# koide3/hdl_graph_slam

Measured on AMD Instinct MI355X. Metric: registrations/sec (64-beam ~120k-pt pair), loop-closure batch, higher is better.
Workload: dtype f64; 1 GPU; loop-closure batch: 64 candidate keyframes/GPU x HDL-64E (~118848 pts) vs 1 query keyframe, FAST_GICP + getFitnessScore, cold (index + covariances rebuilt every step); candidate set: SURVEY 8d (distinct ray-casts at poses within 20 m of the query, guess = ground truth + 0.5 m / 2 deg noise, z forced to 0); candidates_per_gpu=64, points_per_cloud=118848, method=FAST_GICP, distinct_scans=16, parallelism=single GPU

## Files before the change

hdl_graph_slam_amd/csrc/hgs_consts.h:

```cpp
#pragma once
#include <cfloat>
#include <cmath>

#include "../../include/hgs_registration.h"
#include "hgs_floor.h"
#include "hgs_gicp.h"
#include "hgs_icp.h"
#include "hgs_ndt.h"
#include "hgs_vgicp.h"

namespace hgs {

inline GicpConsts gicp_consts(const hgs_params& p) {
  GicpConsts c;
  const double thr = p.max_correspondence_distance;
  c.max_corr2 = thr * thr;
  c.search_bound2 = c.max_corr2 >= (double)FLT_MAX ? FLT_MAX : nextafterf((float)c.max_corr2, FLT_MAX);
  c.rotation_eps = p.rotation_epsilon;
  c.translation_eps = p.transformation_epsilon;
  c.lm_init_lambda_factor = p.lm_init_lambda_factor;
  c.lm_max_iterations = p.lm_max_iterations;
  c.max_iterations = p.max_iterations;
  c.k_correspondences = p.correspondence_randomness;
  return c;
}

inline VgicpConsts vgicp_consts(const hgs_params& p) {
  VgicpConsts c;
  c.resolution = p.resolution;
  c.search = p.neighbor_search == HGS_DIRECT27 ? 3 : (p.neighbor_search == HGS_DIRECT7 ? 2 : 1);
  c.pad = 0;
  return c;
}

inline IcpConsts icp_consts(const hgs_params& p) {
  IcpConsts c;
  const double thr = p.max_correspondence_distance;
  c.max_corr2 = thr * thr;
  c.search_bound2 = c.max_corr2 >= (double)FLT_MAX ? FLT_MAX : nextafterf((float)c.max_corr2, FLT_MAX);
  c.max_iterations = p.max_iterations;
  c.trans_eps = p.transformation_epsilon;
  c.rot_thr = p.rotation_epsilon > 0 ? p.rotation_epsilon : 1.0 - p.transformation_epsilon;
  c.reciprocal = p.icp_reciprocal ? 1 : 0;
  c.pad = 0;
  return c;
}

inline NdtConsts ndt_consts(const hgs_params& p) {
  NdtConsts c;
  const double c1 = 10.0 * (1 - p.ndt_outlier_ratio);
  const double c2 = p.ndt_outlier_ratio / std::pow(p.resolution, 3);
  const double d3 = -std::log(c2);
  c.gauss_d1 = -std::log(c1 + c2) - d3;
  c.gauss_d2 = -2 * std::log((-std::log(c1 * std::exp(-0.5) + c2) - d3) / c.gauss_d1);
  c.step_size = p.ndt_step_size;
  c.trans_eps = p.transformation_epsilon;
  c.max_iterations = p.max_iterations;
  c.search = p.neighbor_search == HGS_DIRECT1 ? 1 : (p.neighbor_search == HGS_KDTREE ? 0 : 2);
  c.kdtree_radius2 = (float)(p.resolution * p.resolution);
  c.line_search = p.ndt_line_search ? 1 : 0;
  c.upstream_hd1_sign = p.ndt_upstream_hd1_sign;
  c.pad = 0;
  return c;
}

inline FloorConsts floor_consts(const hgs_floor_params* p) {
  FloorConsts c{};
  const double angle = (double)(float)(p->tilt_deg * M_PI / 180.0);
  c.rx = p->tilt_deg == 0.0 ? 0.f : -(float)std::sin(angle);
  c.rz = p->tilt_deg == 0.0 ? 1.f : (float)std::cos(angle);
  c.nrx = (double)c.rx, c.nrz = (double)c.rz;
  c.clip_lo = (float)(p->sensor_height + p->height_clip_range);
  c.clip_hi = (float)(p->sensor_height - p->height_clip_range);
  c.normal_cos = std::cos(p->normal_filter_thresh * M_PI / 180.0);
  c.dist_thresh = p->ransac_distance_threshold;
  c.log_prob = std::log(1.0 - p->ransac_probability);
  c.max_iterations = p->ransac_max_iterations;
  c.seed = p->seed;
  return c;
}

}
```

hdl_graph_slam_amd/csrc/hgs_device.h:

```cpp
#pragma once
#include <hip/hip_runtime.h>
#include "hgs_gicp.h"
#include "hgs_floor.h"
#include "hgs_icp.h"
#include "hgs_ndt.h"
#include "hgs_vgicp.h"

namespace hgs {

struct CloudMeta {
  int nvalid;
  int ndt_ncells;
  unsigned bbmin[3];
  unsigned bbmax[3];
  int ndt_min_b[3], ndt_max_b[3], ndt_div_mul[3];
  int ndt_error;
  int vg_ncells;
  int vg_min_b[3], vg_max_b[3], vg_div_mul[3];
  int vg_error;
  int pad[1];
};

struct CloudDesc {
  const float4* raw;
  float4* pts;
  float4* lpts;
  float4* nodes;
  float4* cov;
  int* corr;
  CloudMeta* meta;
  int n_input;
  int P;
  int sort_off;
  int pad;
};

struct TargetView {
  const float4* nodes;
  const float4* pts;
  const float4* lpts;
  const float4* cov;
  const CloudMeta* meta;
  int P;
  int seed_bits;
  const unsigned* seed_tab;
};

struct NdtTargetView {
  const int* hash_keys;
  const int* hash_vals;
  const NdtCellRec* cells;
  const CloudMeta* meta;
  const int2* hash_kv;
  int hash_mask;
  float inv_leaf;
};

struct NdtAccum {
  unsigned long long w[kAccNdt * 4];
  unsigned tiles_done;
  unsigned overflow;
  double out[kAccNdt];
};

struct DevResult {
  float T[16];
  int converged, iterations, lm_tries, pad;
  double error;
  double fit_sum;
  unsigned fit_count;
  unsigned pad2;
};

struct Progress {
  int* dev;
  volatile int* host_done;
  volatile int* host_rounds;
  int B;
  int pad;
};

constexpr int kFusedRoundMaxProblems = 4;
constexpr int kBlock = 256;
constexpr int kKnnLaneList = 16;
constexpr int kKnnLeafLog = 128;
constexpr int kNW = 1;
constexpr int kTileNN = kBlock * kNW;

void launch_pack_aos(hipStream_t s, const float4* staged , int n, float4* raw, float* intensity , CloudMeta* meta_to_reset ,
                     const CloudDesc* desc = nullptr , CloudDesc* desc_out = nullptr);
void launch_meta_init(hipStream_t s, const CloudDesc* descs, int ncloud);
void launch_bbox_count(hipStream_t s, const CloudDesc* descs, int ncloud, int max_n);
void launch_hilbert_keys(hipStream_t s, const CloudDesc* descs, int ncloud, int max_n, unsigned long long* keys, unsigned* vals, int drop_bits);
void launch_gather_sorted(hipStream_t s, const CloudDesc* descs, int ncloud, int max_slots, const unsigned* sorted_vals);
void launch_build_tree(hipStream_t s, const CloudDesc* descs, int ncloud, int max_P);
void launch_knn_cov(hipStream_t s, const CloudDesc* descs, int ncloud, int max_n, int k, int qpw, int reg_method, int gather ,
                    double* raw_stage = nullptr );

void launch_gicp_init(hipStream_t s, GicpState* states, const float* guesses, int B, Progress prog);
struct Guess16 {
  float m[16];
};
void launch_gicp_init1(hipStream_t s, GicpState* states, const float* guess_host , Progress prog);
void launch_gicp_linearize(hipStream_t s, const CloudDesc* descs, TargetView tgt, const GicpState* states, GicpConsts c, double* partials, int max_blocks, int B,
                           int qpw);
void launch_gicp_solve(hipStream_t s, const CloudDesc* descs, GicpState* states, GicpConsts c, const double* partials, int max_blocks, int B,
                       int tile_points );
void launch_gicp_error(hipStream_t s, const CloudDesc* descs, TargetView tgt, const GicpState* states, double* partials_err, int max_blocks, int B);
void launch_gicp_linearize_round2(hipStream_t s, const CloudDesc* descs, TargetView tgt, const GicpState* states_in, GicpState* states_out, GicpConsts c, double* partials,
                                  const double* partials_err, int max_blocks , int lin_blocks , int B, int qpw, Progress prog,
                                  DevResult* results, DevResult* early_out );
void launch_gicp_error_round2(hipStream_t s, const CloudDesc* descs, TargetView tgt, const GicpState* states_in, GicpState* states_out, GicpConsts c, const double* partials,
                              double* partials_err, int max_blocks, int err_blocks , int B, int lin_tile_points);
void launch_gicp_decide(hipStream_t s, const CloudDesc* descs, GicpState* states, GicpConsts c, const double* partials_err, int max_blocks, int B, Progress prog);
void launch_gicp_results(hipStream_t s, const GicpState* states, DevResult* out, int B);

void launch_icp_init(hipStream_t s, IcpState* states, const float* guesses, int B, Progress prog);
void launch_icp_correspond(hipStream_t s, const CloudDesc* descs, TargetView tgt, const IcpState* states, IcpConsts c, double* partials, int max_blocks, int B);
void launch_icp_solve(hipStream_t s, const CloudDesc* descs, IcpState* states, IcpConsts c, const double* partials, int max_blocks, int B, Progress prog);
void launch_icp_results(hipStream_t s, const IcpState* states, DevResult* out, int B);

void launch_fitness(hipStream_t s, const CloudDesc* descs, TargetView tgt, const DevResult* poses, double max_range, double* partials, int max_blocks, int B,
                    int use_seed, int qpw);
void launch_fitness_final(hipStream_t s, const CloudDesc* descs, const double* partials, int max_blocks, DevResult* out, int B, int tile_pts);
void launch_gicp_linearize(hipStream_t s, const CloudDesc* descs, const TargetView* tviews, const GicpState* states, GicpConsts c, double* partials, int max_blocks, int B,
                           int qpw);
void launch_gicp_error(hipStream_t s, const CloudDesc* descs, const TargetView* tviews, const GicpState* states, double* partials_err, int max_blocks, int B);
void launch_gicp_linearize_round2(hipStream_t s, const CloudDesc* descs, const TargetView* tviews, const GicpState* states_in, GicpState* states_out, GicpConsts c, double* partials,
                                  const double* partials_err, int max_blocks, int lin_blocks, int B, int qpw, Progress prog, DevResult* results, DevResult* early_out);
void launch_gicp_error_round2(hipStream_t s, const CloudDesc* descs, const TargetView* tviews, const GicpState* states_in, GicpState* states_out, GicpConsts c, const double* partials,
                              double* partials_err, int max_blocks, int err_blocks, int B, int lin_tile_points);
void launch_icp_correspond(hipStream_t s, const CloudDesc* descs, const TargetView* tviews, const IcpState* states, IcpConsts c, double* partials, int max_blocks, int B);
void launch_fitness(hipStream_t s, const CloudDesc* descs, const TargetView* tviews, const DevResult* poses, double max_range, double* partials, int max_blocks, int B,
                    int use_seed, int qpw);
}
struct hgs_result;
namespace hgs {
void launch_results_to_records(hipStream_t s, const DevResult* res, const int* candidate_ids, int n, int n_slots, ::hgs_result* out);
void launch_nn_query(hipStream_t s, TargetView tgt, const float4* q, int nq, int* idx, float* d2);
void launch_seed_grid_build(hipStream_t s, const float4* pts, const CloudMeta* meta, int n_max, unsigned* tab, int bits);
inline size_t seed_grid_entries(int bits) { return ((size_t)1 << bits) + ((size_t)1 << (bits - 2)) + ((size_t)1 << (bits - 4)); }
struct SeedGridJob {
  const float4* pts;
  const CloudMeta* meta;
  unsigned* tab;
  int bits;
  int pad;
};
void launch_seed_grid_build_batch(hipStream_t s, const SeedGridJob* jobs, int njobs, size_t max_entries, int max_n);
void launch_transform(hipStream_t s, const float4* raw, int n, const float* T16_colmajor_dev, float4* out);

void launch_ndt_grid_params(hipStream_t s, CloudDesc desc, float inv_leaf);
void launch_ndt_cell_keys(hipStream_t s, CloudDesc desc, float inv_leaf, unsigned long long* keys, unsigned* vals);
void launch_ndt_build_cells(hipStream_t s, CloudDesc desc, const unsigned long long* sorted_keys, const unsigned* sorted_vals, int min_points,
                            int* hash_keys, int* hash_vals, int hash_mask, NdtCellRec* cells);
void launch_ndt_init(hipStream_t s, NdtState* states, NdtAngles* angles, const float* guesses, NdtConsts c, int B, Progress prog, NdtAccum* accum_to_zero );
void launch_ndt_pack_hash(hipStream_t s, const int* keys, const int* vals, int2* kv, int cap);
void launch_ndt_pass(hipStream_t s, const CloudDesc* descs, NdtTargetView tgt, NdtState* states, NdtAngles* angles, NdtConsts c, NdtAccum* accum, const int* tile_base,
                     unsigned long long* queues, int B, int parity, int blocks, int chunk, int sorted, int debug, Progress prog);
void launch_ndt_pass(hipStream_t s, const CloudDesc* descs, const NdtTargetView* tviews, NdtState* states, NdtAngles* angles, NdtConsts c, NdtAccum* accum, const int* tile_base,
                     unsigned long long* queues, int B, int parity, int blocks, int chunk, int sorted, int debug, Progress prog);
void launch_ndt_results(hipStream_t s, const CloudDesc* descs, const NdtState* states, DevResult* out, int B);

void launch_vgicp_grid_params(hipStream_t s, CloudDesc desc, double resolution);
void launch_vgicp_cell_keys(hipStream_t s, CloudDesc desc, double resolution, unsigned long long* keys, unsigned* vals);
void launch_vgicp_build_cells(hipStream_t s, CloudDesc desc, const unsigned long long* sorted_keys, const unsigned* sorted_vals, int* hash_keys,
                              int* hash_vals, int hash_mask, NdtCellRec* cells);
void launch_vgicp_linearize(hipStream_t s, const CloudDesc* descs, NdtTargetView tgt, const GicpState* states, VgicpConsts c, double* partials,
                            int max_blocks, int B);
void launch_vgicp_error(hipStream_t s, const CloudDesc* descs, NdtTargetView tgt, const GicpState* states, VgicpConsts c, double* partials_err,
                        int max_blocks, int B);
void launch_vgicp_linearize(hipStream_t s, const CloudDesc* descs, const NdtTargetView* tviews, const GicpState* states, VgicpConsts c, double* partials,
                            int max_blocks, int B);
void launch_vgicp_error(hipStream_t s, const CloudDesc* descs, const NdtTargetView* tviews, const GicpState* states, VgicpConsts c, double* partials_err,
                        int max_blocks, int B);

struct MapSource {
  const float4* raw;
  const float* intensity;
  int n, offset;
  float T[16];
};
void launch_map_transform(hipStream_t s, const MapSource* srcs, int nsrc, int max_n, float4* out);
constexpr int kMapMaxDepth = 21;
constexpr int kMapMaxEvents = kMapMaxDepth + 3;
struct MapOctreeEvent {
  int index, depth;
  double mn[3];
  unsigned long long gained[3];
};
struct MapOctree {
  int first;
  int next_viol;
  int n_events, overflow, done, pad;
  double mx[3];
  MapOctreeEvent events[kMapMaxEvents];
};
void launch_map_first_finite(hipStream_t s, const float4* pts, int n, MapOctree* oct);
void launch_map_octree_init(hipStream_t s, const float4* pts, int n, double res, MapOctree* oct);
void launch_map_octree_step(hipStream_t s, const float4* pts, int n, double res, MapOctree* oct);
void launch_map_keys(hipStream_t s, const float4* pts, int n, double res, const MapOctree* oct, unsigned long long* keys, unsigned* vals);
void launch_map_centers(hipStream_t s, const unsigned long long* keys, const unsigned* head, const unsigned* slot, int n, double res, const MapOctree* oct, float4* out,
                        int* count_out);

struct PfFrame {
  float rows[12];
};
void launch_pf_load(hipStream_t s, const float4* staged, int n, float4* out, const float* deskew_w , double scan_period,
                    const PfFrame* frame , int* count_out, unsigned* meta_out );
void launch_pf_distance_flags(hipStream_t s, const float4* pts, int n, int use_filter, double near_thresh, double far_thresh, unsigned* keep);
void launch_pf_compact(hipStream_t s, const float4* in, int n, const unsigned* keep, const unsigned* slot, float4* out, int* count);
void launch_pf_bbox(hipStream_t s, const float4* pts, const int* count, int cap, unsigned* meta, int dist_filter = 0, double near_thresh = 0, double far_thresh = 0);
void launch_pf_grid(hipStream_t s, unsigned* meta, float inv_leaf);
void launch_pf_voxel_keys(hipStream_t s, const float4* pts, const int* count, const unsigned* meta, float inv_leaf, int cap, unsigned long long* keys, unsigned* vals,
                          int dist_filter = 0, double near_thresh = 0, double far_thresh = 0);
void launch_pf_voxel_heads(hipStream_t s, const unsigned long long* keys, int cap, unsigned* head, unsigned long long invalid_key);
constexpr unsigned long long kVoxelInvalidKey = 0xffffffffull;
constexpr unsigned long long kMapInvalidKey = ~0ull;
void launch_pf_voxel_centroids(hipStream_t s, const float4* pts, const unsigned long long* keys, const unsigned* vals, const unsigned* head, const unsigned* slot, int cap,
                               float4* out, int* count_out, unsigned* ukeys = nullptr );
void launch_pf_grid_radius_flags(hipStream_t s, const float4* cen, const int* count, const unsigned* ukeys, const unsigned* meta, float inv_leaf, float radius, float r2,
                                 int min_neighbors, int cap, unsigned* keep);
void launch_pf_approx_keys(hipStream_t s, const float4* pts, const int* count, float inv_leaf, int cap, unsigned long long* keys, unsigned* vals);
void launch_pf_approx_heads(hipStream_t s, const float4* pts, const unsigned long long* keys, const unsigned* vals, float inv_leaf, int cap, unsigned* head, unsigned* evict,
                            unsigned* bucket_used , unsigned* bucket_rank );
void launch_pf_approx_centroids(hipStream_t s, const float4* pts, const unsigned long long* keys, const unsigned* vals, const unsigned* head, const unsigned* evict,
                                const unsigned* evict_rank, const unsigned* bucket_rank, int cap, float4* out, int* count_out);
void launch_pf_radius_flags(hipStream_t s, CloudDesc d, float r2, int min_neighbors, unsigned* keep);
void launch_pf_mean_knn_dist(hipStream_t s, CloudDesc d, int mean_k, double* dist);
void launch_pf_statistical(hipStream_t s, CloudDesc d, const double* dist, double* stats, double stddev_mul, unsigned* keep);
void launch_pf_to_cloud(hipStream_t s, const float4* in, int n, float4* raw, float* intensity, CloudMeta* meta_to_reset, const CloudDesc* desc = nullptr, CloudDesc* desc_out = nullptr);

struct PfSweep {
  int off, n;
  int count;
  int deskew, frame;
  float w[3];
  double scan_period;
  float rows[12];
  unsigned meta[16];
};
constexpr int kPfBatchOrdinalBits = 12;
void launch_pfb_load(hipStream_t s, const float4* staged, PfSweep* sweeps, int nsweeps, int max_n, float4* out);
void launch_pfb_distance_flags(hipStream_t s, const float4* pts, const PfSweep* sweeps, int nsweeps, int max_n, double near_thresh, double far_thresh, unsigned* keep);
void launch_pfb_compact(hipStream_t s, const float4* in, PfSweep* sweeps, int nsweeps, int max_n, const unsigned* keep, const unsigned* slot, float4* out);
void launch_pfb_bbox(hipStream_t s, const float4* pts, PfSweep* sweeps, int nsweeps, int max_n, int dist_filter, double near_thresh, double far_thresh);
void launch_pfb_grid(hipStream_t s, PfSweep* sweeps, int nsweeps, float inv_leaf);
void launch_pfb_voxel_keys(hipStream_t s, const float4* pts, const PfSweep* sweeps, int nsweeps, int max_n, float inv_leaf, unsigned long long* keys, unsigned* vals,
                           int dist_filter, double near_thresh, double far_thresh);
void launch_pfb_voxel_heads(hipStream_t s, const unsigned long long* keys, const PfSweep* sweeps, int nsweeps, int max_n, unsigned* head);
void launch_pfb_voxel_centroids(hipStream_t s, const float4* pts, const unsigned long long* keys, const unsigned* vals, const unsigned* head, const unsigned* slot,
                                PfSweep* sweeps, int nsweeps, int max_n, float4* out, unsigned* ukeys );
void launch_pfb_grid_radius_flags(hipStream_t s, const float4* cen, const unsigned* ukeys, const PfSweep* sweeps, int nsweeps, int max_n, float inv_leaf, float radius,
                                  float r2, int min_neighbors, unsigned* keep);
void launch_pfb_to_cloud(hipStream_t s, const float4* in, const PfSweep* sweeps, const CloudDesc* descs, CloudDesc* const* desc_outs, float* const* intensities, int nsweeps,
                         int max_m);

void launch_floor_clip_flags(hipStream_t s, const float4* raw, const float* intensity, int n, FloorConsts c, float4* out , unsigned* keep);
void launch_knn_cov_raw(hipStream_t s, const CloudDesc* descs , int max_n, int k, int qpw, int gather, double* raw_stage );
void launch_floor_normal_flags(hipStream_t s, CloudDesc d, const double* raw_cov, FloorConsts c, unsigned* keep , double* normals );
void launch_floor_ransac_init(hipStream_t s, FloorRansacState* st, int max_iterations, Progress prog);
void launch_floor_ransac_planes(hipStream_t s, const float4* pts, int n, unsigned seed, int i0, int nh, const FloorRansacState* st , double* planes ,
                                int* counts );
void launch_floor_ransac_count(hipStream_t s, const float4* pts, int n, double thresh, const double* planes, int nh, const FloorRansacState* st , int* counts);
void launch_floor_ransac_decide(hipStream_t s, const int* counts, const double* planes, int i0, int nh, int n, int max_iterations, double log_prob, FloorRansacState* st,
                                Progress prog);
void launch_floor_inlier_flags(hipStream_t s, const float4* pts, int n, const FloorRansacState* st, double thresh, unsigned* keep);

void launch_gicp_debug_state(hipStream_t s, GicpState* st, const double* T12_dev);
void launch_ndt_debug_state(hipStream_t s, NdtState* st, NdtAngles* ang, const double* p6_dev, NdtConsts c);
void launch_reduce_partials(hipStream_t s, const double* partials, int ntiles, int width , double* out);

}
```

hdl_graph_slam_amd/csrc/hgs_engine.hip:

```cpp
#include <hip/hip_runtime.h>
#include <algorithm>
#include <atomic>
#include <chrono>
#include <climits>
#include <condition_variable>
#include <cmath>
#include <cstdio>
#include <cstdlib>
#include <cstring>
#include <exception>
#include <limits>
#include <mutex>
#include <new>
#include <stdexcept>
#include <string>
#include <thread>
#include <vector>

#include "../../include/hgs_registration.h"
#include "hgs_comm.h"
#include "hgs_consts.h"
#include "hgs_device.h"
#include "hgs_resources.h"
#include "hgs_sort.h"

using namespace hgs;

namespace {

thread_local std::string g_create_error;


int next_pow2(int v) {
  int p = 1;
  while (p < v) p <<= 1;
  return p;
}
size_t align_up(size_t v, size_t a) { return (v + a - 1) / a * a; }

}

struct VoxelTable {
  DeviceBuffer block;
  int* hash_keys = nullptr;
  int* hash_vals = nullptr;
  int2* hash_kv = nullptr;
  NdtCellRec* cells = nullptr;
  int hash_cap = 0;
};

struct hgs_cloud {
  hgs_handle* owner = nullptr;
  size_t n_input = 0;
  int P = 1;
  DeviceBuffer block;
  CloudDesc desc{};
  CloudDesc* dev_desc = nullptr;
  float* intensity = nullptr;
  bool has_index = false;
  bool corr_stale = false;
  bool has_cov = false;
  int cov_k = 0;
  bool has_ndt = false;
  double ndt_resolution = 0;
  int ndt_min_points = 0;
  VoxelTable ndt;
  bool has_vg = false;
  double vg_resolution = 0;
  int vg_cov_k = 0;
  long long vg_span[3] = {0, 0, 0};
  bool vg_too_large = false;
  VoxelTable vg;
  bool has_seed = false;
  DeviceBuffer seed_block;
  int seed_bits = 0;
};

struct ProfEvent {
  int stage;
  hipEvent_t a, b;
};

struct hgs_handle {
  hgs_params prm{};
  int device = 0;
  hipStream_t stream = nullptr;
  hipStream_t lane_stream[7] = {};
  hipEvent_t lane_event[8] = {};
  int lane_start = 1;
  int nn_qpw = 0;
  int nn_qpw16_below = 96, nn_qpw32_below = 0;
  int hilbert_levels = 13;
  hipEvent_t comm_event = nullptr;
  int prefilter_fast = 1;
  int upload_trace = 0;
  int floor_chunk = 64;
  int early_run_ahead = 2;
  int early_result = 1;
  PinnedBuffer h_early;
  hipEvent_t early_event = nullptr;
  bool early_pending = false, early_valid = false;
  int fused_rounds = 1;
  int fused_rounds_below = 262144;
  int fused_rounds_max_problems = kFusedRoundMaxProblems, fused_rounds_max_blocks = 640;
  int cov_split = 1;
  int resident_descs = 1;
  int knn_qpw_tiny = -1;
  int knn_tiny_below = 32768;
  int seed_grid = 1;
  int knn_replay = -1;
  int batch_lanes = 0;
  std::string err;
  hgs_cloud* target = nullptr;
  hgs_cloud* source = nullptr;
  bool own_target = false, own_source = false;
  float final_T[16];

  DeviceBuffer staging, sort_keys[2], sort_vals[2], sort_tmp, descs, states, angles, partials, partials_err, results, guesses, done, misc;
  DeviceBuffer lane_partials[7], lane_partials_err[7];
  DeviceBuffer ndt_accum;
  DeviceBuffer group_tviews, group_corr;
  DeviceBuffer group_vviews;
  DeviceBuffer seed_jobs;
  int pair_chunk = 0;
  hgs::Comm* comm = nullptr;
  DeviceBuffer comm_send, comm_recv, comm_ids;
  DeviceBuffer pf_ukeys;
  DeviceBuffer cov_raw;
  DeviceBuffer ndt_plan;
  int ndt_resident_blocks = 0;
  int ndt_chunk = 0;
  int ndt_sort = -1;
  DeviceBuffer pf_a, pf_b, pf_keep, pf_slot, pf_small, pf_dist;
  DeviceBuffer pf_table;
  PinnedBuffer h_pf_table;
  PinnedBuffer h_results, h_small, h_flags, h_comm;
  PinnedRing up;
  PinnedRing up_points;
  PinnedBuffer up_big;
  hipEvent_t up_big_event = nullptr;
  bool up_big_pending = false;
  PackPool pack_pool;
  PinnedBuffer h_xform;

  std::vector<DeviceBuffer> block_pool;
  std::vector<hgs_cloud*> live_clouds;
  std::recursive_mutex api_mutex;

  bool profiling = false;
  std::vector<ProfEvent> prof_events;
  std::vector<ProfEvent> prof_free;
  double prof_ms[HGS_STAGE_COUNT];
  uint64_t prof_launches[HGS_STAGE_COUNT];

  hgs_handle() = default;
  hgs_handle(const hgs_handle&) = delete;
  hgs_handle& operator=(const hgs_handle&) = delete;
  void synchronize_streams() {
    if (stream) (void)hipStreamSynchronize(stream);
    for (hipStream_t ls : lane_stream)
      if (ls) (void)hipStreamSynchronize(ls);
  }
  ~hgs_handle();
};

namespace {

#define HGS_HIP(h, call)                                                                                           \
  do {                                                                                                             \
    hipError_t e__ = (call);                                                                                       \
    if (e__ != hipSuccess) {                                                                                       \
      char buf__[512];                                                                                             \
      snprintf(buf__, sizeof(buf__), "%s failed: %s (%s:%d)", #call, hipGetErrorString(e__), __FILE__, __LINE__);  \
      (h)->err = buf__;                                                                                            \
      return HGS_ERR_HIP;                                                                                          \
    }                                                                                                              \
  } while (0)

#define HGS_TRY(expr)             \
  do {                            \
    int rc__ = (expr);            \
    if (rc__ != HGS_OK) return rc__; \
  } while (0)

struct StageTimer {
  hgs_handle* h;
  ProfEvent ev{};
  bool active = false;
  StageTimer(hgs_handle* h_, int stage) : h(h_) {
    if (!h->profiling) return;
    if (!h->prof_free.empty()) {
      ev = h->prof_free.back();
      h->prof_free.pop_back();
    } else {
      if (hipEventCreate(&ev.a) != hipSuccess || hipEventCreate(&ev.b) != hipSuccess) return;
    }
    ev.stage = stage;
    active = hipEventRecord(ev.a, h->stream) == hipSuccess;
  }
  ~StageTimer() {
    if (!active) return;
    (void)hipEventRecord(ev.b, h->stream);
    h->prof_events.push_back(ev);
  }
};

struct ApiLock {
  std::unique_lock<std::recursive_mutex> lk;
  explicit ApiLock(hgs_handle* h) {
    if (h) lk = std::unique_lock<std::recursive_mutex>(h->api_mutex);
  }
  explicit ApiLock(hgs_cloud* c) : ApiLock(c ? c->owner : nullptr) {}
};

int set_device(hgs_handle* h) {
  HGS_HIP(h, hipSetDevice(h->device));
  return HGS_OK;
}

constexpr size_t kUploadChunkPoints = 16384;
#ifndef HGS_UPLOAD_PARALLEL_POINTS
#define HGS_UPLOAD_PARALLEL_POINTS 49152
#endif
constexpr size_t kUploadParallelPoints = HGS_UPLOAD_PARALLEL_POINTS;
int upload_image_open(hgs_handle* h, size_t records) {
  if (h->up_big_pending) {
    HGS_HIP(h, hipEventSynchronize(h->up_big_event));
    h->up_big_pending = false;
  }
  HGS_HIP(h, h->up_big.reserve(records * sizeof(float4)));
  return HGS_OK;
}
int upload_image_close(hgs_handle* h) {
  if (!h->up_big_event) HGS_HIP(h, hipEventCreateWithFlags(&h->up_big_event, hipEventDisableTiming));
  HGS_HIP(h, hipEventRecord(h->up_big_event, h->stream));
  h->up_big_pending = true;
  return HGS_OK;
}
int upload_points_at(hgs_handle* h, const void* pts, size_t n, size_t stride_bytes, size_t off, bool in_image) {
  const bool has_intensity = stride_bytes >= 20;
  const char* src = static_cast<const char*>(pts);
  float4* const dev = h->staging.as<float4>() + off;
  if (n >= kUploadParallelPoints) {
    if (!in_image) HGS_TRY(upload_image_open(h, n));
    float4* const image = h->up_big.as<float4>() + (in_image ? off : 0);
    const size_t nchunks = (n + kUploadChunkPoints - 1) / kUploadChunkPoints;
    std::vector<std::atomic<unsigned char>> ready(nchunks);
    for (auto& r : ready) r.store(0, std::memory_order_relaxed);
    PackPool::Job job;
    job.src = src, job.dst = reinterpret_cast<float*>(image), job.n = n, job.stride = stride_bytes, job.chunk = kUploadChunkPoints, job.nchunks = nchunks;
    job.has_intensity = has_intensity, job.ready = ready.data();
    h->pack_pool.post(&job);
    hipError_t err = hipSuccess;
    for (size_t c = 0; c < nchunks; c++) {
      while (!ready[c].load(std::memory_order_acquire))
        if (!PackPool::help(job)) std::this_thread::yield();
      const size_t i0 = c * kUploadChunkPoints, m = std::min(kUploadChunkPoints, n - i0);
      if (err == hipSuccess) err = hipMemcpyAsync(dev + i0, image + i0, m * sizeof(float4), hipMemcpyHostToDevice, h->stream);
    }
    h->pack_pool.retire();
    HGS_HIP(h, err);
    if (!in_image) HGS_TRY(upload_image_close(h));
    return HGS_OK;
// ... 250 lines not shown
}

template <typename P, typename K, typename C>
int build_voxel_table(hgs_handle* h, const hgs_cloud* c, VoxelTable& t, int cap, int max_cells, bool packed, P&& grid_params, K&& cell_keys, C&& build_cells) {
  const size_t n = c->n_input;
  if (!t.block.p || t.hash_cap != cap) {
    const size_t o_keys = 0, o_vals = align_up((size_t)cap * 4, 256), o_kv = o_vals + align_up((size_t)cap * 4, 256);
    const size_t o_cells = o_kv + (packed ? align_up((size_t)cap * 8, 256) : 0);
    HGS_HIP(h, t.block.alloc(o_cells + (size_t)max_cells * sizeof(NdtCellRec)));
    char* base = t.block.as<char>();
    t.hash_keys = (int*)(base + o_keys);
    t.hash_vals = (int*)(base + o_vals);
    t.hash_kv = packed ? (int2*)(base + o_kv) : nullptr;
    t.cells = (NdtCellRec*)(base + o_cells);
    t.hash_cap = cap;
  }
  HGS_HIP(h, hipMemsetAsync(t.hash_keys, 0xff, (size_t)cap * 4, h->stream));
  grid_params();
  if (n > 0) {
    HGS_TRY(reserve_sort_pairs(h, n));
    cell_keys(h->sort_keys[0].as<unsigned long long>(), h->sort_vals[0].as<unsigned>());
    HGS_TRY(sort_pairs(h, n, 0, 32));
    build_cells(h->sort_keys[1].as<unsigned long long>(), h->sort_vals[1].as<unsigned>());
  }
  return HGS_OK;
}

int ensure_ndt_target(hgs_handle* h, hgs_cloud* c) {
  const double res = h->prm.resolution;
  const int min_pts = h->prm.ndt_min_points_per_voxel;
  if (c->has_ndt && c->ndt_resolution == res && c->ndt_min_points == min_pts) return HGS_OK;
  StageTimer tm(h, HGS_STAGE_VOXELIZE);
  const int max_cells = (int)(c->n_input / (size_t)std::max(1, min_pts)) + 1;
  const int cap = next_pow2(std::max(64, 4 * max_cells));
  const float inv_leaf = 1.0f / (float)res;
  VoxelTable& t = c->ndt;
  HGS_TRY(build_voxel_table(
      h, c, t, cap, max_cells, true, [&] { launch_ndt_grid_params(h->stream, c->desc, inv_leaf); },
      [&](unsigned long long* keys, unsigned* vals) { launch_ndt_cell_keys(h->stream, c->desc, inv_leaf, keys, vals); },
      [&](unsigned long long* keys, unsigned* vals) { launch_ndt_build_cells(h->stream, c->desc, keys, vals, min_pts, t.hash_keys, t.hash_vals, cap - 1, t.cells); }));
  launch_ndt_pack_hash(h->stream, t.hash_keys, t.hash_vals, t.hash_kv, cap);
  HGS_HIP(h, hipGetLastError());
  c->has_ndt = true;
  c->ndt_resolution = res;
  c->ndt_min_points = min_pts;
  return HGS_OK;
}

int vgicp_grid_too_large(hgs_handle* h, const hgs_cloud* c) {
  char msg[256];
  snprintf(msg, sizeof(msg),
           "FAST_VGICP: the target's voxel grid spans %lld x %lld x %lld cells at resolution %g, more than the 2147483647 a linear voxel key addresses "
           "(a far stray point in the target?)",
           c->vg_span[0], c->vg_span[1], c->vg_span[2], c->vg_resolution);
  h->err = msg;
  return HGS_ERR_UNSUPPORTED;
}

int ensure_vgicp_target(hgs_handle* h, hgs_cloud* c) {
  const double res = h->prm.resolution;
  const int k = h->prm.correspondence_randomness;
  if (c->has_vg && c->vg_resolution == res && c->vg_cov_k == cov_cache_key(h, k)) return c->vg_too_large ? vgicp_grid_too_large(h, c) : HGS_OK;
  StageTimer tm(h, HGS_STAGE_VOXELIZE);
  const int max_cells = (int)c->n_input + 1;
  const int cap = next_pow2(std::max<int>(64, 2 * max_cells));
  VoxelTable& t = c->vg;
  HGS_TRY(build_voxel_table(
      h, c, t, cap, max_cells, false, [&] { launch_vgicp_grid_params(h->stream, c->desc, res); },
      [&](unsigned long long* keys, unsigned* vals) { launch_vgicp_cell_keys(h->stream, c->desc, res, keys, vals); },
      [&](unsigned long long* keys, unsigned* vals) { launch_vgicp_build_cells(h->stream, c->desc, keys, vals, t.hash_keys, t.hash_vals, cap - 1, t.cells); }));
  HGS_HIP(h, hipGetLastError());
  HGS_HIP(h, h->h_small.reserve(sizeof(CloudMeta)));
  const CloudMeta* hm = h->h_small.as<CloudMeta>();
  HGS_HIP(h, hipMemcpyAsync(h->h_small.p, c->desc.meta, sizeof(CloudMeta), hipMemcpyDeviceToHost, h->stream));
  HGS_HIP(h, hipStreamSynchronize(h->stream));
  for (int d = 0; d < 3; d++) c->vg_span[d] = (long long)hm->vg_max_b[d] - hm->vg_min_b[d] + 1;
  c->vg_too_large = hm->vg_error != 0;
  c->has_vg = true;
  c->vg_resolution = res;
  c->vg_cov_k = cov_cache_key(h, k);
  return c->vg_too_large ? vgicp_grid_too_large(h, c) : HGS_OK;
}

NdtTargetView voxel_target_view(const hgs_cloud* c, const VoxelTable& t, float inv_leaf) {
  NdtTargetView tv;
  tv.hash_keys = t.hash_keys, tv.hash_vals = t.hash_vals, tv.cells = t.cells, tv.meta = c->desc.meta, tv.hash_kv = t.hash_kv;
  tv.hash_mask = t.hash_cap - 1, tv.inv_leaf = inv_leaf;
  return tv;
}
NdtTargetView ndt_target_view(const hgs_handle* h, const hgs_cloud* t) { return voxel_target_view(t, t->ndt, 1.0f / (float)h->prm.resolution); }
NdtTargetView vgicp_target_view(const hgs_cloud* t) { return voxel_target_view(t, t->vg, 0.f); }

TargetView target_view(const hgs_cloud* c) {
  TargetView t;
  t.nodes = c->desc.nodes, t.pts = c->desc.pts, t.lpts = c->desc.lpts, t.cov = c->desc.cov, t.meta = c->desc.meta, t.P = c->P;
  t.seed_bits = c->has_seed ? c->seed_bits : 0, t.seed_tab = c->has_seed ? c->seed_block.as<const unsigned>() : nullptr;
  return t;
}

int ensure_seed_grid(hgs_handle* h, hgs_cloud* c) {
  if (!h->seed_grid || c->has_seed || !c->has_index || c->n_input == 0) return HGS_OK;
  int bits = 12;
  while (bits < 24 && ((size_t)1 << bits) < 4 * c->n_input) bits++;
  const size_t bytes = seed_grid_entries(bits) * sizeof(unsigned);
  if (!c->seed_block.p || c->seed_bits != bits) {
    HGS_HIP(h, c->seed_block.alloc(bytes));
    c->seed_bits = bits;
  }
  HGS_HIP(h, hipMemsetAsync(c->seed_block.p, 0xff, bytes, h->stream));
  launch_seed_grid_build(h->stream, c->desc.pts, c->desc.meta, (int)c->n_input, c->seed_block.as<unsigned>(), bits);
  HGS_HIP(h, hipGetLastError());
  c->has_seed = true;
  return HGS_OK;
}

int ensure_seed_grids(hgs_handle* h, const std::vector<hgs_cloud*>& all) {
  if (!h->seed_grid) return HGS_OK;
  std::vector<hgs_cloud*> todo;
  for (hgs_cloud* c : all)
    if (!c->has_seed && c->has_index && c->n_input > 0 && std::find(todo.begin(), todo.end(), c) == todo.end()) todo.push_back(c);
  constexpr size_t kMaxJobs = 65535;
  for (size_t start = 0; start < todo.size(); start += kMaxJobs) {
    const size_t nj = std::min(kMaxJobs, todo.size() - start);
    std::vector<SeedGridJob> jobs(nj);
    size_t max_entries = 0;
    int max_n = 0;
    for (size_t j = 0; j < nj; j++) {
      hgs_cloud* c = todo[start + j];
      int bits = 12;
      while (bits < 24 && ((size_t)1 << bits) < 4 * c->n_input) bits++;
      const size_t entries = seed_grid_entries(bits);
      if (!c->seed_block.p || c->seed_bits != bits) {
        HGS_HIP(h, c->seed_block.alloc(entries * sizeof(unsigned)));
        c->seed_bits = bits;
      }
      jobs[j] = SeedGridJob{c->desc.pts, c->desc.meta, c->seed_block.as<unsigned>(), bits, 0};
      max_entries = std::max(max_entries, entries), max_n = std::max(max_n, (int)c->n_input);
    }
    HGS_HIP(h, h->seed_jobs.reserve(nj * sizeof(SeedGridJob)));
    HGS_HIP(h, h->up.upload(h->seed_jobs.p, jobs.data(), nj * sizeof(SeedGridJob), h->stream));
    launch_seed_grid_build_batch(h->stream, h->seed_jobs.as<SeedGridJob>(), (int)nj, max_entries, max_n);
    HGS_HIP(h, hipGetLastError());
    for (size_t j = 0; j < nj; j++) todo[start + j]->has_seed = true;
  }
  return HGS_OK;
}

NdtConsts engine_ndt_consts(const hgs_params& p) {
  NdtConsts c = ndt_consts(p);
  c.pad = std::getenv("HGS_TRACE") ? 1 : 0;
  return c;
}

constexpr int kMaxCountedDevices = 64;
std::atomic<int> g_streams_in_use[kMaxCountedDevices] = {};
std::atomic<int>& streams_in_use(int device) { return g_streams_in_use[(unsigned)device % kMaxCountedDevices]; }
int hw_queue_budget() {
  static const int budget = [] {
    const char* e = std::getenv("GPU_MAX_HW_QUEUES");
    const int v = e ? std::atoi(e) : 0;
    return v > 0 ? v : 4;
  }();
  return budget;
}
constexpr int kFloorMaxChunk = 4096;
constexpr int kMaxLanes = 8;

int make_progress(hgs_handle* h, int lane, int B, Progress* out) {
  if (h->early_pending) {
    HGS_HIP(h, hipEventSynchronize(h->early_event));
    h->early_pending = false;
  }
  HGS_HIP(h, h->done.reserve(64));
  HGS_HIP(h, h->h_flags.reserve(64));
  volatile int* hf = h->h_flags.as<volatile int>() + 2 * lane;
  hf[0] = 0, hf[1] = 0;
  out->dev = h->done.as<int>() + 2 * lane;
  out->host_done = hf, out->host_rounds = hf + 1;
  out->B = B, out->pad = 0;
  return HGS_OK;
}

struct BatchLane {
  hipStream_t stream = nullptr;
  int b0 = 0, B = 0;
  Progress prog{};
  double* partials = nullptr;
  double* partials_err = nullptr;
  long round = 0;
  bool finished = false;
};

int open_lanes(hgs_handle* h, int B, size_t partial_bytes_per_problem, size_t partial_err_bytes_per_problem, std::vector<BatchLane>& lanes, int tiles_per_problem) {
  const bool small_problems = tiles_per_problem > 0 && tiles_per_problem <= 96;
  const int by_size = h->prm.method == HGS_NDT_OMP ? (B > 32 && !small_problems ? 3 : 4) : (small_problems && (long)B * tiles_per_problem <= 3072 ? 1 : 4);
  const int wanted = h->batch_lanes > 0 ? h->batch_lanes : by_size;
  int n = h->profiling ? 1 : std::max(1, std::min(std::min(wanted, kMaxLanes), B));
  if (h->batch_lanes <= 0) {
    int owned = 0;
    while (owned < kMaxLanes - 1 && h->lane_stream[owned]) owned++;
    const int room = std::max(0, hw_queue_budget() - streams_in_use(h->device).load(std::memory_order_relaxed));
    n = std::min(n, 1 + owned + room);
  }
  lanes.assign(n, BatchLane{});
  for (int i = 0, b0 = 0; i < n; i++) {
    BatchLane& L = lanes[i];
    L.b0 = b0, L.B = (B - b0) / (n - i);
    b0 += L.B;
    HGS_TRY(make_progress(h, i, L.B, &L.prog));
    if (i == 0) {
      L.stream = h->stream;
      L.partials = h->partials.as<double>(), L.partials_err = h->partials_err.as<double>();
      continue;
    }
    if (!h->lane_stream[i - 1]) {
      HGS_HIP(h, hipStreamCreateWithFlags(&h->lane_stream[i - 1], hipStreamNonBlocking));
      streams_in_use(h->device).fetch_add(1, std::memory_order_relaxed);
    }
    L.stream = h->lane_stream[i - 1];
    HGS_HIP(h, h->lane_partials[i - 1].reserve((size_t)L.B * partial_bytes_per_problem));
    HGS_HIP(h, h->lane_partials_err[i - 1].reserve((size_t)L.B * partial_err_bytes_per_problem));
    L.partials = h->lane_partials[i - 1].as<double>(), L.partials_err = h->lane_partials_err[i - 1].as<double>();
  }
  if (n > 1) {
    if (h->lane_start != 0) HGS_HIP(h, hipStreamSynchronize(h->stream));
    if (!h->lane_event[0]) HGS_HIP(h, hipEventCreateWithFlags(&h->lane_event[0], hipEventDisableTiming));
    HGS_HIP(h, hipEventRecord(h->lane_event[0], h->stream));
    for (int i = 1; i < n; i++) HGS_HIP(h, hipStreamWaitEvent(lanes[i].stream, h->lane_event[0], 0));
  }
  return HGS_OK;
}

int close_lanes(hgs_handle* h, std::vector<BatchLane>& lanes) {
  for (size_t i = 1; i < lanes.size(); i++) {
    if (!h->lane_event[i]) HGS_HIP(h, hipEventCreateWithFlags(&h->lane_event[i], hipEventDisableTiming));
    HGS_HIP(h, hipEventRecord(h->lane_event[i], lanes[i].stream));
    HGS_HIP(h, hipStreamWaitEvent(h->stream, h->lane_event[i], 0));
  }
  return HGS_OK;
}

constexpr long kRunAhead = 2;
template <typename F, typename G>
void drive_lanes(std::vector<BatchLane>& lanes, long max_rounds, F&& enqueue_round, G&& on_finished, long run_ahead = kRunAhead) {
  long spins = 0;
  for (;;) {
    bool all_finished = true, enqueued = false;
    for (BatchLane& L : lanes) {
      if (L.finished) continue;
      if (*L.prog.host_done || L.round >= max_rounds) {
        L.finished = true;
        on_finished(L);
        continue;
      }
      all_finished = false;
      if (L.round - (long)*L.prog.host_rounds < run_ahead) {
        enqueue_round(L);
        L.round++;
        enqueued = true;
      }
    }
    if (all_finished) return;
    if (enqueued) {
      spins = 0;
      continue;
    }
    if ((++spins & 0x3ff) == 0) {
      for (BatchLane& L : lanes)
        if (!L.finished && !*L.prog.host_done && hipStreamQuery(L.stream) == hipSuccess && !*L.prog.host_done &&
            L.round - (long)*L.prog.host_rounds >= run_ahead) {
          enqueue_round(L);
          L.round++;
        }
    }
#if defined(__x86_64__)
    __builtin_ia32_pause();
#endif
  }
}

struct BatchShape {
  int B, max_n;
  int qpw, nn_tile;
  bool gicp_round2;
  int lin_qpw, lin_tile, lin_blocks;
  int max_blocks, err_blocks;
  const CloudDesc* d_descs;
  const TargetView* d_tviews;
  const NdtTargetView* d_vviews;
};

template <typename F>
void with_lane_target(const BatchShape& s, const BatchLane& L, const TargetView& tv, F&& launch) {
  if (s.d_tviews) launch(s.d_tviews + L.b0);
  else launch(tv);
}

int batch_shape(hgs_handle* h, const std::vector<hgs_cloud*>& sources, bool lm_rounds, BatchShape* out, int* const* corr_of = nullptr) {
  BatchShape& s = *out;
  s.d_tviews = nullptr, s.d_vviews = nullptr;
  s.B = (int)sources.size();
  s.max_n = 0;
  for (hgs_cloud* c : sources) s.max_n = std::max(s.max_n, (int)c->n_input);
  const int B = s.B, max_n = s.max_n;
  s.qpw = 64;
  s.nn_tile = (kBlock / 64) * s.qpw * kNW;
  s.gicp_round2 = lm_rounds && h->prm.method == HGS_FAST_GICP && h->fused_rounds && max_n <= h->fused_rounds_below &&
                  (B <= h->fused_rounds_max_problems || (long)B * ((max_n + kBlock - 1) / kBlock) <= (long)h->fused_rounds_max_blocks);
  const long tiles64 = (long)B * ((max_n + s.nn_tile - 1) / s.nn_tile);
  s.lin_qpw = !s.gicp_round2 ? 64 : h->nn_qpw > 0 ? h->nn_qpw : tiles64 <= (long)h->nn_qpw16_below ? 16 : tiles64 <= (long)h->nn_qpw32_below ? 32 : 64;
  s.lin_tile = (kBlock / 64) * s.lin_qpw * kNW;
  s.lin_blocks = std::max(1, (max_n + s.lin_tile - 1) / s.lin_tile);
  s.max_blocks = std::max(1, s.lin_qpw < 64 ? (max_n + 63) / 64 : (max_n + s.nn_tile - 1) / s.nn_tile);
  s.err_blocks = std::max(1, (max_n + kBlock - 1) / kBlock);
  return upload_descs(h, sources, false, &s.d_descs, nullptr, corr_of);
}

bool corr_seeds_fitness(int method) { return method == HGS_FAST_GICP || method == HGS_ICP; }
void lane_fitness(hgs_handle* h, BatchLane& L, const BatchShape& s, double max_range, bool corr_seeds) {
  StageTimer tm(h, HGS_STAGE_FITNESS);
  DevResult* res = h->results.as<DevResult>() + L.b0;
  with_lane_target(s, L, s.d_tviews ? TargetView{} : target_view(h->target),
                   [&](auto tgt) { launch_fitness(L.stream, s.d_descs + L.b0, tgt, res, max_range, L.partials_err, s.max_blocks, L.B, corr_seeds ? 1 : 0, s.qpw); });
  launch_fitness_final(L.stream, s.d_descs + L.b0, L.partials_err, s.max_blocks, res, L.B, s.nn_tile);
}
void lane_fitness_tail(hgs_handle* h, BatchLane& L, const BatchShape& s, const double* fit_max_range) {
  if (fit_max_range) lane_fitness(h, L, s, *fit_max_range, corr_seeds_fitness(h->prm.method));
}

int run_gicp_rounds(hgs_handle* h, const BatchShape& s, const float* guesses_host, bool guess_in_args, const double* fit_max_range) {
  const int B = s.B, max_blocks = s.max_blocks;
  hgs_cloud* tgt = h->target;
  const bool voxel = h->prm.method == HGS_FAST_VGICP;
  const GicpConsts c = gicp_consts(h->prm);
  const VgicpConsts vc = vgicp_consts(h->prm);
  const bool round2 = s.gicp_round2;
  const bool early = round2 && B == 1 && !fit_max_range && h->early_result && !h->profiling;
  DevResult* early_out = nullptr;
  if (early) {
    HGS_HIP(h, h->h_early.reserve(sizeof(DevResult)));
    early_out = h->h_early.as<DevResult>();
  }
  HGS_HIP(h, h->states.reserve((size_t)B * sizeof(GicpState) * (round2 ? 2 : 1)));
  GicpState* st = h->states.as<GicpState>();
  GicpState* st_other = st + B;
  const TargetView tv = s.d_tviews || s.d_vviews ? TargetView{} : target_view(tgt);
  const NdtTargetView vtv = voxel && !s.d_vviews ? vgicp_target_view(tgt) : NdtTargetView{};
  const long max_rounds = (long)std::max(1, c.max_iterations) * std::max(1, c.lm_max_iterations) + 2 + (round2 ? 1 : 0);
  std::vector<BatchLane> lanes;
  HGS_TRY(open_lanes(h, B, (size_t)max_blocks * kAccNdt * sizeof(double), (size_t)max_blocks * 2 * sizeof(double), lanes, s.err_blocks));
  auto finish_lane = [&](BatchLane& L) {
    if (early && *L.prog.host_done) {
      h->early_valid = true;
      return;
    }
    launch_gicp_results(L.stream, st + L.b0, h->results.as<DevResult>() + L.b0, L.B);
    lane_fitness_tail(h, L, s, fit_max_range);
  };
  if (guess_in_args) launch_gicp_init1(lanes[0].stream, st, guesses_host, lanes[0].prog);
  else
    for (BatchLane& L : lanes) launch_gicp_init(L.stream, st + L.b0, h->guesses.as<float>() + (size_t)L.b0 * 16, L.B, L.prog);
  drive_lanes(lanes, max_rounds, [&](BatchLane& L) {
    const CloudDesc* dd = s.d_descs + L.b0;
    GicpState* ls = st + L.b0;
    if (round2) {
      {
        StageTimer tm(h, HGS_STAGE_LINEARIZE);
        with_lane_target(s, L, tv, [&](auto t) {
          launch_gicp_linearize_round2(L.stream, dd, t, ls, st_other + L.b0, c, L.partials, L.partials_err, max_blocks, s.lin_blocks, L.B, s.lin_qpw, L.prog,
                                       h->results.as<DevResult>() + L.b0, early_out);
        });
      }
      StageTimer tm(h, HGS_STAGE_ERROR);
      with_lane_target(s, L, tv, [&](auto t) {
        launch_gicp_error_round2(L.stream, dd, t, st_other + L.b0, ls, c, L.partials, L.partials_err, max_blocks, s.err_blocks, L.B, s.lin_tile);
      });
      return;
    }
    {
      StageTimer tm(h, HGS_STAGE_LINEARIZE);
      if (voxel && s.d_vviews) launch_vgicp_linearize(L.stream, dd, s.d_vviews + L.b0, ls, vc, L.partials, max_blocks, L.B);
      else if (voxel) launch_vgicp_linearize(L.stream, dd, vtv, ls, vc, L.partials, max_blocks, L.B);
      else with_lane_target(s, L, tv, [&](auto t) { launch_gicp_linearize(L.stream, dd, t, ls, c, L.partials, max_blocks, L.B, s.qpw); });
    }
    {
      StageTimer tm(h, HGS_STAGE_SOLVE);
      launch_gicp_solve(L.stream, dd, ls, c, L.partials, max_blocks, L.B, voxel ? kBlock : s.nn_tile);
    }
    {
      StageTimer tm(h, HGS_STAGE_ERROR);
      if (voxel && s.d_vviews) launch_vgicp_error(L.stream, dd, s.d_vviews + L.b0, ls, vc, L.partials_err, max_blocks, L.B);
      else if (voxel) launch_vgicp_error(L.stream, dd, vtv, ls, vc, L.partials_err, max_blocks, L.B);
      else with_lane_target(s, L, tv, [&](auto t) { launch_gicp_error(L.stream, dd, t, ls, L.partials_err, max_blocks, L.B); });
    }
    {
      StageTimer tm(h, HGS_STAGE_SOLVE);
      launch_gicp_decide(L.stream, dd, ls, c, L.partials_err, max_blocks, L.B, L.prog);
    }
  }, finish_lane, early ? (long)h->early_run_ahead : kRunAhead);
  HGS_TRY(close_lanes(h, lanes));
  if (h->early_valid) {
    if (!h->early_event) HGS_HIP(h, hipEventCreateWithFlags(&h->early_event, hipEventDisableTiming));
    HGS_HIP(h, hipEventRecord(h->early_event, h->stream));
    h->early_pending = true;
  }
  return HGS_OK;
}

int run_icp_rounds(hgs_handle* h, const BatchShape& s, const double* fit_max_range) {
  const int B = s.B, max_blocks = s.max_blocks;
  const IcpConsts c = icp_consts(h->prm);
  HGS_HIP(h, h->states.reserve((size_t)B * sizeof(IcpState)));
  IcpState* st = h->states.as<IcpState>();
  const TargetView tv = s.d_tviews ? TargetView{} : target_view(h->target);
  const long max_rounds = (long)std::max(0, c.max_iterations) + 2;
  std::vector<BatchLane> lanes;
  HGS_TRY(open_lanes(h, B, (size_t)max_blocks * kAccIcp * sizeof(double), (size_t)max_blocks * 2 * sizeof(double), lanes, s.err_blocks));
  auto finish_lane = [&](BatchLane& L) {
    launch_icp_results(L.stream, st + L.b0, h->results.as<DevResult>() + L.b0, L.B);
    lane_fitness_tail(h, L, s, fit_max_range);
  };
  for (BatchLane& L : lanes) launch_icp_init(L.stream, st + L.b0, h->guesses.as<float>() + (size_t)L.b0 * 16, L.B, L.prog);
  drive_lanes(lanes, max_rounds, [&](BatchLane& L) {
    {
      StageTimer tm(h, HGS_STAGE_LINEARIZE);
      with_lane_target(s, L, tv, [&](auto t) { launch_icp_correspond(L.stream, s.d_descs + L.b0, t, st + L.b0, c, L.partials, max_blocks, L.B); });
    }
    StageTimer tm(h, HGS_STAGE_SOLVE);
    launch_icp_solve(L.stream, s.d_descs + L.b0, st + L.b0, c, L.partials, max_blocks, L.B, L.prog);
  }, finish_lane);
  return close_lanes(h, lanes);
}

struct NdtLanePlan {
  int* tile_base;
  unsigned long long* queues;
  int blocks, chunk;
};
int ndt_lane_plans(hgs_handle* h, const std::vector<hgs_cloud*>& sources, const std::vector<BatchLane>& lanes, std::vector<NdtLanePlan>& plans) {
  plans.assign(lanes.size(), NdtLanePlan{});
  const size_t per_lane = align_up(16 + (sources.size() + 1) * sizeof(int), 256);
  bool tile_overflow = false;
  constexpr long long kMaxNdtBlocks = 1 << 16, kMaxNdtChunk = 1 << 10;
  HGS_HIP(h, h->ndt_plan.reserve(per_lane * lanes.size()));
  void* staged = nullptr;
  int plan_slot = 0;
  HGS_HIP(h, h->up.stage(per_lane * lanes.size(), &staged, &plan_slot));
  std::memset(staged, 0, per_lane * lanes.size());
  char* const host = static_cast<char*>(staged);
  for (size_t li = 0; li < lanes.size(); li++) {
    const BatchLane& L = lanes[li];
    int* tb = reinterpret_cast<int*>(host + li * per_lane + 16);
    tb[0] = 0;
    long long tiles64 = 0;
    for (int k = 0; k < L.B; k++) {
      tiles64 += std::max<long long>(1, ((long long)sources[L.b0 + k]->n_input + kBlock - 1) / kBlock);
      tile_overflow = tile_overflow || tiles64 > (long long)INT_MAX - (long long)kMaxNdtBlocks * kMaxNdtChunk;
      tb[k + 1] = tile_overflow ? 0 : (int)tiles64;
    }
    NdtLanePlan& P = plans[li];
    const int total = tb[L.B];
    if (tile_overflow) continue;
    P.blocks = std::max(1, std::min(total, h->ndt_resident_blocks > 0 ? std::min(h->ndt_resident_blocks, (int)kMaxNdtBlocks) : (lanes.size() > 1 ? 512 : 768)));
    P.chunk = h->ndt_chunk > 0 ? std::min(h->ndt_chunk, (int)kMaxNdtChunk) : 8;
    P.queues = reinterpret_cast<unsigned long long*>((char*)h->ndt_plan.p + li * per_lane);
    P.tile_base = reinterpret_cast<int*>((char*)h->ndt_plan.p + li * per_lane + 16);
  }
  if (tile_overflow) {
    h->err = "NDT batch too large: the tiles of one lane do not fit 32-bit item arithmetic (more than ~5e11 source points in one call)";
    return HGS_ERR_INVALID_ARGUMENT;
  }
  HGS_HIP(h, hipMemcpyAsync(h->ndt_plan.p, host, per_lane * lanes.size(), hipMemcpyHostToDevice, h->stream));
  HGS_HIP(h, h->up.commit(plan_slot, h->stream));
  if (lanes.size() > 1) {
    HGS_HIP(h, hipEventRecord(h->lane_event[0], h->stream));
    for (size_t i = 1; i < lanes.size(); i++) HGS_HIP(h, hipStreamWaitEvent(lanes[i].stream, h->lane_event[0], 0));
  }
  return HGS_OK;
}

int run_ndt_rounds(hgs_handle* h, const std::vector<hgs_cloud*>& sources, const BatchShape& s, const double* fit_max_range) {
  const int B = s.B, max_blocks = s.max_blocks;
  const NdtConsts c = engine_ndt_consts(h->prm);
  HGS_HIP(h, h->states.reserve((size_t)B * sizeof(NdtState)));
  HGS_HIP(h, h->angles.reserve((size_t)B * sizeof(NdtAngles)));
  NdtState* st = h->states.as<NdtState>();
  NdtAngles* ang = h->angles.as<NdtAngles>();
  const NdtTargetView tv = s.d_vviews ? NdtTargetView{} : ndt_target_view(h, h->target);
  if (h->ndt_sort == 1) HGS_TRY(ensure_index(h, sources));
  bool sorted = h->ndt_sort != 0;
  for (hgs_cloud* sc : sources) sorted = sorted && sc->has_index;
  HGS_HIP(h, h->ndt_accum.reserve((size_t)B * sizeof(NdtAccum)));
  NdtAccum* accum = h->ndt_accum.as<NdtAccum>();
  const long max_rounds = ((long)c.max_iterations + 4) * (c.line_search ? 11 : 1);
  std::vector<BatchLane> lanes;
  HGS_TRY(open_lanes(h, B, (size_t)max_blocks * 2 * sizeof(double), (size_t)max_blocks * 2 * sizeof(double), lanes, s.err_blocks));
  auto finish_lane = [&](BatchLane& L) {
    launch_ndt_results(L.stream, s.d_descs + L.b0, st + L.b0, h->results.as<DevResult>() + L.b0, L.B);
    lane_fitness_tail(h, L, s, fit_max_range);
  };
  std::vector<NdtLanePlan> plans;
  HGS_TRY(ndt_lane_plans(h, sources, lanes, plans));
  for (BatchLane& L : lanes) launch_ndt_init(L.stream, st + L.b0, ang + L.b0, h->guesses.as<float>() + (size_t)L.b0 * 16, c, L.B, L.prog, accum + L.b0);
  drive_lanes(lanes, max_rounds, [&](BatchLane& L) {
    StageTimer tm(h, HGS_STAGE_LINEARIZE);
    const NdtLanePlan& P = plans[&L - lanes.data()];
    if (s.d_vviews)
      launch_ndt_pass(L.stream, s.d_descs + L.b0, s.d_vviews + L.b0, st + L.b0, ang + L.b0, c, accum + L.b0, P.tile_base, P.queues, L.B, (int)(L.round & 1), P.blocks,
                      P.chunk, sorted ? 1 : 0, 0, L.prog);
    else
      launch_ndt_pass(L.stream, s.d_descs + L.b0, tv, st + L.b0, ang + L.b0, c, accum + L.b0, P.tile_base, P.queues, L.B, (int)(L.round & 1), P.blocks, P.chunk,
                      sorted ? 1 : 0, 0, L.prog);
  }, finish_lane);
  return close_lanes(h, lanes);
}

int run_batch(hgs_handle* h, const std::vector<hgs_cloud*>& sources, const float* guesses_host, const double* fit_max_range = nullptr) {
  const int B = (int)sources.size();
  h->early_valid = false;
  hgs_cloud* tgt = h->target;
  const int method = h->prm.method;
  const bool gicp = method == HGS_FAST_GICP || method == HGS_FAST_VGICP;
  std::vector<hgs_cloud*> all(sources);
  if (fit_max_range) {
    std::vector<hgs_cloud*> searched(sources);
    searched.push_back(tgt);
    HGS_TRY(ensure_index(h, searched));
  }
  if (gicp) {
    all.push_back(tgt);
    HGS_TRY(ensure_cov(h, all, h->prm.correspondence_randomness));
    if (method == HGS_FAST_VGICP) HGS_TRY(ensure_vgicp_target(h, tgt));
  } else if (method == HGS_ICP) {
    all.push_back(tgt);
    HGS_TRY(ensure_index(h, all));
  } else {
    HGS_TRY(ensure_ndt_target(h, tgt));
  }
  if (fit_max_range && method != HGS_FAST_GICP) HGS_TRY(ensure_seed_grid(h, tgt));
  BatchShape s;
  HGS_TRY(batch_shape(h, sources, true, &s));
  const bool guess_in_args = B == 1 && method == HGS_FAST_GICP;
  HGS_HIP(h, h->guesses.reserve((size_t)B * 16 * sizeof(float)));
  if (!guess_in_args) HGS_HIP(h, h->up.upload(h->guesses.p, guesses_host, (size_t)B * 16 * sizeof(float), h->stream));
  HGS_HIP(h, h->results.reserve((size_t)B * sizeof(DevResult)));
  HGS_HIP(h, h->partials.reserve((size_t)B * s.max_blocks * kAccNdt * sizeof(double)));
  HGS_HIP(h, h->partials_err.reserve((size_t)B * s.max_blocks * 2 * sizeof(double)));
  if (gicp) HGS_TRY(run_gicp_rounds(h, s, guesses_host, guess_in_args, fit_max_range));
  else if (method == HGS_ICP) HGS_TRY(run_icp_rounds(h, s, fit_max_range));
  else HGS_TRY(run_ndt_rounds(h, sources, s, fit_max_range));
  HGS_HIP(h, hipGetLastError());
  return HGS_OK;
}

int run_group_batch(hgs_handle* h, const std::vector<hgs_cloud*>& targets, const std::vector<hgs_cloud*>& sources, const float* guesses_host, const double* fit_max_range) {
  const int B = (int)sources.size();
  const int method = h->prm.method;
  h->early_valid = false;
  std::vector<hgs_cloud*> all(sources);
  all.insert(all.end(), targets.begin(), targets.end());
  if (method == HGS_FAST_GICP) HGS_TRY(ensure_cov(h, all, h->prm.correspondence_randomness));
  else HGS_TRY(ensure_index(h, all));
  if (fit_max_range && method != HGS_FAST_GICP)
    for (hgs_cloud* t : targets) HGS_TRY(ensure_seed_grid(h, t));
// ... 66 lines not shown
    HGS_HIP(h, h->group_tviews.reserve((size_t)B * sizeof(TargetView)));
    HGS_HIP(h, h->up.upload(h->group_tviews.p, views.data(), (size_t)B * sizeof(TargetView), h->stream));
  }
  BatchShape s;
  HGS_TRY(batch_shape(h, sources, true, &s, voxel ? corr_of.data() : nullptr));
  s.d_vviews = h->group_vviews.as<NdtTargetView>();
  s.d_tviews = fit_max_range ? h->group_tviews.as<TargetView>() : nullptr;
  HGS_HIP(h, h->guesses.reserve((size_t)B * 16 * sizeof(float)));
  HGS_HIP(h, h->up.upload(h->guesses.p, guesses_host, (size_t)B * 16 * sizeof(float), h->stream));
  HGS_HIP(h, h->results.reserve((size_t)B * sizeof(DevResult)));
  HGS_HIP(h, h->partials.reserve((size_t)B * s.max_blocks * kAccNdt * sizeof(double)));
  HGS_HIP(h, h->partials_err.reserve((size_t)B * s.max_blocks * 2 * sizeof(double)));
  if (voxel) HGS_TRY(run_gicp_rounds(h, s, guesses_host, false, fit_max_range));
  else HGS_TRY(run_ndt_rounds(h, sources, s, fit_max_range));
  HGS_HIP(h, hipGetLastError());
  return HGS_OK;
}

int run_fitness(hgs_handle* h, const std::vector<hgs_cloud*>& sources, double max_range, bool use_corr_seeds) {
  std::vector<hgs_cloud*> all(sources);
  all.push_back(h->target);
  HGS_TRY(ensure_index(h, all));
  if (!use_corr_seeds) HGS_TRY(ensure_seed_grid(h, h->target));
  BatchShape s;
  HGS_TRY(batch_shape(h, sources, false, &s));
  HGS_HIP(h, h->partials_err.reserve((size_t)s.B * s.max_blocks * 2 * sizeof(double)));
  BatchLane whole;
  whole.stream = h->stream, whole.B = s.B, whole.partials_err = h->partials_err.as<double>();
  lane_fitness(h, whole, s, max_range, use_corr_seeds);
  HGS_HIP(h, hipGetLastError());
  return HGS_OK;
}

int fetch_results(hgs_handle* h, int B, std::vector<DevResult>& out) {
  HGS_HIP(h, h->h_results.reserve((size_t)B * sizeof(DevResult)));
  HGS_HIP(h, hipMemcpyAsync(h->h_results.p, h->results.p, (size_t)B * sizeof(DevResult), hipMemcpyDeviceToHost, h->stream));
  HGS_HIP(h, hipStreamSynchronize(h->stream));
  out.assign(h->h_results.as<DevResult>(), h->h_results.as<DevResult>() + B);
  return HGS_OK;
}

double fitness_score(const DevResult& d) { return d.fit_count > 0 ? d.fit_sum / (double)d.fit_count : std::numeric_limits<double>::max(); }

int run_pair_fitness(hgs_handle* h, hgs_cloud* const* cloud1, hgs_cloud* const* cloud2, const float* relposes, size_t n_pairs, double max_range,
                     std::vector<DevResult>& out) {
  std::vector<hgs_cloud*> all(cloud2, cloud2 + n_pairs);
  all.insert(all.end(), cloud1, cloud1 + n_pairs);
  HGS_TRY(ensure_index(h, all));
  HGS_TRY(ensure_seed_grids(h, std::vector<hgs_cloud*>(cloud1, cloud1 + n_pairs)));
  const size_t chunk = h->pair_chunk > 0 ? (size_t)h->pair_chunk : 65535;
  out.clear();
  out.reserve(n_pairs);
  for (size_t p0 = 0; p0 < n_pairs; p0 += chunk) {
    const size_t B = std::min(chunk, n_pairs - p0);
    std::vector<TargetView> views(B);
    for (size_t b = 0; b < B; b++) views[b] = target_view(cloud1[p0 + b]);
    HGS_HIP(h, h->group_tviews.reserve(B * sizeof(TargetView)));
    HGS_HIP(h, h->up.upload(h->group_tviews.p, views.data(), B * sizeof(TargetView), h->stream));
    BatchShape s;
    HGS_TRY(batch_shape(h, std::vector<hgs_cloud*>(cloud2 + p0, cloud2 + p0 + B), false, &s));
    s.d_tviews = h->group_tviews.as<TargetView>();
    std::vector<DevResult> poses(B);
    std::memset(poses.data(), 0, B * sizeof(DevResult));
    for (size_t b = 0; b < B; b++) std::memcpy(poses[b].T, relposes + 16 * (p0 + b), sizeof(float) * 16);
    HGS_HIP(h, h->results.reserve(B * sizeof(DevResult)));
    HGS_HIP(h, h->up.upload(h->results.p, poses.data(), B * sizeof(DevResult), h->stream));
    HGS_HIP(h, h->partials_err.reserve(B * s.max_blocks * 2 * sizeof(double)));
    BatchLane whole;
    whole.stream = h->stream, whole.B = (int)B, whole.partials_err = h->partials_err.as<double>();
    lane_fitness(h, whole, s, max_range, false);
    HGS_HIP(h, hipGetLastError());
    std::vector<DevResult> r;
    HGS_TRY(fetch_results(h, (int)B, r));
    out.insert(out.end(), r.begin(), r.end());
  }
  return HGS_OK;
}

void to_public(const DevResult& d, int candidate, bool with_fitness, hgs_result* r) {
  std::memcpy(r->final_transformation, d.T, sizeof(float) * 16);
  r->converged = d.converged;
  r->iterations = d.iterations;
  r->error = d.error;
  r->lm_tries = d.lm_tries;
  r->candidate_id = candidate;
  r->reserved = 0;
  if (with_fitness) {
    r->num_inliers = d.fit_count;
    r->fitness_score = fitness_score(d);
  } else {
    r->num_inliers = 0;
    r->fitness_score = std::numeric_limits<double>::quiet_NaN();
  }
}

int upload_pose_as_result(hgs_handle* h, const float T[16]) {
  HGS_HIP(h, h->results.reserve(sizeof(DevResult)));
  HGS_HIP(h, h->h_results.reserve(sizeof(DevResult)));
  DevResult* r = h->h_results.as<DevResult>();
  std::memset(r, 0, sizeof(DevResult));
  std::memcpy(r->T, T, sizeof(float) * 16);
  HGS_HIP(h, hipMemcpyAsync(h->results.p, r, sizeof(DevResult), hipMemcpyHostToDevice, h->stream));
  return HGS_OK;
}

int status_of_current_exception(hgs_handle* h) noexcept {
  int rc = HGS_ERR_INTERNAL;
  char what[256] = "unknown C++ exception inside the backend";
  try {
    throw;
  } catch (const std::bad_alloc&) {
    rc = HGS_ERR_OUT_OF_MEMORY;
    snprintf(what, sizeof(what), "out of host memory");
  } catch (const std::exception& e) {
    snprintf(what, sizeof(what), "C++ exception inside the backend: %s", e.what());
  } catch (...) {
  }
  try {
    if (h) h->err = what;
    else g_create_error = what;
  } catch (...) {
  }
  return rc;
}

int set_role_cloud(hgs_handle* h, hgs_cloud* c, hgs_cloud* hgs_handle::*role, bool hgs_handle::*own) {
  ApiLock lock(h);
  if (!h || !c || c->owner != h) return HGS_ERR_INVALID_ARGUMENT;
  if (h->*own && h->*role != c) cloud_free(h->*role);
  h->*role = c;
  h->*own = false;
  return HGS_OK;
}
int set_role_points(hgs_handle* h, const void* pts, size_t n, size_t stride_bytes, hgs_cloud* hgs_handle::*role, bool hgs_handle::*own) {
  ApiLock lock(h);
  if (!h) return HGS_ERR_INVALID_ARGUMENT;
  hgs_cloud* c = nullptr;
  HGS_TRY(hgs_cloud_create(h, pts, n, stride_bytes, &c));
  if (h->*own) cloud_free(h->*role);
  h->*role = c;
  h->*own = true;
  return HGS_OK;
}

}

hgs_handle::~hgs_handle() {
  (void)hipSetDevice(device);
  synchronize_streams();
  pack_pool.shutdown();
  if (comm) hgs::comm_destroy(comm);
  for (hipEvent_t ev : lane_event)
    if (ev) (void)hipEventDestroy(ev);
  for (hipEvent_t ev : {comm_event, early_event, up_big_event})
    if (ev) (void)hipEventDestroy(ev);
  for (const std::vector<ProfEvent>* list : {&prof_events, &prof_free})
    for (const ProfEvent& ev : *list) (void)hipEventDestroy(ev.a), (void)hipEventDestroy(ev.b);
  for (hipStream_t ls : lane_stream)
    if (ls) (void)hipStreamDestroy(ls), streams_in_use(device).fetch_sub(1, std::memory_order_relaxed);
  if (stream) (void)hipStreamDestroy(stream), streams_in_use(device).fetch_sub(1, std::memory_order_relaxed);
}

extern "C" {

int hgs_abi_version(void) { return HGS_ABI_VERSION; }

int hgs_debug_set_option(hgs_handle* h, const char* key, int value) try {
  ApiLock lock(h);
  if (!h || !key) return HGS_ERR_INVALID_ARGUMENT;
  const std::string k(key);
  if (k == "batch_lanes") h->batch_lanes = value <= 0 ? 0 : std::min(kMaxLanes, value);
  else if (k == "lane_start") h->lane_start = value != 0 ? 1 : 0;
  else if (k == "ndt_sort") h->ndt_sort = std::max(-1, std::min(1, value));
  else if (k == "cov_split") h->cov_split = value != 0 ? 1 : 0;
  else if (k == "fused_rounds") h->fused_rounds = value != 0 ? 1 : 0;
  else if (k == "early_result") h->early_result = value != 0 ? 1 : 0;
  else if (k == "early_run_ahead") h->early_run_ahead = std::max(1, std::min(8, value));
  else if (k == "fused_rounds_max_problems") h->fused_rounds_max_problems = std::max(0, value);
  else if (k == "fused_rounds_max_blocks") h->fused_rounds_max_blocks = std::max(0, value);
  else if (k == "fused_rounds_below") h->fused_rounds_below = std::max(0, value);
  else if (k == "resident_descs") h->resident_descs = value != 0 ? 1 : 0;
  else if (k == "knn_qpw_tiny") h->knn_qpw_tiny = value < 0 ? -1 : std::max(0, std::min(32, value & ~7));
  else if (k == "knn_tiny_below") h->knn_tiny_below = std::max(0, value);
  else if (k == "seed_grid") h->seed_grid = value != 0 ? 1 : 0;
  else if (k == "knn_replay") h->knn_replay = std::max(-1, std::min(2, value));
  else if (k == "ndt_resident") h->ndt_resident_blocks = std::max(0, value);
  else if (k == "ndt_chunk") h->ndt_chunk = std::max(0, value);
  else if (k == "hilbert_levels") h->hilbert_levels = std::max(4, std::min(16, value));
  else if (k == "nn_qpw") h->nn_qpw = value == 16 ? 16 : (value == 32 ? 32 : (value == 64 ? 64 : 0));
  else if (k == "nn_qpw16_below") h->nn_qpw16_below = std::max(0, value);
  else if (k == "nn_qpw32_below") h->nn_qpw32_below = std::max(0, value);
  else if (k == "upload_trace") h->upload_trace = value != 0 ? 1 : 0;
  else if (k == "prefilter_fast") h->prefilter_fast = value != 0 ? 1 : 0;
  else if (k == "floor_chunk") h->floor_chunk = std::max(1, std::min(kFloorMaxChunk, value));
  else if (k == "pair_chunk") h->pair_chunk = std::max(0, std::min(65535, value));
  else {
    h->err = "hgs_debug_set_option: unknown option '" + k + "'";
    return HGS_ERR_INVALID_ARGUMENT;
  }
  return HGS_OK;
} catch (...) {
  return status_of_current_exception(h);
}

int hgs_params_default(int32_t method, hgs_params* p) try {
  if (!p || method < HGS_FAST_GICP || method > HGS_ICP) return HGS_ERR_INVALID_ARGUMENT;
  std::memset(p, 0, sizeof(*p));
  p->method = method;
  p->max_iterations = 64;
  p->transformation_epsilon = 0.01;
  p->rotation_epsilon = method == HGS_ICP ? 0.0 : 2e-3;
  p->max_correspondence_distance = method == HGS_FAST_GICP || method == HGS_ICP ? 2.5 : (double)FLT_MAX;
  p->correspondence_randomness = 20;
  p->neighbor_search = method == HGS_NDT_OMP ? HGS_DIRECT7 : HGS_DIRECT1;
  p->resolution = method == HGS_NDT_OMP ? 0.5 : 1.0;
  p->ndt_step_size = 0.1;
  p->ndt_outlier_ratio = 0.55;
  p->ndt_min_points_per_voxel = 6;
  p->ndt_upstream_hd1_sign = 1;
  p->lm_max_iterations = 10;
  p->lm_init_lambda_factor = 1e-9;
  p->device_id = 0;
  p->regularization_method = HGS_REG_FROBENIUS;
  p->ndt_line_search = 0;
  p->icp_reciprocal = 0;
  return HGS_OK;
} catch (...) {
  return status_of_current_exception(nullptr);
}

int hgs_create(const hgs_params* p, hgs_handle** out) try {
  if (!p || !out) return HGS_ERR_INVALID_ARGUMENT;
  *out = nullptr;
  if (p->method < HGS_FAST_GICP || p->method > HGS_ICP || p->max_iterations < 0 || p->correspondence_randomness < 1 || p->correspondence_randomness > 64  || !(p->resolution > 0) ||
      p->regularization_method < HGS_REG_FROBENIUS || p->regularization_method > HGS_REG_NONE) {
    g_create_error = "invalid hgs_params";
    return HGS_ERR_INVALID_ARGUMENT;
  }
  int ndev = 0;
  hipError_t e = hipGetDeviceCount(&ndev);
  if (e != hipSuccess || ndev <= 0 || p->device_id < 0 || p->device_id >= ndev) {
    g_create_error = std::string("no usable HIP device: ") + (e != hipSuccess ? hipGetErrorString(e) : "device ordinal out of range");
    return HGS_ERR_NO_DEVICE;
  }
  hgs_handle* h = new hgs_handle();
  h->prm = *p;
  h->device = p->device_id;
  for (int i = 0; i < 16; i++) h->final_T[i] = (i % 5 == 0) ? 1.f : 0.f;
  for (int i = 0; i < HGS_STAGE_COUNT; i++) h->prof_ms[i] = 0, h->prof_launches[i] = 0;
  if (hipSetDevice(h->device) != hipSuccess || hipStreamCreateWithFlags(&h->stream, hipStreamNonBlocking) != hipSuccess) {
    g_create_error = "hipSetDevice / hipStreamCreate failed";
    delete h;
    return HGS_ERR_HIP;
  }
  streams_in_use(h->device).fetch_add(1, std::memory_order_relaxed);
  *out = h;
  return HGS_OK;
} catch (...) {
  return status_of_current_exception(nullptr);
}

int hgs_destroy(hgs_handle* h) try {
  if (!h) return HGS_OK;
  { std::lock_guard<std::recursive_mutex> wait_for_running_call(h->api_mutex); }
  (void)hipSetDevice(h->device);
  h->synchronize_streams();
  if (h->own_target) cloud_free(h->target);
  if (h->own_source) cloud_free(h->source);
  for (hgs_cloud* c : h->live_clouds) {
    cloud_release_device(c, false);
    c->owner = nullptr;
    c->n_input = 0;
  }
  delete h;
  return HGS_OK;
} catch (...) {
  return status_of_current_exception(nullptr);
}

const char* hgs_last_error(const hgs_handle* h) { return h ? h->err.c_str() : g_create_error.c_str(); }

int hgs_cloud_create(hgs_handle* h, const void* pts, size_t n, size_t stride_bytes, hgs_cloud** out) try {
  ApiLock lock(h);
  if (!h || !out || (n > 0 && !pts) || stride_bytes < 12 || (stride_bytes % 4) != 0 || n > (size_t)1 << 30) return HGS_ERR_INVALID_ARGUMENT;
  HGS_TRY(set_device(h));
  const bool trace = h->upload_trace != 0;
  const auto t0 = std::chrono::steady_clock::now();
  hgs_cloud* c = nullptr;
  HGS_TRY(cloud_alloc(h, n, &c));
  const auto t1 = std::chrono::steady_clock::now();
  auto t2 = t1;
  {
    StageTimer tm(h, HGS_STAGE_UPLOAD);
    const float4* staged = nullptr;
    {
      const int rc = upload_points_packed(h, pts, n, stride_bytes, &staged);
      t2 = std::chrono::steady_clock::now();
      if (rc != HGS_OK) {
        cloud_free(c);
        return rc;
      }
    }
    const CloudDesc resident = resident_desc(c);
    launch_pack_aos(h->stream, staged, (int)n, const_cast<float4*>(c->desc.raw), c->intensity, c->desc.meta, &resident, c->dev_desc);
    launch_bbox_count(h->stream, c->dev_desc, 1, (int)n);
    hipError_t e = hipGetLastError();
    if (e != hipSuccess) {
      h->err = std::string("cloud upload failed: ") + hipGetErrorString(e);
      cloud_free(c);
      return HGS_ERR_HIP;
    }
  }
  if (trace) {
    const auto t3 = std::chrono::steady_clock::now();
    auto us = [](auto a, auto b) { return std::chrono::duration<double, std::micro>(b - a).count(); };
    std::fprintf(stderr, "[hgs upload] n %zu: alloc %.1f us, pack + DMA enqueue %.1f us, launches %.1f us\n", n, us(t0, t1), us(t1, t2), us(t2, t3));
  }
  *out = c;
  return HGS_OK;
} catch (...) {
  return status_of_current_exception(h);
}

int hgs_cloud_destroy(hgs_cloud* c) try {
  ApiLock lock(c);
  if (!c) return HGS_OK;
  hgs_handle* h = c->owner;
  if (h) {
    (void)hipSetDevice(h->device);
    (void)hipStreamSynchronize(h->stream);
    if (h->target == c) h->target = nullptr, h->own_target = false;
    if (h->source == c) h->source = nullptr, h->own_source = false;
  }
  cloud_free(c);
  c = nullptr;
  return HGS_OK;
} catch (...) {
// ... 1266 lines not shown
  return HGS_OK;
}

}

extern "C" int hgs_detect_floor(hgs_handle* h, hgs_cloud* cloud, const hgs_floor_params* p, hgs_floor_result* out, hgs_cloud** filtered_out, hgs_cloud** inliers_out) try {
  ApiLock lock(h);
  if (filtered_out) *filtered_out = nullptr;
  if (inliers_out) *inliers_out = nullptr;
  if (!h || !cloud || !p || !out || cloud->owner != h || !floor_params_valid(p)) return HGS_ERR_INVALID_ARGUMENT;
  HGS_TRY(set_device(h));
  std::memset(out, 0, sizeof(*out));
  FloorWork w;
  const int rc = detect_floor_locked(h, cloud, p, out, filtered_out, inliers_out, w);
  cloud_free(w.clipped);
  if (rc != HGS_OK) {
    if (filtered_out && *filtered_out) cloud_free(*filtered_out), *filtered_out = nullptr;
    if (inliers_out && *inliers_out) cloud_free(*inliers_out), *inliers_out = nullptr;
  }
  return rc;
} catch (...) {
  return status_of_current_exception(h);
}

extern "C" int hgs_debug_floor_filter(hgs_handle* h, hgs_cloud* cloud, const hgs_floor_params* p, uint8_t* keep_clip, uint8_t* keep_normal, double* normals3) try {
  ApiLock lock(h);
  if (!h || !cloud || !p || cloud->owner != h || !floor_params_valid(p)) return HGS_ERR_INVALID_ARGUMENT;
  HGS_TRY(set_device(h));
  FloorWork w;
  const int rc = floor_filter(h, cloud, p, floor_consts(p), &w, keep_clip, keep_normal, normals3);
  cloud_free(w.clipped);
  return rc;
} catch (...) {
  return status_of_current_exception(h);
}

extern "C" int hgs_debug_floor_ransac_counts(hgs_handle* h, hgs_cloud* cloud, const hgs_floor_params* p, uint32_t i0, uint32_t n, int32_t* counts, double* coeffs4) try {
  ApiLock lock(h);
  if (!h || !cloud || !p || cloud->owner != h || !floor_params_valid(p) || (n > 0 && !counts) || (uint64_t)i0 + n > 0x7fffffffull) return HGS_ERR_INVALID_ARGUMENT;
  HGS_TRY(set_device(h));
  const int chunk = std::max(1, std::min(kFloorMaxChunk, h->floor_chunk));
  FloorRansacBufs b;
  HGS_TRY(floor_ransac_bufs(h, chunk, &b));
  const FloorConsts c = floor_consts(p);
  const int np = (int)cloud->n_input;
  for (uint32_t done = 0; done < n; done += (uint32_t)chunk) {
    const int nh = (int)std::min<uint32_t>((uint32_t)chunk, n - done);
    launch_floor_ransac_planes(h->stream, cloud->desc.raw, np, c.seed, (int)(i0 + done), nh, nullptr, b.planes, b.counts);
    launch_floor_ransac_count(h->stream, cloud->desc.raw, np, c.dist_thresh, b.planes, nh, nullptr, b.counts);
    HGS_HIP(h, hipGetLastError());
    HGS_HIP(h, hipMemcpyAsync(counts + done, b.counts, (size_t)nh * sizeof(int), hipMemcpyDeviceToHost, h->stream));
    if (coeffs4) HGS_HIP(h, hipMemcpyAsync(coeffs4 + 4 * (size_t)done, b.planes, (size_t)nh * 4 * sizeof(double), hipMemcpyDeviceToHost, h->stream));
    HGS_HIP(h, hipStreamSynchronize(h->stream));
  }
  return HGS_OK;
} catch (...) {
  return status_of_current_exception(h);
}

int hgs_profile_enable(hgs_handle* h, int enabled) try {
  ApiLock lock(h);
  if (!h) return HGS_ERR_INVALID_ARGUMENT;
  h->profiling = enabled != 0;
  return HGS_OK;
} catch (...) {
  return status_of_current_exception(h);
}

int hgs_profile_read(hgs_handle* h, double* ms, uint64_t* launches, int reset) try {
  ApiLock lock(h);
  if (!h) return HGS_ERR_INVALID_ARGUMENT;
  HGS_TRY(set_device(h));
  HGS_HIP(h, hipStreamSynchronize(h->stream));
  for (auto& ev : h->prof_events) {
    float t = 0.f;
    if (hipEventElapsedTime(&t, ev.a, ev.b) == hipSuccess) {
      h->prof_ms[ev.stage] += (double)t;
      h->prof_launches[ev.stage]++;
    }
    h->prof_free.push_back(ev);
  }
  h->prof_events.clear();
  for (int i = 0; i < HGS_STAGE_COUNT; i++) {
    if (ms) ms[i] = h->prof_ms[i];
    if (launches) launches[i] = h->prof_launches[i];
    if (reset) h->prof_ms[i] = 0, h->prof_launches[i] = 0;
  }
  return HGS_OK;
} catch (...) {
  return status_of_current_exception(h);
}

int hgs_synchronize(hgs_handle* h) try {
  ApiLock lock(h);
  if (!h) return HGS_ERR_INVALID_ARGUMENT;
  HGS_TRY(set_device(h));
  HGS_HIP(h, hipStreamSynchronize(h->stream));
  return HGS_OK;
} catch (...) {
  return status_of_current_exception(h);
}

int hgs_debug_target_covariances(hgs_handle* h, float* out6) try {
  ApiLock lock(h);
  if (!h || !out6) return HGS_ERR_INVALID_ARGUMENT;
  if (!h->target) return HGS_ERR_NO_TARGET;
  HGS_TRY(set_device(h));
  hgs_cloud* t = h->target;
  std::vector<hgs_cloud*> all{t};
  HGS_TRY(ensure_cov(h, all, h->prm.correspondence_randomness));
  const size_t slots = (size_t)t->P * kLeaf;
  std::vector<float4> pts(slots), cov(2 * slots);
  int nvalid = 0;
  HGS_HIP(h, hipMemcpyAsync(pts.data(), t->desc.pts, slots * sizeof(float4), hipMemcpyDeviceToHost, h->stream));
  HGS_HIP(h, hipMemcpyAsync(cov.data(), t->desc.cov, 2 * slots * sizeof(float4), hipMemcpyDeviceToHost, h->stream));
  HGS_HIP(h, hipMemcpyAsync(&nvalid, &t->desc.meta->nvalid, sizeof(int), hipMemcpyDeviceToHost, h->stream));
  HGS_HIP(h, hipStreamSynchronize(h->stream));
  std::memset(out6, 0, t->n_input * 6 * sizeof(float));
  for (int i = 0; i < nvalid; i++) {
    int o;
    std::memcpy(&o, &pts[i].w, 4);
    if (o < 0 || (size_t)o >= t->n_input) continue;
    float* p = out6 + (size_t)o * 6;
    p[0] = cov[2 * i].x, p[1] = cov[2 * i].y, p[2] = cov[2 * i].z, p[3] = cov[2 * i].w, p[4] = cov[2 * i + 1].x, p[5] = cov[2 * i + 1].y;
  }
  return HGS_OK;
} catch (...) {
  return status_of_current_exception(h);
}

int hgs_debug_gicp_linearize(hgs_handle* h, const double T12[12], double* H36, double* b6, double* err, int32_t* corr) try {
  ApiLock lock(h);
  if (!h || !T12 || !H36 || !b6 || !err) return HGS_ERR_INVALID_ARGUMENT;
  if (h->prm.method != HGS_FAST_GICP && h->prm.method != HGS_FAST_VGICP) return HGS_ERR_UNSUPPORTED;
  if (!h->target) return HGS_ERR_NO_TARGET;
  if (!h->source) return HGS_ERR_NO_SOURCE;
  HGS_TRY(set_device(h));
  hgs_cloud *s = h->source, *t = h->target;
  const bool voxel = h->prm.method == HGS_FAST_VGICP;
  std::vector<hgs_cloud*> all{s, t};
  HGS_TRY(ensure_cov(h, all, h->prm.correspondence_randomness));
  if (voxel) HGS_TRY(ensure_vgicp_target(h, t));
  const int max_blocks = std::max(1, ((int)s->n_input + kBlock - 1) / kBlock);
  std::vector<hgs_cloud*> src{s};
  const CloudDesc* d_descs = nullptr;
  HGS_TRY(upload_descs(h, src, false, &d_descs, nullptr));
  HGS_HIP(h, h->states.reserve(sizeof(GicpState)));
  HGS_HIP(h, h->partials.reserve((size_t)max_blocks * kAcc * sizeof(double)));
  HGS_HIP(h, h->misc.reserve(64 * sizeof(double)));
  HGS_HIP(h, hipMemsetAsync(h->partials.p, 0, (size_t)max_blocks * kAcc * sizeof(double), h->stream));
  HGS_HIP(h, hipMemcpyAsync(h->misc.p, T12, 12 * sizeof(double), hipMemcpyHostToDevice, h->stream));
  launch_gicp_debug_state(h->stream, h->states.as<GicpState>(), h->misc.as<double>());
  if (voxel) launch_vgicp_linearize(h->stream, d_descs, vgicp_target_view(t), h->states.as<GicpState>(), vgicp_consts(h->prm), h->partials.as<double>(), max_blocks, 1);
  else launch_gicp_linearize(h->stream, d_descs, target_view(t), h->states.as<GicpState>(), gicp_consts(h->prm), h->partials.as<double>(), max_blocks, 1, 64);
  double* d_out = h->misc.as<double>() + 16;
  launch_reduce_partials(h->stream, h->partials.as<double>(), max_blocks, kAcc, d_out);
  double acc[kAcc];
  HGS_HIP(h, hipMemcpyAsync(acc, d_out, sizeof(acc), hipMemcpyDeviceToHost, h->stream));
  const size_t s_slots = (size_t)s->P * kLeaf, t_slots = (size_t)t->P * kLeaf;
  std::vector<float4> spts, tpts;
  std::vector<int> dcorr;
  int s_nvalid = 0;
  if (corr) {
    spts.resize(s_slots), tpts.resize(t_slots), dcorr.resize(s_slots);
    HGS_HIP(h, hipMemcpyAsync(spts.data(), s->desc.pts, s_slots * sizeof(float4), hipMemcpyDeviceToHost, h->stream));
    HGS_HIP(h, hipMemcpyAsync(tpts.data(), t->desc.pts, t_slots * sizeof(float4), hipMemcpyDeviceToHost, h->stream));
    HGS_HIP(h, hipMemcpyAsync(dcorr.data(), s->desc.corr, s_slots * sizeof(int), hipMemcpyDeviceToHost, h->stream));
    HGS_HIP(h, hipMemcpyAsync(&s_nvalid, &s->desc.meta->nvalid, sizeof(int), hipMemcpyDeviceToHost, h->stream));
  }
  HGS_HIP(h, hipStreamSynchronize(h->stream));
  int k = 0;
  for (int r = 0; r < 6; r++)
    for (int c = r; c < 6; c++) H36[r * 6 + c] = H36[c * 6 + r] = acc[k++];
  for (int i = 0; i < 6; i++) b6[i] = acc[21 + i];
  *err = acc[27];
  if (corr) {
    for (size_t i = 0; i < s->n_input; i++) corr[i] = voxel ? 0 : -1;
    for (int i = 0; i < s_nvalid; i++) {
      int so, to = -1;
      std::memcpy(&so, &spts[i].w, 4);
      const int j = dcorr[i];
      if (voxel) to = j;
      else if (j >= 0 && (size_t)j < t_slots) std::memcpy(&to, &tpts[j].w, 4);
      if (so >= 0 && (size_t)so < s->n_input) corr[so] = to;
    }
  }
  return HGS_OK;
} catch (...) {
  return status_of_current_exception(h);
}

int hgs_debug_icp_correspond(hgs_handle* h, const double T12[12], double* sums17, int32_t* corr) try {
  ApiLock lock(h);
  if (!h || !T12 || !sums17) return HGS_ERR_INVALID_ARGUMENT;
  if (h->prm.method != HGS_ICP) return HGS_ERR_UNSUPPORTED;
  if (!h->target) return HGS_ERR_NO_TARGET;
  if (!h->source) return HGS_ERR_NO_SOURCE;
  HGS_TRY(set_device(h));
  hgs_cloud *s = h->source, *t = h->target;
  std::vector<hgs_cloud*> all{s, t};
  HGS_TRY(ensure_index(h, all));
  const int max_blocks = std::max(1, ((int)s->n_input + kTileNN - 1) / kTileNN);
  std::vector<hgs_cloud*> src{s};
  const CloudDesc* d_descs = nullptr;
  HGS_TRY(upload_descs(h, src, false, &d_descs, nullptr));
  IcpState st;
  for (int i = 0; i < 12; i++) st.x.m[i] = T12[i];
  st.mse = st.mse_prev = DBL_MAX, st.phase = ICP_RUN, st.iterations = st.passes = st.converged = 0;
  HGS_HIP(h, h->states.reserve(sizeof(IcpState)));
  HGS_HIP(h, h->partials.reserve((size_t)max_blocks * kAccIcp * sizeof(double)));
  HGS_HIP(h, hipMemcpyAsync(h->states.p, &st, sizeof(st), hipMemcpyHostToDevice, h->stream));
  launch_icp_correspond(h->stream, d_descs, target_view(t), h->states.as<IcpState>(), icp_consts(h->prm), h->partials.as<double>(), max_blocks, 1);
  HGS_HIP(h, hipGetLastError());
  std::vector<double> part((size_t)max_blocks * kAccIcp);
  int s_nvalid = 0;
  HGS_HIP(h, hipMemcpyAsync(&s_nvalid, &s->desc.meta->nvalid, sizeof(int), hipMemcpyDeviceToHost, h->stream));
  HGS_HIP(h, hipMemcpyAsync(part.data(), h->partials.p, part.size() * sizeof(double), hipMemcpyDeviceToHost, h->stream));
  const size_t s_slots = (size_t)s->P * kLeaf, t_slots = (size_t)t->P * kLeaf;
  std::vector<float4> spts, tpts;
  std::vector<int> dcorr;
  if (corr) {
    spts.resize(s_slots), tpts.resize(t_slots), dcorr.resize(s_slots);
    HGS_HIP(h, hipMemcpyAsync(spts.data(), s->desc.pts, s_slots * sizeof(float4), hipMemcpyDeviceToHost, h->stream));
    HGS_HIP(h, hipMemcpyAsync(tpts.data(), t->desc.pts, t_slots * sizeof(float4), hipMemcpyDeviceToHost, h->stream));
    HGS_HIP(h, hipMemcpyAsync(dcorr.data(), s->desc.corr, s_slots * sizeof(int), hipMemcpyDeviceToHost, h->stream));
  }
  HGS_HIP(h, hipStreamSynchronize(h->stream));
  const int ntiles = (s_nvalid + kTileNN - 1) / kTileNN;
  for (int k = 0; k < kAccIcp; k++) sums17[k] = 0.0;
  for (int tile = 0; tile < ntiles && tile < max_blocks; tile++)
    for (int k = 0; k < kAccIcp; k++) sums17[k] += part[(size_t)tile * kAccIcp + k];
  if (corr) {
    for (size_t i = 0; i < s->n_input; i++) corr[i] = -1;
    for (int i = 0; i < s_nvalid && (size_t)i < s_slots; i++) {
      int so, to = -1;
      std::memcpy(&so, &spts[i].w, 4);
      const int j = dcorr[i];
      if (j >= 0 && (size_t)j < t_slots) std::memcpy(&to, &tpts[j].w, 4);
      if (so >= 0 && (size_t)so < s->n_input) corr[so] = to;
    }
  }
  return HGS_OK;
} catch (...) {
  return status_of_current_exception(h);
}

int hgs_debug_icp_step(hgs_handle* h, const double sums17[17], const double T12_in[12], double mse_prev, int32_t iterations_in, double T12_out[12],
                       int32_t flags3[3], double* mse) try {
  ApiLock lock(h);
  if (!h || !sums17 || !T12_in || !T12_out || !flags3 || !mse) return HGS_ERR_INVALID_ARGUMENT;
  if (h->prm.method != HGS_ICP) return HGS_ERR_UNSUPPORTED;
  if (!h->source) return HGS_ERR_NO_SOURCE;
  HGS_TRY(set_device(h));
  hgs_cloud* s = h->source;
  std::vector<hgs_cloud*> src{s};
  HGS_TRY(ensure_index(h, src));
  const int max_blocks = std::max(1, ((int)s->n_input + kTileNN - 1) / kTileNN);
  const CloudDesc* d_descs = nullptr;
  HGS_TRY(upload_descs(h, src, false, &d_descs, nullptr));
  IcpState st;
  for (int i = 0; i < 12; i++) st.x.m[i] = T12_in[i];
  st.mse = DBL_MAX, st.mse_prev = mse_prev, st.phase = ICP_RUN, st.iterations = iterations_in, st.passes = 0, st.converged = 0;
  Progress prog;
  HGS_TRY(make_progress(h, 0, 1, &prog));
  HGS_HIP(h, h->states.reserve(sizeof(IcpState)));
  HGS_HIP(h, h->partials.reserve((size_t)max_blocks * kAccIcp * sizeof(double)));
  HGS_HIP(h, hipMemsetAsync(prog.dev, 0, 2 * sizeof(int), h->stream));
  HGS_HIP(h, hipMemcpyAsync(h->states.p, &st, sizeof(st), hipMemcpyHostToDevice, h->stream));
  HGS_HIP(h, hipMemsetAsync(h->partials.p, 0, (size_t)max_blocks * kAccIcp * sizeof(double), h->stream));
  HGS_HIP(h, hipMemcpyAsync(h->partials.p, sums17, kAccIcp * sizeof(double), hipMemcpyHostToDevice, h->stream));
  launch_icp_solve(h->stream, d_descs, h->states.as<IcpState>(), icp_consts(h->prm), h->partials.as<double>(), max_blocks, 1, prog);
  HGS_HIP(h, hipGetLastError());
  HGS_HIP(h, hipMemcpyAsync(&st, h->states.p, sizeof(st), hipMemcpyDeviceToHost, h->stream));
  HGS_HIP(h, hipStreamSynchronize(h->stream));
  for (int i = 0; i < 12; i++) T12_out[i] = st.x.m[i];
  flags3[0] = st.converged, flags3[1] = st.phase == ICP_DONE ? 1 : 0, flags3[2] = st.iterations;
  *mse = st.mse;
  return HGS_OK;
} catch (...) {
  return status_of_current_exception(h);
}

int hgs_debug_cloud_seed_grid(hgs_handle* h, hgs_cloud* cloud, uint32_t* tab, size_t cap, int32_t* bits, size_t* entries) try {
  ApiLock lock(h);
  if (!h || !cloud || cloud->owner != h || !entries || (cap > 0 && !tab)) return HGS_ERR_INVALID_ARGUMENT;
  *entries = 0;
  if (bits) *bits = 0;
  if (!cloud->has_seed) return HGS_OK;
  HGS_TRY(set_device(h));
  const size_t n = seed_grid_entries(cloud->seed_bits), m = std::min(cap, n);
  if (m > 0) {
    HGS_HIP(h, h->h_xform.reserve(m * sizeof(uint32_t)));
    HGS_HIP(h, hipMemcpyAsync(h->h_xform.p, cloud->seed_block.p, m * sizeof(uint32_t), hipMemcpyDeviceToHost, h->stream));
    HGS_HIP(h, hipStreamSynchronize(h->stream));
    std::memcpy(tab, h->h_xform.p, m * sizeof(uint32_t));
  }
  *entries = n;
  if (bits) *bits = cloud->seed_bits;
  return HGS_OK;
} catch (...) {
  return status_of_current_exception(h);
}

int hgs_debug_ndt_cells(hgs_handle* h, int32_t cap, int32_t* ijk3, double* mean3, float* icov6, int32_t* npts, int32_t* n_cells) try {
  ApiLock lock(h);
  if (!h || !n_cells) return HGS_ERR_INVALID_ARGUMENT;
  if (h->prm.method != HGS_NDT_OMP) return HGS_ERR_UNSUPPORTED;
  if (!h->target) return HGS_ERR_NO_TARGET;
  HGS_TRY(set_device(h));
  hgs_cloud* t = h->target;
  HGS_TRY(ensure_ndt_target(h, t));
  CloudMeta meta;
  HGS_HIP(h, hipMemcpyAsync(&meta, t->desc.meta, sizeof(CloudMeta), hipMemcpyDeviceToHost, h->stream));
  HGS_HIP(h, hipStreamSynchronize(h->stream));
  *n_cells = meta.ndt_ncells;
  const int n = std::min<int>(meta.ndt_ncells, cap);
  if (n <= 0) return HGS_OK;
  std::vector<NdtCellRec> cells(n);
  HGS_HIP(h, hipMemcpyAsync(cells.data(), t->ndt.cells, (size_t)n * sizeof(NdtCellRec), hipMemcpyDeviceToHost, h->stream));
  HGS_HIP(h, hipStreamSynchronize(h->stream));
  for (int i = 0; i < n; i++) {
    int key;
    std::memcpy(&key, &cells[i].v1.w, 4);
    if (ijk3) {
      const int m1 = meta.ndt_div_mul[1], m2 = meta.ndt_div_mul[2];
      ijk3[3 * i] = key % m1 + meta.ndt_min_b[0];
      ijk3[3 * i + 1] = (key % m2) / m1 + meta.ndt_min_b[1];
      ijk3[3 * i + 2] = key / m2 + meta.ndt_min_b[2];
    }
    if (mean3) mean3[3 * i] = cells[i].mean[0], mean3[3 * i + 1] = cells[i].mean[1], mean3[3 * i + 2] = cells[i].mean[2];
    if (icov6) {
      float* o = icov6 + 6 * i;
      o[0] = cells[i].v0.x, o[1] = cells[i].v0.y, o[2] = cells[i].v0.z, o[3] = cells[i].v0.w, o[4] = cells[i].v1.x, o[5] = cells[i].v1.y;
    }
    if (npts) npts[i] = (int)cells[i].v1.z;
  }
  return HGS_OK;
} catch (...) {
  return status_of_current_exception(h);
}

int hgs_debug_vgicp_voxels(hgs_handle* h, int32_t cap, int32_t* ijk3, double* mean3, float* cov6, int32_t* npts, int32_t* n_cells) try {
  ApiLock lock(h);
  if (!h || !n_cells) return HGS_ERR_INVALID_ARGUMENT;
  if (h->prm.method != HGS_FAST_VGICP) return HGS_ERR_UNSUPPORTED;
  if (!h->target) return HGS_ERR_NO_TARGET;
  HGS_TRY(set_device(h));
  hgs_cloud* t = h->target;
  std::vector<hgs_cloud*> all{t};
  HGS_TRY(ensure_cov(h, all, h->prm.correspondence_randomness));
  HGS_TRY(ensure_vgicp_target(h, t));
  CloudMeta meta;
  HGS_HIP(h, hipMemcpyAsync(&meta, t->desc.meta, sizeof(CloudMeta), hipMemcpyDeviceToHost, h->stream));
  HGS_HIP(h, hipStreamSynchronize(h->stream));
  *n_cells = meta.vg_ncells;
  const int n = std::min<int>(meta.vg_ncells, cap);
  if (n <= 0) return HGS_OK;
  std::vector<NdtCellRec> cells(n);
  HGS_HIP(h, hipMemcpyAsync(cells.data(), t->vg.cells, (size_t)n * sizeof(NdtCellRec), hipMemcpyDeviceToHost, h->stream));
  HGS_HIP(h, hipStreamSynchronize(h->stream));
  for (int i = 0; i < n; i++) {
    int key;
    std::memcpy(&key, &cells[i].v1.w, 4);
    if (ijk3) {
      const int m1 = meta.vg_div_mul[1], m2 = meta.vg_div_mul[2];
// ... 60 lines not shown
```

hdl_graph_slam_amd/csrc/hgs_gicp.h:

```cpp
#pragma once
#include "hgs_bvh.h"

namespace hgs {

constexpr int kAcc = 28;

struct GicpConsts {
  double max_corr2;
  float search_bound2;
  double rotation_eps, translation_eps;
  double lm_init_lambda_factor;
  int lm_max_iterations;
  int max_iterations;
  int k_correspondences;
};

HGS_HD Sym3 gicp_neighbour_cov(const double* s1, const Sym3& s2, int found, int k, double lambda) {
  const double inv_f = 1.0 / (double)found, inv_k = 1.0 / (double)k;
  const double mx = s1[0] * inv_f, my = s1[1] * inv_f, mz = s1[2] * inv_f;
  Sym3 c;
  c.xx = (s2.xx - found * mx * mx) * inv_k + lambda;
  c.xy = (s2.xy - found * mx * my) * inv_k;
  c.xz = (s2.xz - found * mx * mz) * inv_k;
  c.yy = (s2.yy - found * my * my) * inv_k + lambda;
  c.yz = (s2.yz - found * my * mz) * inv_k;
  c.zz = (s2.zz - found * mz * mz) * inv_k + lambda;
  return c;
}
HGS_HD Sym3 gicp_regularized_cov(const double* s1, const Sym3& s2, int found, int k) {
  const Sym3 c = gicp_neighbour_cov(s1, s2, found, k, 1e-3);
  const Sym3 ci = sym3_inverse(c);
  const double f = sqrt(ci.xx * ci.xx + ci.yy * ci.yy + ci.zz * ci.zz + 2.0 * (ci.xy * ci.xy + ci.xz * ci.xz + ci.yz * ci.yz));
  Sym3 o;
  o.xx = f * c.xx, o.xy = f * c.xy, o.xz = f * c.xz, o.yy = f * c.yy, o.yz = f * c.yz, o.zz = f * c.zz;
  return o;
}
HGS_HD Sym3 gicp_regularize_cov(const Sym3& c, int method) {
  if (method == 4) return c;
  const double A[9] = {c.xx, c.xy, c.xz, c.xy, c.yy, c.yz, c.xz, c.yz, c.zz};
  double w[3], V[9];
  eig_sym3(A, w, V);
  double v[3];
  if (method == 1) {
    v[0] = 1e-3, v[1] = 1.0, v[2] = 1.0;
  } else {
    const double scale = method == 3 ? w[2] : 1.0;
    for (int i = 0; i < 3; i++) {
      const double sv = fabs(w[i]) / scale;
      v[i] = sv > 1e-3 ? sv : 1e-3;
    }
  }
  Sym3 o = {0, 0, 0, 0, 0, 0};
  for (int i = 0; i < 3; i++) {
    const double x = V[0 * 3 + i], y = V[1 * 3 + i], z = V[2 * 3 + i];
    o.xx += v[i] * x * x, o.xy += v[i] * x * y, o.xz += v[i] * x * z, o.yy += v[i] * y * y, o.yz += v[i] * y * z, o.zz += v[i] * z * z;
  }
  return o;
}
HGS_HD Sym3 gicp_regularized_cov(const double* s1, const Sym3& s2, int found, int k, int method) {
  if (method == 0) return gicp_regularized_cov(s1, s2, found, k);
  return gicp_regularize_cov(gicp_neighbour_cov(s1, s2, found, k, 0.0), method);
}

HGS_HD Sym3 gicp_mahalanobis(const double* R , const Sym3& ca, const Sym3& cb) {
  Sym3 rcr = sym3_rotate(R, ca);
  rcr.xx += cb.xx, rcr.xy += cb.xy, rcr.xz += cb.xz, rcr.yy += cb.yy, rcr.yz += cb.yz, rcr.zz += cb.zz;
  return sym3_inverse(rcr);
}

struct GicpPointResidual {
  double x, y, z;
  double mex, mey, mez;
  double err;
};
HGS_HD GicpPointResidual gicp_point_residual(const Pose& T, const Sym3& M, float ax, float ay, float az, double bx, double by, double bz) {
  GicpPointResidual r;
  r.x = T.m[0] * ax + T.m[1] * ay + T.m[2] * az + T.m[3];
  r.y = T.m[4] * ax + T.m[5] * ay + T.m[6] * az + T.m[7];
  r.z = T.m[8] * ax + T.m[9] * ay + T.m[10] * az + T.m[11];
  const double ex = bx - r.x, ey = by - r.y, ez = bz - r.z;
  r.mex = M.xx * ex + M.xy * ey + M.xz * ez;
  r.mey = M.xy * ex + M.yy * ey + M.yz * ez;
  r.mez = M.xz * ex + M.yz * ey + M.zz * ez;
  r.err = ex * r.mex + ey * r.mey + ez * r.mez;
  return r;
}
HGS_HD void gicp_terms_b(const GicpPointResidual& r, double* o ) {
  o[0] = r.z * r.mey - r.y * r.mez;
  o[1] = -r.z * r.mex + r.x * r.mez;
  o[2] = r.y * r.mex - r.x * r.mey;
  o[3] = -r.mex, o[4] = -r.mey, o[5] = -r.mez;
  o[6] = r.err;
}
HGS_HD void gicp_terms_tt(const Sym3& M, double* o ) { o[0] = M.xx, o[1] = M.xy, o[2] = M.xz, o[3] = M.yy, o[4] = M.yz, o[5] = M.zz; }
HGS_HD void gicp_terms_rt(const GicpPointResidual& r, const Sym3& M, double* o ) {
  const double x = r.x, y = r.y, z = r.z;
  const double Mr[3][3] = {{M.xx, M.xy, M.xz}, {M.xy, M.yy, M.yz}, {M.xz, M.yz, M.zz}};
  for (int j = 0; j < 3; j++) {
    o[0 + j] = -(z * Mr[1][j] - y * Mr[2][j]);
    o[3 + j] = -(-z * Mr[0][j] + x * Mr[2][j]);
    o[6 + j] = -(y * Mr[0][j] - x * Mr[1][j]);
  }
}
HGS_HD void gicp_terms_rr(const GicpPointResidual& r, const Sym3& M, double* o ) {
  const double x = r.x, y = r.y, z = r.z;
  const double Mr[3][3] = {{M.xx, M.xy, M.xz}, {M.xy, M.yy, M.yz}, {M.xz, M.yz, M.zz}};
  double A[3][3];
  for (int q = 0; q < 3; q++) {
    A[q][0] = Mr[q][1] * z - Mr[q][2] * y;
    A[q][1] = -Mr[q][0] * z + Mr[q][2] * x;
    A[q][2] = Mr[q][0] * y - Mr[q][1] * x;
  }
  o[0] = z * A[1][0] - y * A[2][0], o[1] = z * A[1][1] - y * A[2][1], o[2] = z * A[1][2] - y * A[2][2];
  o[3] = -z * A[0][1] + x * A[2][1], o[4] = -z * A[0][2] + x * A[2][2];
  o[5] = y * A[0][2] - x * A[1][2];
}

HGS_HD void gicp_point_terms_by_slot(const GicpPointResidual& r, const Sym3& M, double* t ) {
  double rr[6], rt[9], tt[6], bb[7];
  gicp_terms_rr(r, M, rr), gicp_terms_rt(r, M, rt), gicp_terms_tt(M, tt), gicp_terms_b(r, bb);
  t[0] = rr[0], t[1] = rr[1], t[2] = rr[2], t[3] = rt[0], t[4] = rt[1], t[5] = rt[2];
  t[6] = rr[3], t[7] = rr[4], t[8] = rt[3], t[9] = rt[4], t[10] = rt[5];
  t[11] = rr[5], t[12] = rt[6], t[13] = rt[7], t[14] = rt[8];
  for (int k = 0; k < 6; k++) t[15 + k] = tt[k];
  for (int k = 0; k < 7; k++) t[21 + k] = bb[k];
}
template <bool WITH_JACOBIAN>
HGS_HD double gicp_point_terms(const Pose& T, const Sym3& M, float ax, float ay, float az, double bx, double by, double bz, double* acc) {
  const GicpPointResidual r = gicp_point_residual(T, M, ax, ay, az, bx, by, bz);
  if (WITH_JACOBIAN) {
    double rr[6], rt[9], tt[6], bb[7];
    gicp_terms_rr(r, M, rr), gicp_terms_rt(r, M, rt), gicp_terms_tt(M, tt), gicp_terms_b(r, bb);
    acc[0] += rr[0], acc[1] += rr[1], acc[2] += rr[2], acc[3] += rt[0], acc[4] += rt[1], acc[5] += rt[2];
    acc[6] += rr[3], acc[7] += rr[4], acc[8] += rt[3], acc[9] += rt[4], acc[10] += rt[5];
    acc[11] += rr[5], acc[12] += rt[6], acc[13] += rt[7], acc[14] += rt[8];
    for (int k = 0; k < 6; k++) acc[15 + k] += tt[k];
    for (int k = 0; k < 6; k++) acc[21 + k] += bb[k];
  }
  return r.err;
}

HGS_HD Sym3 sym3_from_floats(float xx, float xy, float xz, float yy, float yz, float zz) {
  Sym3 s;
  s.xx = xx, s.xy = xy, s.xz = xz, s.yy = yy, s.yz = yz, s.zz = zz;
  return s;
}

enum GicpPhase { GICP_LINEARIZE = 0, GICP_TRY = 1, GICP_DONE = 2 };

struct GicpState {
  Pose x0;
  Pose xi;
  double H[36];
  double b[6];
  double d[6];
  double y0, yi;
  double lambda, nu;
  int phase;
  int iterations;
  int lm_try;
  int lm_tries_total;
  int converged;
  int pad;
};

HGS_HD void gicp_state_init(GicpState& s, const float* guess_colmajor) {
  s.x0 = pose_from_colmajor_f(guess_colmajor);
  s.xi = s.x0;
// ... 113 lines not shown
```

hdl_graph_slam_amd/csrc/hgs_icp.h:

```cpp
#pragma once
#include "hgs_math.h"

namespace hgs {

constexpr int kAccIcp = 17;

struct IcpConsts {
  double max_corr2;
  float search_bound2;
  int max_iterations;
  double trans_eps;
  double rot_thr;
  int reciprocal;
  int pad;
};

enum IcpPhase { ICP_RUN = 0, ICP_DONE = 2 };

struct IcpState {
  Pose x;
  double mse;
  double mse_prev;
  int phase;
  int iterations;
  int passes;
  int converged;
};

HGS_HD void icp_state_init(IcpState& s, const float* guess_colmajor) {
  s.x = pose_from_colmajor_f(guess_colmajor);
  s.mse = DBL_MAX, s.mse_prev = DBL_MAX;
  s.phase = ICP_RUN;
  s.iterations = 0, s.passes = 0, s.converged = 0;
}

HGS_HD F3 icp_move_point(const Pose& T, float ax, float ay, float az) {
  HGS_FP_STRICT
  const double x = (double)ax, y = (double)ay, z = (double)az;
  F3 q;
  q.x = (float)(((T.m[0] * x + T.m[1] * y) + T.m[2] * z) + T.m[3]);
  q.y = (float)(((T.m[4] * x + T.m[5] * y) + T.m[6] * z) + T.m[7]);
  q.z = (float)(((T.m[8] * x + T.m[9] * y) + T.m[10] * z) + T.m[11]);
  return q;
}
HGS_HD F3 icp_unmove_point(const Pose& T, float qx, float qy, float qz) {
  HGS_FP_STRICT
  const double x = (double)qx - T.m[3], y = (double)qy - T.m[7], z = (double)qz - T.m[11];
  F3 p;
  p.x = (float)((T.m[0] * x + T.m[4] * y) + T.m[8] * z);
  p.y = (float)((T.m[1] * x + T.m[5] * y) + T.m[9] * z);
  p.z = (float)((T.m[2] * x + T.m[6] * y) + T.m[10] * z);
  return p;
}

HGS_HD void icp_pair_terms(const F3& p, float qx, float qy, float qz, float d2, double* t ) {
  const double px = p.x, py = p.y, pz = p.z, tx = qx, ty = qy, tz = qz;
  t[0] = 1.0;
  t[1] = px, t[2] = py, t[3] = pz;
  t[4] = tx, t[5] = ty, t[6] = tz;
  t[7] = tx * px, t[8] = tx * py, t[9] = tx * pz;
  t[10] = ty * px, t[11] = ty * py, t[12] = ty * pz;
  t[13] = tz * px, t[14] = tz * py, t[15] = tz * pz;
  t[16] = (double)d2;
}

HGS_HD void svd3(const double* A, double* U, double* s, double* V) {
  HGS_FP_STRICT
  double B[9];
  for (int i = 0; i < 9; i++) B[i] = A[i], V[i] = (i % 4 == 0) ? 1.0 : 0.0;
  for (int sweep = 0; sweep < 32; sweep++) {
    bool rotated = false;
    for (int pair = 0; pair < 3; pair++) {
      const int p = pair == 2 ? 1 : 0, q = pair == 0 ? 1 : 2;
      double alpha = 0, beta = 0, gamma = 0;
      for (int k = 0; k < 3; k++) {
        alpha += B[k * 3 + p] * B[k * 3 + p];
        beta += B[k * 3 + q] * B[k * 3 + q];
        gamma += B[k * 3 + p] * B[k * 3 + q];
      }
      if (gamma == 0.0 || fabs(gamma) <= DBL_EPSILON * sqrt(alpha * beta)) continue;
      const double zeta = (beta - alpha) / (2.0 * gamma);
      const double t = (zeta >= 0 ? 1.0 : -1.0) / (fabs(zeta) + sqrt(1.0 + zeta * zeta));
      const double c = 1.0 / sqrt(1.0 + t * t), sn = c * t;
      for (int k = 0; k < 3; k++) {
        const double bp = B[k * 3 + p], bq = B[k * 3 + q], vp = V[k * 3 + p], vq = V[k * 3 + q];
        B[k * 3 + p] = c * bp - sn * bq, B[k * 3 + q] = sn * bp + c * bq;
        V[k * 3 + p] = c * vp - sn * vq, V[k * 3 + q] = sn * vp + c * vq;
      }
      rotated = true;
    }
    if (!rotated) break;
  }
  int order[3] = {0, 1, 2};
  double nrm[3];
  for (int j = 0; j < 3; j++) nrm[j] = sqrt(B[j] * B[j] + B[3 + j] * B[3 + j] + B[6 + j] * B[6 + j]);
  for (int i = 0; i < 2; i++)
    for (int j = 0; j < 2 - i; j++)
      if (nrm[order[j]] < nrm[order[j + 1]]) {
        const int o = order[j];
        order[j] = order[j + 1], order[j + 1] = o;
      }
  double Vs[9];
  for (int j = 0; j < 3; j++) {
    const int o = order[j];
    s[j] = nrm[o];
    for (int k = 0; k < 3; k++) Vs[k * 3 + j] = V[k * 3 + o], U[k * 3 + j] = s[j] > 0.0 ? B[k * 3 + o] / s[j] : 0.0;
  }
  for (int i = 0; i < 9; i++) V[i] = Vs[i];
  const double tiny = s[0] * 1e-13;
  if (!(s[0] > 0.0)) {
    for (int i = 0; i < 9; i++) U[i] = (i % 4 == 0) ? 1.0 : 0.0;
    return;
  }
  if (!(s[1] > tiny)) {
    const double ax = fabs(U[0]), ay = fabs(U[3]), az = fabs(U[6]);
    const double e[3] = {ax <= ay && ax <= az ? 1.0 : 0.0, ay < ax && ay <= az ? 1.0 : 0.0, az < ax && az < ay ? 1.0 : 0.0};
    double w[3] = {U[3] * e[2] - U[6] * e[1], U[6] * e[0] - U[0] * e[2], U[0] * e[1] - U[3] * e[0]};
    const double wn = sqrt(w[0] * w[0] + w[1] * w[1] + w[2] * w[2]);
    for (int k = 0; k < 3; k++) U[k * 3 + 1] = w[k] / wn;
  }
  if (!(s[2] > tiny)) {
    U[2] = U[3] * U[7] - U[6] * U[4];
    U[5] = U[6] * U[1] - U[0] * U[7];
    U[8] = U[0] * U[4] - U[3] * U[1];
  }
}

HGS_HD double det3(const double* M) {
  return M[0] * (M[4] * M[8] - M[5] * M[7]) - M[1] * (M[3] * M[8] - M[5] * M[6]) + M[2] * (M[3] * M[7] - M[4] * M[6]);
}

HGS_HD void icp_umeyama(const double* acc, Pose& delta) {
  HGS_FP_STRICT
  const double inv = 1.0 / acc[0];
  const double mp[3] = {acc[1] * inv, acc[2] * inv, acc[3] * inv}, mq[3] = {acc[4] * inv, acc[5] * inv, acc[6] * inv};
  double S[9], U[9], sv[3], V[9];
  for (int r = 0; r < 3; r++)
    for (int c = 0; c < 3; c++) S[r * 3 + c] = acc[7 + r * 3 + c] * inv - mq[r] * mp[c];
  svd3(S, U, sv, V);
  const double d = det3(U) * det3(V) < 0.0 ? -1.0 : 1.0;
  for (int r = 0; r < 3; r++) {
    for (int c = 0; c < 3; c++) delta.m[r * 4 + c] = (U[r * 3 + 0] * V[c * 3 + 0] + U[r * 3 + 1] * V[c * 3 + 1]) + d * U[r * 3 + 2] * V[c * 3 + 2];
  }
  for (int r = 0; r < 3; r++) delta.m[r * 4 + 3] = mq[r] - ((delta.m[r * 4 + 0] * mp[0] + delta.m[r * 4 + 1] * mp[1]) + delta.m[r * 4 + 2] * mp[2]);
}

HGS_HD void icp_after_pass(IcpState& s, const double* acc, const IcpConsts& c) {
  HGS_FP_STRICT
  s.passes++;
  if (!(acc[0] >= 3.0)) {
    s.converged = 0;
    s.phase = ICP_DONE;
    return;
  }
  const double mse = acc[16] / acc[0];
  Pose delta;
  icp_umeyama(acc, delta);
  s.x = pose_mul(delta, s.x);
  s.iterations++;
  s.mse = mse;
  bool done = s.iterations >= c.max_iterations;
  if (!done) {
    const double cos_angle = 0.5 * (delta.m[0] + delta.m[5] + delta.m[10] - 1.0);
    const double t2 = delta.m[3] * delta.m[3] + delta.m[7] * delta.m[7] + delta.m[11] * delta.m[11];
    done = cos_angle >= c.rot_thr && t2 <= c.trans_eps;
  }
  if (!done) done = fabs(mse - s.mse_prev) < 1e-12;
// ... 10 lines not shown
```

hdl_graph_slam_amd/csrc/hgs_kernels.hip:

```cpp
#include <hip/hip_runtime.h>
#include <type_traits>
#include "../../include/hgs_registration.h"
#include "hgs_device.h"
#include "hgs_wave_bvh.h"

namespace hgs {

#ifndef HGS_OPAQUE_POINTER
#define HGS_OPAQUE_POINTER(p) asm volatile("" : "+v"(p))
#define HGS_WAIT_VMEM() asm volatile("s_waitcnt vmcnt(0)" ::: "memory")
#define HGS_LANE_ID(dst) asm volatile("v_mbcnt_lo_u32_b32 %0, -1, 0\n\tv_mbcnt_hi_u32_b32 %0, -1, %0" : "=v"(dst))
#endif
#ifndef HGS_COMPILER_MEMORY_BARRIER
#define HGS_COMPILER_MEMORY_BARRIER() asm volatile("" ::: "memory")
#endif
#ifndef HGS_LOAD_GLOBAL_XYZ
__device__ __forceinline__ float4 hgs_load_global_xyz(const float4* p) {
  const __attribute__((address_space(1))) float* g = (const __attribute__((address_space(1))) float*)(p);
  return make_float4(g[0], g[1], g[2], 0.f);
}
#define HGS_LOAD_GLOBAL_XYZ(p) hgs_load_global_xyz(p)
#define HGS_OPAQUE_OFFSET(off) asm volatile("" : "+v"(off))
#define HGS_WAIT_VMEM_TRACKED() __builtin_amdgcn_s_waitcnt(0x0F70)
#endif
// ... 598 lines not shown
  else if (gather == 1) launch_knn_cov_t<REG, 1>(s, descs, ncloud, max_n, k, qpw, reg_method, raw, raw_stride);
  else launch_knn_cov_t<REG, 0>(s, descs, ncloud, max_n, k, qpw, reg_method, raw, raw_stride);
}
void launch_knn_cov(hipStream_t s, const CloudDesc* descs, int ncloud, int max_n, int k, int qpw, int reg_method, int gather, double* raw_stage) {
  if (max_n <= 0) return;
  if (reg_method == 0) {
    launch_knn_cov_g<0>(s, descs, ncloud, max_n, k, qpw, reg_method, gather, nullptr, 0);
  } else if (raw_stage) {
    launch_knn_cov_g<2>(s, descs, ncloud, max_n, k, qpw, reg_method, gather, raw_stage, max_n);
    hipLaunchKernelGGL(k_cov_regularize, dim3((max_n + kBlock - 1) / kBlock, ncloud), dim3(kBlock), 0, s, descs, raw_stage, max_n, reg_method);
  } else {
    launch_knn_cov_g<1>(s, descs, ncloud, max_n, k, qpw, reg_method, gather, nullptr, 0);
  }
}

__global__ void k_gicp_init(GicpState* states, const float* guesses, int B, Progress prog) {
  const int b = blockIdx.x * blockDim.x + threadIdx.x;
  if (b == 0) prog.dev[0] = 0, prog.dev[1] = 0;
  if (b >= B) return;
  gicp_state_init(states[b], guesses + 16 * b);
}
void launch_gicp_init(hipStream_t s, GicpState* states, const float* guesses, int B, Progress prog) {
  hipLaunchKernelGGL(k_gicp_init, dim3((B + 63) / 64), dim3(64), 0, s, states, guesses, B, prog);
}
__global__ void k_gicp_init1(GicpState* states, Guess16 guess, Progress prog) {
  if (threadIdx.x != 0) return;
  prog.dev[0] = 0, prog.dev[1] = 0;
  gicp_state_init(states[0], guess.m);
}
void launch_gicp_init1(hipStream_t s, GicpState* states, const float* guess_host, Progress prog) {
  Guess16 g;
  for (int i = 0; i < 16; i++) g.m[i] = guess_host[i];
  hipLaunchKernelGGL(k_gicp_init1, dim3(1), dim3(64), 0, s, states, g, prog);
}

__device__ __forceinline__ Sym3 load_cov(const float4* cov, int i) {
  const float4 a = cov[2 * i], b = cov[2 * i + 1];
  return sym3_from_floats(a.x, a.y, a.z, a.w, b.x, b.y);
}
__device__ __forceinline__ float4 load_stream(const float4* p) {
  typedef float v4 __attribute__((ext_vector_type(4)));
  const v4 v = __builtin_nontemporal_load(reinterpret_cast<const v4*>(p));
  return make_float4(v.x, v.y, v.z, v.w);
}
__device__ __forceinline__ Sym3 load_cov_stream(const float4* cov, int i) {
  const float4 a = load_stream(cov + 2 * i), b = load_stream(cov + 2 * i + 1);
  return sym3_from_floats(a.x, a.y, a.z, a.w, b.x, b.y);
}

template <int N>
__device__ __forceinline__ void last_wave_stores(const double* lds , unsigned* arrivals, double* out, int lane) {
  unsigned ticket = 0;
  if (lane == 0) ticket = __hip_atomic_fetch_add(arrivals, 1u, __ATOMIC_ACQ_REL, __HIP_MEMORY_SCOPE_WORKGROUP);
  ticket = (unsigned)__builtin_amdgcn_readlane((int)ticket, 0);
  if (ticket == kBlock / 64 - 1 && lane < N) out[lane] = (lds[lane] + lds[N + lane]) + (lds[2 * N + lane] + lds[3 * N + lane]);
}

#ifndef HGS_SEED_INV0
#define HGS_SEED_INV0 4.0f
#endif
constexpr float kSeedInv0 = HGS_SEED_INV0;
__device__ __forceinline__ unsigned seed_hash(int cx, int cy, int cz) {
  unsigned h = (unsigned)cx * 73856093u ^ (unsigned)cy * 19349663u ^ (unsigned)cz * 83492791u;
  h ^= h >> 15;
  h *= 0x2c1b3c6du;
  h ^= h >> 12;
  return h;
}
__device__ __forceinline__ void seed_cells(float x, float y, float z, int& cx, int& cy, int& cz) {
  cx = (int)floorf(fminf(fmaxf(x * kSeedInv0, -1.0e9f), 1.0e9f));
  cy = (int)floorf(fminf(fmaxf(y * kSeedInv0, -1.0e9f), 1.0e9f));
  cz = (int)floorf(fminf(fmaxf(z * kSeedInv0, -1.0e9f), 1.0e9f));
}
__device__ __forceinline__ void seed_slots(int cx, int cy, int cz, int bits, unsigned& s0, unsigned& s1, unsigned& s2) {
  const unsigned n0 = 1u << bits, n1 = n0 >> 2, n2 = n0 >> 4;
  s0 = seed_hash(cx, cy, cz) & (n0 - 1u);
  s1 = n0 + (seed_hash(cx >> 2, cy >> 2, cz >> 2) & (n1 - 1u));
  s2 = n0 + n1 + (seed_hash(cx >> 4, cy >> 4, cz >> 4) & (n2 - 1u));
}
__global__ __launch_bounds__(kBlock) void k_seed_grid_build(const float4* __restrict__ pts, const CloudMeta* meta, unsigned* __restrict__ tab, int bits) {
  const int i = blockIdx.x * kBlock + threadIdx.x;
  if (i >= meta->nvalid) return;
  const float4 p = pts[i];
  int cx, cy, cz;
  seed_cells(p.x, p.y, p.z, cx, cy, cz);
  unsigned s0, s1, s2;
  seed_slots(cx, cy, cz, bits, s0, s1, s2);
  atomicMin(tab + s0, (unsigned)i);
  atomicMin(tab + s1, (unsigned)i);
  atomicMin(tab + s2, (unsigned)i);
}
void launch_seed_grid_build(hipStream_t s, const float4* pts, const CloudMeta* meta, int n_max, unsigned* tab, int bits) {
  if (n_max <= 0) return;
  hipLaunchKernelGGL(k_seed_grid_build, dim3((n_max + kBlock - 1) / kBlock), dim3(kBlock), 0, s, pts, meta, tab, bits);
}
__device__ __forceinline__ SeedGridJob seed_grid_job(const SeedGridJob* __restrict__ jobs, int j) {
  SeedGridJob job = global_pointer(jobs)[j];
  job.pts = global_pointer(job.pts), job.meta = global_pointer(job.meta), job.tab = global_pointer_rw(job.tab);
  return job;
}
__global__ __launch_bounds__(kBlock) void k_seed_grid_clear_batch(const SeedGridJob* __restrict__ jobs) {
  const SeedGridJob job = seed_grid_job(jobs, blockIdx.y);
  const unsigned entries = (1u << job.bits) + (1u << (job.bits - 2)) + (1u << (job.bits - 4));
  const unsigned first = blockIdx.x * kBlock;
  if (first >= entries) return;
  const unsigned step = gridDim.x * kBlock;
  for (unsigned i = first + threadIdx.x; i < entries; i += step) job.tab[i] = 0xffffffffu;
}
__global__ __launch_bounds__(kBlock) void k_seed_grid_build_batch(const SeedGridJob* __restrict__ jobs) {
  const SeedGridJob job = seed_grid_job(jobs, blockIdx.y);
  const int n = job.meta->nvalid;
  const int first = blockIdx.x * kBlock;
  if (first >= n) return;
  const int step = gridDim.x * kBlock;
  for (int i = first + (int)threadIdx.x; i < n; i += step) {
    const float4 p = job.pts[i];
    int cx, cy, cz;
    seed_cells(p.x, p.y, p.z, cx, cy, cz);
    unsigned s0, s1, s2;
    seed_slots(cx, cy, cz, job.bits, s0, s1, s2);
    atomicMin(job.tab + s0, (unsigned)i);
    atomicMin(job.tab + s1, (unsigned)i);
    atomicMin(job.tab + s2, (unsigned)i);
  }
}
void launch_seed_grid_build_batch(hipStream_t s, const SeedGridJob* jobs, int njobs, size_t max_entries, int max_n) {
  if (njobs <= 0) return;
  const unsigned clear_x = (unsigned)std::min<size_t>(1024, std::max<size_t>(1, (max_entries + (size_t)kBlock * 8 - 1) / ((size_t)kBlock * 8)));
  hipLaunchKernelGGL(k_seed_grid_clear_batch, dim3(clear_x, njobs), dim3(kBlock), 0, s, jobs);
  const unsigned build_x = (unsigned)std::min(4096, std::max(1, (max_n + kBlock - 1) / kBlock));
  hipLaunchKernelGGL(k_seed_grid_build_batch, dim3(build_x, njobs), dim3(kBlock), 0, s, jobs);
}
__device__ __forceinline__ int seed_grid_lookup(const TargetView& t, const F3& q) {
  int cx, cy, cz;
  seed_cells(q.x, q.y, q.z, cx, cy, cz);
  unsigned s0, s1, s2;
  seed_slots(cx, cy, cz, t.seed_bits, s0, s1, s2);
  const unsigned e0 = t.seed_tab[s0], e1 = t.seed_tab[s1], e2 = t.seed_tab[s2];
  const unsigned n = (unsigned)t.meta->nvalid;
  int best = -1;
  float best_d = FLT_MAX;
  const unsigned e[3] = {e0, e1, e2};
#pragma unroll
  for (int l = 0; l < 3; l++) {
    if (e[l] < n) {
      const float4 p = t.pts[e[l]];
      const float d = dist2f(q, p.x, p.y, p.z);
      if (d < best_d) best_d = d, best = (int)e[l];
    }
  }
  return best;
}

__device__ __forceinline__ void packet_nn1(const BvhView& tv, float* park, const F3& q, bool active, float bound2, int seed, int qpw, float& d2, int& pos, int& orig) {
  const bool seeded = seed >= 0 && seed < tv.n;
  int leaf;
  bool tie, found;
  if (__ballot(active && !seeded) != 0ull) wave_nn1_quad<true, true>(tv, park, q, active, bound2, seed, qpw >> 1, d2, leaf, tie, found);
  else wave_nn1_quad<false, true>(tv, park, q, active, bound2, seed, qpw >> 1, d2, leaf, tie, found);
  if (__ballot(tie) != 0ull) {
    const F3 qa[1] = {q};
    const bool aa[1] = {active};
    const int sa[1] = {seed};
    float da[1];
    int pa[1], oa[1];
    wave_nn1<1>(tv, park, qa, aa, bound2, sa, da, pa, oa, qpw);
    d2 = da[0], pos = pa[0], orig = oa[0];
  } else {
    nn1_resolve_leaf(tv, q, found ? leaf : -1, d2, pos, orig);
  }
}

__device__ __forceinline__ DevResult gicp_result_of(const GicpState& st) {
  DevResult r;
  pose_to_colmajor_f(st.x0, r.T);
  r.converged = st.converged, r.iterations = st.iterations, r.lm_tries = st.lm_tries_total, r.pad = 0;
  r.error = st.y0;
  r.fit_sum = 0, r.fit_count = 0, r.pad2 = 0;
  return r;
}
__device__ __forceinline__ void gicp_early_result(DevResult* mapped, const DevResult& r) {
  static_assert(sizeof(DevResult) % 8 == 0, "stored as 64-bit words");
  const unsigned long long* w = reinterpret_cast<const unsigned long long*>(&r);
  unsigned long long* o = reinterpret_cast<unsigned long long*>(mapped);
#pragma unroll
  for (int k = 0; k < (int)(sizeof(DevResult) / 8); k++) __hip_atomic_store(o + k, w[k], __ATOMIC_RELAXED, __HIP_MEMORY_SCOPE_SYSTEM);
}
__device__ __forceinline__ void gicp_state_load(GicpState& st, const GicpState* src) {
  static_assert(sizeof(GicpState) % sizeof(double) == 0 && sizeof(GicpState) / sizeof(double) <= kBlock, "state copied one double per thread");
  if (threadIdx.x < sizeof(GicpState) / sizeof(double)) reinterpret_cast<double*>(&st)[threadIdx.x] = reinterpret_cast<const double*>(src)[threadIdx.x];
}
__device__ __forceinline__ void gicp_state_store(GicpState* dst, const GicpState& st) {
  if (threadIdx.x < sizeof(GicpState) / sizeof(double)) reinterpret_cast<double*>(dst)[threadIdx.x] = reinterpret_cast<const double*>(&st)[threadIdx.x];
}

__device__ __forceinline__ void gicp_wave_row(const GicpPointResidual& r, const Sym3& M, double* row, int lane) {
  double even[14], odd[14];
  {
    double t[kAcc];
    gicp_point_terms_by_slot(r, M, t);
#pragma unroll
    for (int j = 0; j < 14; j++) even[j] = t[2 * j];
  }
  __builtin_amdgcn_sched_barrier(0);
  {
    double t[kAcc];
    gicp_point_terms_by_slot(r, M, t);
#pragma unroll
    for (int j = 0; j < 14; j++) odd[j] = t[2 * j + 1];
  }
  wave_sums28_to(even, odd, row, lane);
}

template <bool ROUND2, bool SHORT = false, typename TGT = TargetView>
__global__ __launch_bounds__(kBlock) __attribute__((amdgpu_waves_per_eu(ROUND2 ? 4 : HGS_LINEARIZE_WAVES))) void k_gicp_linearize(const CloudDesc* descs, TGT tgt_arg, const GicpState* states, GicpConsts c,
                                                           double* __restrict__ partials, int max_blocks, int qpw, GicpState* states_out,
                                                           const double* __restrict__ partials_err, Progress prog, DevResult* results, DevResult* early_out) {
  const int b = blockIdx.y;
  const TargetView& tgt = problem_target(tgt_arg, b);
  __shared__ GicpState st2;
  __shared__ double ws2[kGicpControlWorkspace];
  if constexpr (!ROUND2) {
    if (states[b].phase != GICP_LINEARIZE) return;
  }
  const CloudDesc d = descs[b];
  const int n = d.meta->nvalid;
  if constexpr (ROUND2) {
    const int phase_in = states[b].phase;
    gicp_state_load(st2, states + b);
    double s = 0;
    if (phase_in == GICP_TRY && threadIdx.x < 64) {
      const int ntiles_err = (n + kBlock - 1) / kBlock;
      const double* pe = partials_err + (size_t)b * max_blocks;
      for (int t = threadIdx.x; t < ntiles_err; t += 64) s += pe[t];
      s = wave_sum(s);
    }
    __syncthreads();
    if (phase_in == GICP_TRY && threadIdx.x == 0) gicp_after_error(st2, s, c, ws2);
    __syncthreads();
    if (blockIdx.x == 0) {
      gicp_state_store(states_out + b, st2);
      if (threadIdx.x == 0) {
        const bool finished_now = phase_in == GICP_TRY && st2.phase == GICP_DONE;
        if (finished_now && early_out) {
          const DevResult r = gicp_result_of(st2);
          results[b] = r;
          gicp_early_result(early_out + b, r);
        }
        progress_tick(prog, finished_now, early_out != nullptr);
      }
    }
    if (st2.phase != GICP_LINEARIZE) return;
  }
  const int tile_pts = (kBlock / 64) * qpw * kNW;
  const int ntiles = (n + tile_pts - 1) / tile_pts;
  const int tile = xcd_tile(blockIdx.x, ntiles);
  if (tile >= ntiles) return;
  __shared__ double lds[4 * kAcc];
  __shared__ unsigned arrivals;
  __shared__ __attribute__((aligned(512))) float park[kBlock / 64][kParkFloats];
  if (threadIdx.x == 0) arrivals = 0u;
  __syncthreads();
  const int wave = __builtin_amdgcn_readfirstlane((int)(threadIdx.x >> 6));
  const Pose T = ROUND2 ? st2.x0 : states[b].x0;
  float Tf[12];
  pose_to_float(T, Tf);
  static_assert(kNW == 1, "one packet of 64 consecutive source points per wave");
  const int idx = tile * tile_pts + wave * qpw + (int)(threadIdx.x & 63);
  const bool active = (int)(threadIdx.x & 63) < qpw && idx < n;
  const float4 a = active ? load_stream(d.pts + idx) : make_float4(0.f, 0.f, 0.f, 0.f);
  const F3 q = transform_point_f(Tf, a.x, a.y, a.z);
  const int seed = active ? __builtin_nontemporal_load(d.corr + idx) : -1;
  float d2;
  int j, orig;
  packet_nn1(view_of(tgt), park[wave], q, active, c.search_bound2, seed, qpw, d2, j, orig);
  const double R[9] = {T.m[0], T.m[1], T.m[2], T.m[4], T.m[5], T.m[6], T.m[8], T.m[9], T.m[10]};
  int jj = active ? j : -1;
  if (jj >= 0 && !((double)d2 < c.max_corr2)) jj = -1;
  if (active) __builtin_nontemporal_store(jj, d.corr + idx);
  if constexpr (SHORT) {
    static_assert(ROUND2, "the short-packet form belongs to the two-launch rounds");
    {
      __shared__ int chunk_corr[kBlock];
      int lane;
      HGS_LANE_ID(lane);
      if (lane < qpw) chunk_corr[wave * qpw + lane] = jj;
      unsigned ticket = 0;
      if (lane == 0) ticket = __hip_atomic_fetch_add(&arrivals, 1u, __ATOMIC_ACQ_REL, __HIP_MEMORY_SCOPE_WORKGROUP);
      ticket = (unsigned)__builtin_amdgcn_readlane((int)ticket, 0);
      if (ticket != kBlock / 64 - 1) return;
      const int chunks = tile_pts / 64;
      for (int ch = 0; ch < chunks; ch++) {
        const int i2 = tile * tile_pts + ch * 64 + lane;
        if (tile * tile_pts + ch * 64 >= n) break;
        const int j2 = i2 < n ? chunk_corr[ch * 64 + lane] : -1;
        Sym3 M2 = {0.0, 0.0, 0.0, 0.0, 0.0, 0.0};
        GicpPointResidual r2 = {0.0, 0.0, 0.0, 0.0, 0.0, 0.0, 0.0};
        if (j2 >= 0) {
          const float4 a2 = load_stream(d.pts + i2);
          M2 = gicp_mahalanobis(R, load_cov_stream(d.cov, i2), load_cov(tgt.cov, j2));
          const float4 bp = tgt.pts[j2];
          r2 = gicp_point_residual(T, M2, a2.x, a2.y, a2.z, bp.x, bp.y, bp.z);
        }
        gicp_wave_row(r2, M2, lds, lane);
        __builtin_amdgcn_wave_barrier();
        if (lane < kAcc) partials[((size_t)b * max_blocks + (size_t)tile * chunks + ch) * kAcc + lane] = lds[lane];
        __builtin_amdgcn_wave_barrier();
      }
      return;
    }
  } else {
  Sym3 M = {0.0, 0.0, 0.0, 0.0, 0.0, 0.0};
  GicpPointResidual r = {0.0, 0.0, 0.0, 0.0, 0.0, 0.0, 0.0};
  if (jj >= 0) {
    M = gicp_mahalanobis(R, load_cov_stream(d.cov, idx), load_cov(tgt.cov, jj));
    const float4 bp = tgt.pts[jj];
    r = gicp_point_residual(T, M, a.x, a.y, a.z, bp.x, bp.y, bp.z);
  }
  int lane;
  HGS_LANE_ID(lane);
  double* row = lds + wave * kAcc;
  gicp_wave_row(r, M, row, lane);
  last_wave_stores<kAcc>(lds, &arrivals, partials + ((size_t)b * max_blocks + tile) * kAcc, lane);
  }
}
void launch_gicp_linearize(hipStream_t s, const CloudDesc* descs, TargetView tgt, const GicpState* states, GicpConsts c, double* partials,
                           int max_blocks, int B, int qpw) {
  hipLaunchKernelGGL(k_gicp_linearize<false>, dim3(HGS_GRID_X(max_blocks), B), dim3(kBlock), 0, s, descs, tgt, states, c, partials, max_blocks, qpw, (GicpState*)nullptr,
                     (const double*)nullptr, Progress{}, (DevResult*)nullptr, (DevResult*)nullptr);
}
void launch_gicp_linearize_round2(hipStream_t s, const CloudDesc* descs, TargetView tgt, const GicpState* states_in, GicpState* states_out, GicpConsts c, double* partials,
                                  const double* partials_err, int max_blocks, int lin_blocks, int B, int qpw, Progress prog, DevResult* results, DevResult* early_out) {
  if (qpw < 64)
    hipLaunchKernelGGL((k_gicp_linearize<true, true>), dim3(HGS_GRID_X(lin_blocks), B), dim3(kBlock), 0, s, descs, tgt, states_in, c, partials, max_blocks, qpw, states_out, partials_err, prog, results, early_out);
  else
    hipLaunchKernelGGL((k_gicp_linearize<true, false>), dim3(HGS_GRID_X(lin_blocks), B), dim3(kBlock), 0, s, descs, tgt, states_in, c, partials, max_blocks, qpw, states_out, partials_err, prog, results, early_out);
}
void launch_gicp_linearize(hipStream_t s, const CloudDesc* descs, const TargetView* tviews, const GicpState* states, GicpConsts c, double* partials,
                           int max_blocks, int B, int qpw) {
  hipLaunchKernelGGL((k_gicp_linearize<false, false, const TargetView*>), dim3(HGS_GRID_X(max_blocks), B), dim3(kBlock), 0, s, descs, tviews, states, c, partials, max_blocks, qpw,
                     (GicpState*)nullptr, (const double*)nullptr, Progress{}, (DevResult*)nullptr, (DevResult*)nullptr);
}
void launch_gicp_linearize_round2(hipStream_t s, const CloudDesc* descs, const TargetView* tviews, const GicpState* states_in, GicpState* states_out, GicpConsts c, double* partials,
                                  const double* partials_err, int max_blocks, int lin_blocks, int B, int qpw, Progress prog, DevResult* results, DevResult* early_out) {
  if (qpw < 64)
    hipLaunchKernelGGL((k_gicp_linearize<true, true, const TargetView*>), dim3(HGS_GRID_X(lin_blocks), B), dim3(kBlock), 0, s, descs, tviews, states_in, c, partials, max_blocks, qpw, states_out, partials_err, prog, results, early_out);
  else
    hipLaunchKernelGGL((k_gicp_linearize<true, false, const TargetView*>), dim3(HGS_GRID_X(lin_blocks), B), dim3(kBlock), 0, s, descs, tviews, states_in, c, partials, max_blocks, qpw, states_out, partials_err, prog, results, early_out);
}

__device__ __forceinline__ void gicp_solve_block(int ntiles, GicpState* state, const GicpConsts& c, const double* __restrict__ problem_partials, int nchunks = 0) {
  __shared__ double acc[kAcc];
  __shared__ double scratch[kSolveBlock];
  __shared__ GicpState st;
  __shared__ double ws[kGicpControlWorkspace];
  static_assert(sizeof(GicpState) % sizeof(double) == 0 && sizeof(GicpState) / sizeof(double) <= kSolveBlock, "state copied one double per thread");
  if (threadIdx.x < sizeof(GicpState) / sizeof(double)) reinterpret_cast<double*>(&st)[threadIdx.x] = reinterpret_cast<const double*>(state)[threadIdx.x];
  reduce_tiles<kAcc>(problem_partials, ntiles, acc, scratch, nchunks);
  if (threadIdx.x == 0) gicp_after_linearize(st, acc, c, ws);
  __syncthreads();
  if (threadIdx.x < sizeof(GicpState) / sizeof(double)) reinterpret_cast<double*>(state)[threadIdx.x] = reinterpret_cast<const double*>(&st)[threadIdx.x];
}
__global__ __launch_bounds__(kSolveBlock) __attribute__((amdgpu_waves_per_eu(HGS_CONTROL_WAVES))) void k_gicp_solve(const CloudDesc* descs, GicpState* states, GicpConsts c, const double* __restrict__ partials,
                                                      int max_blocks, int tile_points) {
  const int b = blockIdx.x;
  if (states[b].phase != GICP_LINEARIZE) return;
  if (HGS_CONTROL_PRIO) __builtin_amdgcn_s_setprio(HGS_CONTROL_PRIO);
  const int n = descs[b].meta->nvalid;
  const bool chunked = tile_points < kBlock;
  const int ntiles = chunked ? (n + kBlock - 1) / kBlock : (n + tile_points - 1) / tile_points;
  gicp_solve_block(ntiles, states + b, c, partials + (size_t)b * max_blocks * kAcc, chunked ? (n + 63) / 64 : 0);
}
void launch_gicp_solve(hipStream_t s, const CloudDesc* descs, GicpState* states, GicpConsts c, const double* partials, int max_blocks, int B,
                       int tile_points) {
  hipLaunchKernelGGL(k_gicp_solve, dim3(B), dim3(kSolveBlock), 0, s, descs, states, c, partials, max_blocks, tile_points);
}

template <bool ROUND2, typename TGT = TargetView>
__global__ __launch_bounds__(kBlock) void k_gicp_error(const CloudDesc* descs, TGT tgt_arg, const GicpState* states, double* __restrict__ partials_err,
                                                       int max_blocks, GicpConsts c, GicpState* states_out, const double* __restrict__ partials, int lin_tile_points) {
  const int b = blockIdx.y;
  const TargetView& tgt = problem_target(tgt_arg, b);
  __shared__ GicpState st2;
  __shared__ double ws2[kGicpControlWorkspace];
  __shared__ double acc2[kAcc];
  __shared__ double scratch2[kSolveBlock];
  if constexpr (!ROUND2) {
    if (states[b].phase != GICP_TRY) return;
  }
  const CloudDesc d = descs[b];
  const int n = d.meta->nvalid;
  if constexpr (ROUND2) {
    static_assert(kSolveBlock == kBlock, "reduce_tiles runs on the point kernel's block");
    const int phase_in = states[b].phase;
    gicp_state_load(st2, states + b);
    if (phase_in == GICP_LINEARIZE) {
      const bool chunked = lin_tile_points < kBlock;
      const int ntiles_lin = chunked ? (n + kBlock - 1) / kBlock : (n + lin_tile_points - 1) / lin_tile_points;
      reduce_tiles<kAcc>(partials + (size_t)b * max_blocks * kAcc, ntiles_lin, acc2, scratch2, chunked ? (n + 63) / 64 : 0);
      if (threadIdx.x == 0) gicp_after_linearize(st2, acc2, c, ws2);
    }
    __syncthreads();
    if (blockIdx.x == 0) gicp_state_store(states_out + b, st2);
    if (st2.phase != GICP_TRY) return;
  }
  const int ntiles = (n + kBlock - 1) / kBlock;
  if ((int)blockIdx.x >= ntiles) return;
  const int tile = (int)blockIdx.x;
  const int i = tile * kBlock + threadIdx.x;
  __shared__ double lds[4];
  double err = 0.0;
  if (i < n) {
    const int j = d.corr[i];
    if (j >= 0) {
      const Pose T0 = ROUND2 ? st2.x0 : states[b].x0;
      const Pose Ti = ROUND2 ? st2.xi : states[b].xi;
      const double R[9] = {T0.m[0], T0.m[1], T0.m[2], T0.m[4], T0.m[5], T0.m[6], T0.m[8], T0.m[9], T0.m[10]};
      const Sym3 M = gicp_mahalanobis(R, load_cov(d.cov, i), load_cov(tgt.cov, j));
      const float4 a = d.pts[i], bp = tgt.pts[j];
      err = gicp_point_terms<false>(Ti, M, a.x, a.y, a.z, bp.x, bp.y, bp.z, nullptr);
    }
  }
  block_reduce_store<1>(&err, partials_err + (size_t)b * max_blocks + tile, lds);
}
void launch_gicp_error(hipStream_t s, const CloudDesc* descs, TargetView tgt, const GicpState* states, double* partials_err, int max_blocks, int B) {
  hipLaunchKernelGGL(k_gicp_error<false>, dim3(max_blocks, B), dim3(kBlock), 0, s, descs, tgt, states, partials_err, max_blocks, GicpConsts{}, (GicpState*)nullptr, (const double*)nullptr, 0);
}
void launch_gicp_error_round2(hipStream_t s, const CloudDesc* descs, TargetView tgt, const GicpState* states_in, GicpState* states_out, GicpConsts c, const double* partials,
                              double* partials_err, int max_blocks, int err_blocks, int B, int lin_tile_points) {
  hipLaunchKernelGGL(k_gicp_error<true>, dim3(err_blocks, B), dim3(kBlock), 0, s, descs, tgt, states_in, partials_err, max_blocks, c, states_out, partials, lin_tile_points);
}
void launch_gicp_error(hipStream_t s, const CloudDesc* descs, const TargetView* tviews, const GicpState* states, double* partials_err, int max_blocks, int B) {
  hipLaunchKernelGGL((k_gicp_error<false, const TargetView*>), dim3(max_blocks, B), dim3(kBlock), 0, s, descs, tviews, states, partials_err, max_blocks, GicpConsts{}, (GicpState*)nullptr,
                     (const double*)nullptr, 0);
}
void launch_gicp_error_round2(hipStream_t s, const CloudDesc* descs, const TargetView* tviews, const GicpState* states_in, GicpState* states_out, GicpConsts c, const double* partials,
                              double* partials_err, int max_blocks, int err_blocks, int B, int lin_tile_points) {
  hipLaunchKernelGGL((k_gicp_error<true, const TargetView*>), dim3(err_blocks, B), dim3(kBlock), 0, s, descs, tviews, states_in, partials_err, max_blocks, c, states_out, partials, lin_tile_points);
}

__device__ __forceinline__ bool gicp_decide_wave(int ntiles, GicpState* state, const GicpConsts& c, const double* __restrict__ problem_partials_err) {
  __shared__ GicpState st;
  __shared__ double ws[kGicpControlWorkspace];
  bool finished_now = false;
  double s = 0;
  if (threadIdx.x < 64) {
    for (int k = threadIdx.x; k < (int)(sizeof(GicpState) / sizeof(double)); k += 64) reinterpret_cast<double*>(&st)[k] = reinterpret_cast<const double*>(state)[k];
    for (int t = threadIdx.x; t < ntiles; t += 64) s += problem_partials_err[t];
    s = wave_sum(s);
  }
  __syncthreads();
  if (threadIdx.x == 0) {
    gicp_after_error(st, s, c, ws);
    finished_now = st.phase == GICP_DONE;
  }
  __syncthreads();
  if (threadIdx.x < 64)
    for (int k = threadIdx.x; k < (int)(sizeof(GicpState) / sizeof(double)); k += 64) reinterpret_cast<double*>(state)[k] = reinterpret_cast<const double*>(&st)[k];
  return finished_now;
}
__global__ __launch_bounds__(64) __attribute__((amdgpu_waves_per_eu(HGS_CONTROL_WAVES))) void k_gicp_decide(const CloudDesc* descs, GicpState* states, GicpConsts c, const double* __restrict__ partials_err,
                                                   int max_blocks, Progress prog) {
  const int b = blockIdx.x;
  bool finished_now = false;
  if (HGS_CONTROL_PRIO) __builtin_amdgcn_s_setprio(HGS_CONTROL_PRIO);
  if (states[b].phase == GICP_TRY) {
    const int ntiles = (descs[b].meta->nvalid + kBlock - 1) / kBlock;
    finished_now = gicp_decide_wave(ntiles, states + b, c, partials_err + (size_t)b * max_blocks);
  }
  if (threadIdx.x == 0) progress_tick(prog, finished_now);
}
void launch_gicp_decide(hipStream_t s, const CloudDesc* descs, GicpState* states, GicpConsts c, const double* partials_err, int max_blocks, int B,
                        Progress prog) {
  hipLaunchKernelGGL(k_gicp_decide, dim3(B), dim3(64), 0, s, descs, states, c, partials_err, max_blocks, prog);
}

__global__ void k_gicp_results(const GicpState* states, DevResult* out, int B) {
  const int b = blockIdx.x * blockDim.x + threadIdx.x;
  if (b >= B) return;
  out[b] = gicp_result_of(states[b]);
}
void launch_gicp_results(hipStream_t s, const GicpState* states, DevResult* out, int B) {
  hipLaunchKernelGGL(k_gicp_results, dim3((B + 63) / 64), dim3(64), 0, s, states, out, B);
}

__global__ void k_icp_init(IcpState* states, const float* guesses, int B, Progress prog) {
  const int b = blockIdx.x * blockDim.x + threadIdx.x;
  if (b == 0) prog.dev[0] = 0, prog.dev[1] = 0;
  if (b >= B) return;
  icp_state_init(states[b], guesses + 16 * b);
}
void launch_icp_init(hipStream_t s, IcpState* states, const float* guesses, int B, Progress prog) {
  hipLaunchKernelGGL(k_icp_init, dim3((B + 63) / 64), dim3(64), 0, s, states, guesses, B, prog);
}

template <bool RECIPROCAL, typename TGT = TargetView>
__global__ __launch_bounds__(kBlock) __attribute__((amdgpu_waves_per_eu(HGS_LINEARIZE_WAVES))) void k_icp_correspond(const CloudDesc* descs, TGT tgt_arg, const IcpState* states,
                                                                                                       IcpConsts c, double* __restrict__ partials, int max_blocks) {
  const int b = blockIdx.y;
  const TargetView& tgt = problem_target(tgt_arg, b);
  if (states[b].phase != ICP_RUN) return;
  const CloudDesc d = descs[b];
  const int n = d.meta->nvalid;
  constexpr int qpw = 64;
  const int ntiles = (n + kTileNN - 1) / kTileNN;
  const int tile = xcd_tile(blockIdx.x, ntiles);
  if (tile >= ntiles) return;
  __shared__ double lds[4 * kAccIcp];
  __shared__ unsigned arrivals;
  __shared__ __attribute__((aligned(512))) float park[kBlock / 64][kParkFloats];
  if (threadIdx.x == 0) arrivals = 0u;
  __syncthreads();
  const int wave = __builtin_amdgcn_readfirstlane((int)(threadIdx.x >> 6));
  const Pose T = states[b].x;
  static_assert(kNW == 1 && kTileNN == (kBlock / 64) * qpw, "one packet of 64 consecutive source points per wave");
  const int idx = tile * kTileNN + wave * qpw + (int)(threadIdx.x & 63);
  const bool active = idx < n;
  const float4 a = active ? load_stream(d.pts + idx) : make_float4(0.f, 0.f, 0.f, 0.f);
  const F3 q = icp_move_point(T, a.x, a.y, a.z);
  const int seed = active ? __builtin_nontemporal_load(d.corr + idx) : -1;
  float d2;
  int j, orig;
  packet_nn1(view_of(tgt), park[wave], q, active, c.search_bound2, seed, qpw, d2, j, orig);
  int jj = active ? j : -1;
  if (jj >= 0 && !((double)d2 <= c.max_corr2)) jj = -1;
  const float4 bp = jj >= 0 ? tgt.pts[jj] : make_float4(0.f, 0.f, 0.f, 0.f);
  if constexpr (RECIPROCAL) {
    const bool ractive = jj >= 0;
    if (__ballot(ractive) != 0ull) {
      const F3 r = icp_unmove_point(T, bp.x, bp.y, bp.z);
      BvhView sv;
      sv.nodes = d.nodes, sv.pts = d.pts, sv.lpts = d.lpts, sv.P = d.P, sv.n = n;
      float rd2;
      int rj, rorig;
      packet_nn1(sv, park[wave], r, ractive, c.search_bound2, ractive ? idx : -1, qpw, rd2, rj, rorig);
      if (ractive && !(rj >= 0 && rorig == __float_as_int(a.w) && (double)rd2 <= c.max_corr2)) jj = -1;
    }
  }
  if (active) __builtin_nontemporal_store(jj, d.corr + idx);
  double acc[kAccIcp];
  if (jj >= 0) {
    icp_pair_terms(q, bp.x, bp.y, bp.z, d2, acc);
  } else {
#pragma unroll
    for (int k = 0; k < kAccIcp; k++) acc[k] = 0.0;
  }
  int lane;
  HGS_LANE_ID(lane);
  int slot[kAccIcp];
#pragma unroll
  for (int k = 0; k < kAccIcp; k++) slot[k] = k;
  wave_sums_to<kAccIcp>(acc, slot, lds + wave * kAccIcp, lane);
  last_wave_stores<kAccIcp>(lds, &arrivals, partials + ((size_t)b * max_blocks + tile) * kAccIcp, lane);
}
void launch_icp_correspond(hipStream_t s, const CloudDesc* descs, TargetView tgt, const IcpState* states, IcpConsts c, double* partials, int max_blocks, int B) {
  if (c.reciprocal) hipLaunchKernelGGL(k_icp_correspond<true>, dim3(HGS_GRID_X(max_blocks), B), dim3(kBlock), 0, s, descs, tgt, states, c, partials, max_blocks);
  else hipLaunchKernelGGL(k_icp_correspond<false>, dim3(HGS_GRID_X(max_blocks), B), dim3(kBlock), 0, s, descs, tgt, states, c, partials, max_blocks);
}
void launch_icp_correspond(hipStream_t s, const CloudDesc* descs, const TargetView* tviews, const IcpState* states, IcpConsts c, double* partials, int max_blocks, int B) {
  if (c.reciprocal) hipLaunchKernelGGL((k_icp_correspond<true, const TargetView*>), dim3(HGS_GRID_X(max_blocks), B), dim3(kBlock), 0, s, descs, tviews, states, c, partials, max_blocks);
  else hipLaunchKernelGGL((k_icp_correspond<false, const TargetView*>), dim3(HGS_GRID_X(max_blocks), B), dim3(kBlock), 0, s, descs, tviews, states, c, partials, max_blocks);
}

__global__ __launch_bounds__(64) __attribute__((amdgpu_waves_per_eu(HGS_CONTROL_WAVES))) void k_icp_solve(const CloudDesc* descs, IcpState* states, IcpConsts c,
                                                                                        const double* __restrict__ partials, int max_blocks, Progress prog) {
  const int b = blockIdx.x;
  bool finished_now = false;
  if (HGS_CONTROL_PRIO) __builtin_amdgcn_s_setprio(HGS_CONTROL_PRIO);
  if (states[b].phase == ICP_RUN) {
    const int ntiles = (descs[b].meta->nvalid + kTileNN - 1) / kTileNN;
    const double* p = partials + (size_t)b * max_blocks * kAccIcp;
    double s[kAccIcp];
#pragma unroll
    for (int k = 0; k < kAccIcp; k++) s[k] = 0.0;
    for (int t = threadIdx.x; t < ntiles; t += 64)
#pragma unroll
      for (int k = 0; k < kAccIcp; k++) s[k] += p[(size_t)t * kAccIcp + k];
#pragma unroll
    for (int k = 0; k < kAccIcp; k++) s[k] = wave_sum(s[k]);
    if (threadIdx.x == 0) {
      IcpState st = states[b];
      icp_after_pass(st, s, c);
      states[b] = st;
      finished_now = st.phase == ICP_DONE;
    }
  }
  if (threadIdx.x == 0) progress_tick(prog, finished_now);
}
void launch_icp_solve(hipStream_t s, const CloudDesc* descs, IcpState* states, IcpConsts c, const double* partials, int max_blocks, int B, Progress prog) {
  hipLaunchKernelGGL(k_icp_solve, dim3(B), dim3(64), 0, s, descs, states, c, partials, max_blocks, prog);
}

__global__ void k_icp_results(const IcpState* states, DevResult* out, int B) {
  const int b = blockIdx.x * blockDim.x + threadIdx.x;
  if (b >= B) return;
  const IcpState st = states[b];
  DevResult r;
  pose_to_colmajor_f(st.x, r.T);
  r.converged = st.converged, r.iterations = st.iterations, r.lm_tries = st.passes, r.pad = 0;
  r.error = st.mse;
  r.fit_sum = 0, r.fit_count = 0, r.pad2 = 0;
  out[b] = r;
}
void launch_icp_results(hipStream_t s, const IcpState* states, DevResult* out, int B) {
  hipLaunchKernelGGL(k_icp_results, dim3((B + 63) / 64), dim3(64), 0, s, states, out, B);
}

template <typename TGT = TargetView>
__global__ __launch_bounds__(kBlock) __attribute__((amdgpu_waves_per_eu(HGS_FITNESS_WAVES))) void k_fitness(const CloudDesc* descs, TGT tgt_arg, const DevResult* poses, double max_range,
                                                    double* __restrict__ partials, int max_blocks, int use_seed, int qpw) {
  const int b = blockIdx.y;
  const TargetView& tgt = problem_target(tgt_arg, b);
  const CloudDesc d = descs[b];
  const int n = d.meta->nvalid;
  const int tile_pts = (kBlock / 64) * qpw * kNW;
  const int ntiles = (n + tile_pts - 1) / tile_pts;
  const int tile = xcd_tile(blockIdx.x, ntiles);
  if (tile >= ntiles) return;
  __shared__ double lds[4 * 2];
  __shared__ unsigned arrivals;
  __shared__ __attribute__((aligned(512))) float park[kBlock / 64][kParkFloats];
  if (threadIdx.x == 0) arrivals = 0u;
  __syncthreads();
  const int wave = __builtin_amdgcn_readfirstlane((int)(threadIdx.x >> 6));
  float Tf[12];
  const float* Tc = poses[b].T;
#pragma unroll
  for (int r = 0; r < 3; r++)
#pragma unroll
    for (int cc = 0; cc < 4; cc++) Tf[r * 4 + cc] = Tc[cc * 4 + r];
  const int idx = tile * tile_pts + wave * qpw + (int)(threadIdx.x & 63);
  const bool active = (int)(threadIdx.x & 63) < qpw && idx < n;
  const float4 a = active ? load_stream(d.pts + idx) : make_float4(0.f, 0.f, 0.f, 0.f);
  const F3 q = transform_point_f(Tf, a.x, a.y, a.z);
  int seed = (active && use_seed) ? __builtin_nontemporal_load(d.corr + idx) : -1;
  const BvhView tv = view_of(tgt);
  if (tgt.seed_bits && __ballot(active && !(seed >= 0 && seed < tv.n)) != 0ull) {
    if (active && !(seed >= 0 && seed < tv.n)) seed = seed_grid_lookup(tgt, q);
  }
  const bool seeded = seed >= 0 && seed < tv.n;
  float d2;
  int leaf;
  bool tie, found;
  if (__ballot(active && !seeded) != 0ull) wave_nn1_quad<true, false>(tv, park[wave], q, active, FLT_MAX, seed, qpw >> 1, d2, leaf, tie, found);
  else wave_nn1_quad<false, false>(tv, park[wave], q, active, FLT_MAX, seed, qpw >> 1, d2, leaf, tie, found);
  double acc[2] = {0.0, 0.0};
  if (active && found && (double)d2 <= max_range) acc[0] = (double)d2, acc[1] = 1.0;
  int lane;
  HGS_LANE_ID(lane);
  {
    const int slot[2] = {0, 1};
    wave_sums_to<2>(acc, slot, lds + wave * 2, lane);
  }
  last_wave_stores<2>(lds, &arrivals, partials + ((size_t)b * max_blocks + tile) * 2, lane);
}
void launch_fitness(hipStream_t s, const CloudDesc* descs, TargetView tgt, const DevResult* poses, double max_range, double* partials, int max_blocks,
                    int B, int use_seed, int qpw) {
  hipLaunchKernelGGL(k_fitness<TargetView>, dim3(HGS_GRID_X(max_blocks), B), dim3(kBlock), 0, s, descs, tgt, poses, max_range, partials, max_blocks, use_seed, qpw);
}
void launch_fitness(hipStream_t s, const CloudDesc* descs, const TargetView* tviews, const DevResult* poses, double max_range, double* partials, int max_blocks,
                    int B, int use_seed, int qpw) {
  hipLaunchKernelGGL(k_fitness<const TargetView*>, dim3(HGS_GRID_X(max_blocks), B), dim3(kBlock), 0, s, descs, tviews, poses, max_range, partials, max_blocks, use_seed, qpw);
}
__global__ __launch_bounds__(64) void k_fitness_final(const CloudDesc* descs, const double* __restrict__ partials, int max_blocks, DevResult* out, int tile_pts) {
  const int b = blockIdx.x;
  const int ntiles = (descs[b].meta->nvalid + tile_pts - 1) / tile_pts;
  double s = 0, c = 0;
  for (int t = threadIdx.x; t < ntiles; t += 64) {
    s += partials[((size_t)b * max_blocks + t) * 2];
    c += partials[((size_t)b * max_blocks + t) * 2 + 1];
  }
  s = wave_sum(s), c = wave_sum(c);
  if (threadIdx.x == 0) out[b].fit_sum = s, out[b].fit_count = (unsigned)(c + 0.5);
}
void launch_fitness_final(hipStream_t s, const CloudDesc* descs, const double* partials, int max_blocks, DevResult* out, int B, int tile_pts) {
  hipLaunchKernelGGL(k_fitness_final, dim3(B), dim3(64), 0, s, descs, partials, max_blocks, out, tile_pts);
}

__global__ void k_results_to_records(const DevResult* __restrict__ res, const int* __restrict__ candidate_ids, int n, int n_slots, hgs_result* __restrict__ out) {
  const int s = blockIdx.x * blockDim.x + threadIdx.x;
  if (s >= n_slots) return;
  hgs_result r;
  if (s < n) {
    const DevResult d = res[s];
#pragma unroll
    for (int k = 0; k < 16; k++) r.final_transformation[k] = d.T[k];
    r.converged = d.converged, r.iterations = d.iterations;
    r.error = d.error;
    r.num_inliers = d.fit_count;
    r.fitness_score = d.fit_count > 0 ? d.fit_sum / (double)d.fit_count : DBL_MAX;
    r.candidate_id = candidate_ids[s];
    r.lm_tries = d.lm_tries, r.reserved = 0;
  } else {
#pragma unroll
    for (int k = 0; k < 16; k++) r.final_transformation[k] = 0.f;
    r.converged = 0, r.iterations = 0, r.error = 0.0, r.fitness_score = DBL_MAX, r.num_inliers = 0, r.candidate_id = -1, r.lm_tries = 0, r.reserved = 0;
  }
  out[s] = r;
}
void launch_results_to_records(hipStream_t s, const DevResult* res, const int* candidate_ids, int n, int n_slots, hgs_result* out) {
  if (n_slots <= 0) return;
  hipLaunchKernelGGL(k_results_to_records, dim3((n_slots + 63) / 64), dim3(64), 0, s, res, candidate_ids, n, n_slots, out);
}

__global__ __launch_bounds__(kBlock) void k_nn_query(TargetView tgt, const float4* __restrict__ q, int nq, int* __restrict__ idx, float* __restrict__ d2out) {
  const int i = blockIdx.x * kBlock + threadIdx.x;
  if (i >= nq) return;
  const float4 p = q[i];
  float d2;
  int orig;
  const int j = bvh_nn1(view_of(tgt), F3{p.x, p.y, p.z}, FLT_MAX, &d2, &orig);
  idx[i] = j >= 0 ? orig : -1;
  d2out[i] = d2;
}
void launch_nn_query(hipStream_t s, TargetView tgt, const float4* q, int nq, int* idx, float* d2) {
  if (nq <= 0) return;
  hipLaunchKernelGGL(k_nn_query, dim3((nq + kBlock - 1) / kBlock), dim3(kBlock), 0, s, tgt, q, nq, idx, d2);
}

__global__ __launch_bounds__(kBlock) void k_transform(const float4* __restrict__ raw, int n, const float* __restrict__ T16, float4* __restrict__ out) {
  const int i = blockIdx.x * kBlock + threadIdx.x;
  if (i >= n) return;
  float Tf[12];
#pragma unroll
  for (int r = 0; r < 3; r++)
#pragma unroll
    for (int cc = 0; cc < 4; cc++) Tf[r * 4 + cc] = T16[cc * 4 + r];
  const float4 a = raw[i];
  const F3 q = transform_point_f(Tf, a.x, a.y, a.z);
  out[i] = make_float4(q.x, q.y, q.z, 1.0f);
}
void launch_transform(hipStream_t s, const float4* raw, int n, const float* T16_dev, float4* out) {
  if (n <= 0) return;
  hipLaunchKernelGGL(k_transform, dim3((n + kBlock - 1) / kBlock), dim3(kBlock), 0, s, raw, n, T16_dev, out);
}

__global__ void k_ndt_grid_params(CloudDesc d, float inv_leaf) {
  CloudMeta* m = d.meta;
  m->ndt_ncells = 0;
  m->ndt_error = 0;
  if (m->nvalid <= 0) {
    for (int k = 0; k < 3; k++) m->ndt_min_b[k] = 0, m->ndt_max_b[k] = -1, m->ndt_div_mul[k] = 0;
    return;
  }
  long long div[3];
  for (int k = 0; k < 3; k++) {
    m->ndt_min_b[k] = (int)floorf(ord2f(m->bbmin[k]) * inv_leaf);
    m->ndt_max_b[k] = (int)floorf(ord2f(m->bbmax[k]) * inv_leaf);
    div[k] = (long long)m->ndt_max_b[k] - m->ndt_min_b[k] + 1;
  }
  if (div[0] * div[1] * div[2] > 2147483647LL) m->ndt_error = 1;
  m->ndt_div_mul[0] = 1, m->ndt_div_mul[1] = (int)div[0], m->ndt_div_mul[2] = (int)(div[0] * div[1]);
}
void launch_ndt_grid_params(hipStream_t s, CloudDesc desc, float inv_leaf) { hipLaunchKernelGGL(k_ndt_grid_params, dim3(1), dim3(1), 0, s, desc, inv_leaf); }

__global__ __launch_bounds__(kBlock) void k_ndt_cell_keys(CloudDesc d, float inv_leaf, unsigned long long* __restrict__ keys, unsigned* __restrict__ vals) {
  const int i = blockIdx.x * kBlock + threadIdx.x;
  if (i >= d.n_input) return;
  const float4 p = d.raw[i];
  unsigned long long key = 0xffffffffull;
  const CloudMeta* m = d.meta;
  if (finite3(p) && !m->ndt_error) {
    const int cx = (int)floorf(p.x * inv_leaf) - m->ndt_min_b[0];
    const int cy = (int)floorf(p.y * inv_leaf) - m->ndt_min_b[1];
    const int cz = (int)floorf(p.z * inv_leaf) - m->ndt_min_b[2];
    key = (unsigned long long)(unsigned)(cx * m->ndt_div_mul[0] + cy * m->ndt_div_mul[1] + cz * m->ndt_div_mul[2]);
  }
  keys[i] = key;
  vals[i] = (unsigned)i;
}
void launch_ndt_cell_keys(hipStream_t s, CloudDesc desc, float inv_leaf, unsigned long long* keys, unsigned* vals) {
  if (desc.n_input <= 0) return;
  hipLaunchKernelGGL(k_ndt_cell_keys, dim3((desc.n_input + kBlock - 1) / kBlock), dim3(kBlock), 0, s, desc, inv_leaf, keys, vals);
}

__global__ __launch_bounds__(kBlock) void k_ndt_build_cells(CloudDesc d, const unsigned long long* __restrict__ keys, const unsigned* __restrict__ vals,
                                                            int min_points, int* hash_keys, int* hash_vals, int hash_mask, NdtCellRec* cells) {
  const int i = blockIdx.x * kBlock + threadIdx.x;
  if (i >= d.n_input) return;
  const unsigned long long key = keys[i];
  if (key == 0xffffffffull) return;
  if (i > 0 && keys[i - 1] == key) return;
  double sum[3] = {0, 0, 0};
  Sym3 sq = {0, 0, 0, 0, 0, 0};
  int n = 0;
  for (int j = i; j < d.n_input && keys[j] == key; j++) {
    const float4 p = d.raw[vals[j]];
    const double x = p.x, y = p.y, z = p.z;
    sum[0] += x, sum[1] += y, sum[2] += z;
    sq.xx += x * x, sq.xy += x * y, sq.xz += x * z, sq.yy += y * y, sq.yz += y * z, sq.zz += z * z;
    n++;
  }
  double mean[3];
  Sym3 icov;
  if (!ndt_finalize_cell(n, sum, sq, min_points, mean, &icov)) return;
  const int slot_c = atomicAdd(&d.meta->ndt_ncells, 1);
  NdtCellRec rec;
  rec.v0 = make_float4((float)icov.xx, (float)icov.xy, (float)icov.xz, (float)icov.yy);
  rec.v1 = make_float4((float)icov.yz, (float)icov.zz, (float)n, __int_as_float((int)key));
  rec.mean[0] = mean[0], rec.mean[1] = mean[1], rec.mean[2] = mean[2], rec.pad = 0.0;
  cells[slot_c] = rec;
  unsigned slot = (ndt_hash((int)key) >> 7) & (unsigned)hash_mask;
  for (;;) {
    const int prev = atomicCAS(&hash_keys[slot], -1, (int)key);
    if (prev == -1) {
      hash_vals[slot] = slot_c;
      break;
    }
    slot = (slot + 1) & (unsigned)hash_mask;
  }
}
void launch_ndt_build_cells(hipStream_t s, CloudDesc desc, const unsigned long long* sorted_keys, const unsigned* sorted_vals, int min_points,
                            int* hash_keys, int* hash_vals, int hash_mask, NdtCellRec* cells) {
  if (desc.n_input <= 0) return;
  hipLaunchKernelGGL(k_ndt_build_cells, dim3((desc.n_input + kBlock - 1) / kBlock), dim3(kBlock), 0, s, desc, sorted_keys, sorted_vals, min_points,
                     hash_keys, hash_vals, hash_mask, cells);
}

__global__ __launch_bounds__(64) void k_ndt_init(NdtState* states, NdtAngles* angles, const float* guesses, NdtConsts c, int B, Progress prog, NdtAccum* accum) {
  const int b = blockIdx.x;
  if (b == 0 && threadIdx.x == 0) prog.dev[0] = 0, prog.dev[1] = 0;
  if (accum) {
    static_assert(sizeof(NdtAccum) % sizeof(unsigned long long) == 0, "NdtAccum is zeroed word by word");
    unsigned long long* w = reinterpret_cast<unsigned long long*>(accum + b);
    for (int k = threadIdx.x; k < (int)(sizeof(NdtAccum) / sizeof(unsigned long long)); k += 64) w[k] = 0ull;
  }
  if (threadIdx.x == 0) {
    ndt_state_init(states[b], guesses + 16 * b);
    ndt_angle_tables(states[b].p, c.upstream_hd1_sign, angles[b]);
// ... 1610 lines not shown
```

Measured before the change: 5952 registrations/sec.

## Add early per-problem fitness scoring, neighbour seed borrowing, and majority-ordered NN option

In the fitness kernel, unseeded lanes borrow the nearest seeded lane's seed within the wave so their NN search starts close. An opt-in mode scores fitness for problems as soon as the decide kernel marks them done, overlapping scoring with other lanes' iterations via host-visible flags and events. Another opt-in flag uses the ordered traversal only when most lanes lack seeds. The changes add LDS shuffles and extra launch and sync logic, and borrowed seeds could occasionally be poor starting points.

```diff
diff --git a/hdl_graph_slam_amd/csrc/hgs_consts.h b/hdl_graph_slam_amd/csrc/hgs_consts.h
--- a/hdl_graph_slam_amd/csrc/hgs_consts.h
+++ b/hdl_graph_slam_amd/csrc/hgs_consts.h
@@ -22,6 +22,7 @@
   c.lm_max_iterations = p.lm_max_iterations;
   c.max_iterations = p.max_iterations;
   c.k_correspondences = p.correspondence_randomness;
+  c.nn_flags = 0;
   return c;
 }
 
@@ -42,7 +43,7 @@
   c.trans_eps = p.transformation_epsilon;
   c.rot_thr = p.rotation_epsilon > 0 ? p.rotation_epsilon : 1.0 - p.transformation_epsilon;
   c.reciprocal = p.icp_reciprocal ? 1 : 0;
-  c.pad = 0;
+  c.nn_flags = 0;
   return c;
 }
 
diff --git a/hdl_graph_slam_amd/csrc/hgs_device.h b/hdl_graph_slam_amd/csrc/hgs_device.h
--- a/hdl_graph_slam_amd/csrc/hgs_device.h
+++ b/hdl_graph_slam_amd/csrc/hgs_device.h
@@ -80,6 +80,7 @@
   int pad;
 };
 
+constexpr int kFitnessCorrSeeds = 1, kFitnessBorrowSeeds = 2;
 constexpr int kFusedRoundMaxProblems = 4;
 constexpr int kBlock = 256;
 constexpr int kKnnLaneList = 16;
@@ -112,8 +113,9 @@
                                   DevResult* results, DevResult* early_out );
 void launch_gicp_error_round2(hipStream_t s, const CloudDesc* descs, TargetView tgt, const GicpState* states_in, GicpState* states_out, GicpConsts c, const double* partials,
                               double* partials_err, int max_blocks, int err_blocks , int B, int lin_tile_points);
-void launch_gicp_decide(hipStream_t s, const CloudDesc* descs, GicpState* states, GicpConsts c, const double* partials_err, int max_blocks, int B, Progress prog);
-void launch_gicp_results(hipStream_t s, const GicpState* states, DevResult* out, int B);
+void launch_gicp_decide(hipStream_t s, const CloudDesc* descs, GicpState* states, GicpConsts c, const double* partials_err, int max_blocks, int B, Progress prog,
+                        DevResult* results = nullptr , int* host_finished = nullptr );
+void launch_gicp_results(hipStream_t s, const GicpState* states, DevResult* out, int B, int unfinished_only = 0);
 
 void launch_icp_init(hipStream_t s, IcpState* states, const float* guesses, int B, Progress prog);
 void launch_icp_correspond(hipStream_t s, const CloudDesc* descs, TargetView tgt, const IcpState* states, IcpConsts c, double* partials, int max_blocks, int B);
@@ -121,8 +123,8 @@
 void launch_icp_results(hipStream_t s, const IcpState* states, DevResult* out, int B);
 
 void launch_fitness(hipStream_t s, const CloudDesc* descs, TargetView tgt, const DevResult* poses, double max_range, double* partials, int max_blocks, int B,
-                    int use_seed, int qpw);
-void launch_fitness_final(hipStream_t s, const CloudDesc* descs, const double* partials, int max_blocks, DevResult* out, int B, int tile_pts);
+                    int use_seed , int qpw, unsigned long long skip = 0ull );
+void launch_fitness_final(hipStream_t s, const CloudDesc* descs, const double* partials, int max_blocks, DevResult* out, int B, int tile_pts, unsigned long long skip = 0ull);
 void launch_gicp_linearize(hipStream_t s, const CloudDesc* descs, const TargetView* tviews, const GicpState* states, GicpConsts c, double* partials, int max_blocks, int B,
                            int qpw);
 void launch_gicp_error(hipStream_t s, const CloudDesc* descs, const TargetView* tviews, const GicpState* states, double* partials_err, int max_blocks, int B);
@@ -132,7 +134,7 @@
                               double* partials_err, int max_blocks, int err_blocks, int B, int lin_tile_points);
 void launch_icp_correspond(hipStream_t s, const CloudDesc* descs, const TargetView* tviews, const IcpState* states, IcpConsts c, double* partials, int max_blocks, int B);
 void launch_fitness(hipStream_t s, const CloudDesc* descs, const TargetView* tviews, const DevResult* poses, double max_range, double* partials, int max_blocks, int B,
-                    int use_seed, int qpw);
+                    int use_seed, int qpw, unsigned long long skip = 0ull);
 }
 struct hgs_result;
 namespace hgs {
diff --git a/hdl_graph_slam_amd/csrc/hgs_engine.hip b/hdl_graph_slam_amd/csrc/hgs_engine.hip
--- a/hdl_graph_slam_amd/csrc/hgs_engine.hip
+++ b/hdl_graph_slam_amd/csrc/hgs_engine.hip
@@ -109,6 +109,12 @@
   int knn_tiny_below = 32768;
   int seed_grid = 1;
   int knn_replay = -1;
+  int fitness_borrow_seeds = 1;
+  int early_fitness = 0;
+  int ordered_majority = 0;
+  PinnedBuffer h_finished;
+  DeviceBuffer fit_partials;
+  hipEvent_t score_event[8] = {};
   int batch_lanes = 0;
   std::string err;
   hgs_cloud* target = nullptr;
@@ -665,6 +671,17 @@
   return c;
 }
 
+GicpConsts engine_gicp_consts(const hgs_handle* h) {
+  GicpConsts c = gicp_consts(h->prm);
+  c.nn_flags = h->ordered_majority ? kNnOrderedMajority : 0;
+  return c;
+}
+IcpConsts engine_icp_consts(const hgs_handle* h) {
+  IcpConsts c = icp_consts(h->prm);
+  c.nn_flags = h->ordered_majority ? kNnOrderedMajority : 0;
+  return c;
+}
+
 constexpr int kMaxCountedDevices = 64;
 std::atomic<int> g_streams_in_use[kMaxCountedDevices] = {};
 std::atomic<int>& streams_in_use(int device) { return g_streams_in_use[(unsigned)device % kMaxCountedDevices]; }
@@ -830,11 +847,12 @@
 }
 
 bool corr_seeds_fitness(int method) { return method == HGS_FAST_GICP || method == HGS_ICP; }
+int fitness_seed_flags(const hgs_handle* h, bool corr_seeds) { return (corr_seeds ? kFitnessCorrSeeds : 0) | (h->fitness_borrow_seeds ? kFitnessBorrowSeeds : 0); }
 void lane_fitness(hgs_handle* h, BatchLane& L, const BatchShape& s, double max_range, bool corr_seeds) {
   StageTimer tm(h, HGS_STAGE_FITNESS);
   DevResult* res = h->results.as<DevResult>() + L.b0;
   with_lane_target(s, L, s.d_tviews ? TargetView{} : target_view(h->target),
-                   [&](auto tgt) { launch_fitness(L.stream, s.d_descs + L.b0, tgt, res, max_range, L.partials_err, s.max_blocks, L.B, corr_seeds ? 1 : 0, s.qpw); });
+                   [&](auto tgt) { launch_fitness(L.stream, s.d_descs + L.b0, tgt, res, max_range, L.partials_err, s.max_blocks, L.B, fitness_seed_flags(h, corr_seeds), s.qpw); });
   launch_fitness_final(L.stream, s.d_descs + L.b0, L.partials_err, s.max_blocks, res, L.B, s.nn_tile);
 }
 void lane_fitness_tail(hgs_handle* h, BatchLane& L, const BatchShape& s, const double* fit_max_range) {
@@ -845,7 +863,7 @@
   const int B = s.B, max_blocks = s.max_blocks;
   hgs_cloud* tgt = h->target;
   const bool voxel = h->prm.method == HGS_FAST_VGICP;
-  const GicpConsts c = gicp_consts(h->prm);
+  const GicpConsts c = engine_gicp_consts(h);
   const VgicpConsts vc = vgicp_consts(h->prm);
   const bool round2 = s.gicp_round2;
   const bool early = round2 && B == 1 && !fit_max_range && h->early_result && !h->profiling;
@@ -860,15 +878,62 @@
   const TargetView tv = s.d_tviews || s.d_vviews ? TargetView{} : target_view(tgt);
   const NdtTargetView vtv = voxel && !s.d_vviews ? vgicp_target_view(tgt) : NdtTargetView{};
   const long max_rounds = (long)std::max(1, c.max_iterations) * std::max(1, c.lm_max_iterations) + 2 + (round2 ? 1 : 0);
+  const bool may_score_early = fit_max_range && B > 1 && h->early_fitness && !round2 && !early && !h->profiling;
+  if (may_score_early) {
+    HGS_HIP(h, h->h_finished.reserve((size_t)B * sizeof(int)));
+    HGS_HIP(h, h->fit_partials.reserve((size_t)B * max_blocks * 2 * sizeof(double)));
+  }
   std::vector<BatchLane> lanes;
   HGS_TRY(open_lanes(h, B, (size_t)max_blocks * kAccNdt * sizeof(double), (size_t)max_blocks * 2 * sizeof(double), lanes, s.err_blocks));
+  const bool score_early = may_score_early && lanes.size() > 1;
+  DevResult* const res = h->results.as<DevResult>();
+  volatile int* const finished = score_early ? h->h_finished.as<volatile int>() : nullptr;
+  std::vector<char> scored(score_early ? B : 0, 0);
+  std::vector<int> todo;
+  if (score_early) {
+    for (int b = 0; b < B; b++) finished[b] = 0;
+    for (size_t i = 0; i < lanes.size(); i++)
+      if (!h->score_event[i]) HGS_HIP(h, hipEventCreateWithFlags(&h->score_event[i], hipEventDisableTiming));
+  }
+  auto score = [&](BatchLane& L) {
+    const int flags = fitness_seed_flags(h, corr_seeds_fitness(h->prm.method));
+    for (size_t i = 0; i < todo.size();) {
+      const int base = todo[i];
+      unsigned long long want = 0ull;
+      int span = 0;
+      for (; i < todo.size() && todo[i] - base < 64; i++) want |= 1ull << (todo[i] - base), span = todo[i] - base + 1;
+      double* fp = h->fit_partials.as<double>() + (size_t)base * max_blocks * 2;
+      if (s.d_tviews) launch_fitness(L.stream, s.d_descs + base, s.d_tviews + base, res + base, *fit_max_range, fp, max_blocks, span, flags, s.qpw, ~want);
+      else launch_fitness(L.stream, s.d_descs + base, target_view(h->target), res + base, *fit_max_range, fp, max_blocks, span, flags, s.qpw, ~want);
+      launch_fitness_final(L.stream, s.d_descs + base, fp, max_blocks, res + base, span, s.nn_tile, ~want);
+    }
+    for (int b : todo) scored[b] = 1;
+  };
   auto finish_lane = [&](BatchLane& L) {
     if (early && *L.prog.host_done) {
       h->early_valid = true;
       return;
     }
-    launch_gicp_results(L.stream, st + L.b0, h->results.as<DevResult>() + L.b0, L.B);
-    lane_fitness_tail(h, L, s, fit_max_range);
+    if (!score_early) {
+      launch_gicp_results(L.stream, st + L.b0, res + L.b0, L.B);
+      lane_fitness_tail(h, L, s, fit_max_range);
+      return;
+    }
+    if (!*L.prog.host_done) launch_gicp_results(L.stream, st + L.b0, res + L.b0, L.B, 1);
+    todo.clear();
+    for (int b = L.b0; b < L.b0 + L.B; b++)
+      if (!scored[b]) todo.push_back(b);
+    score(L);
+    for (size_t r = 0; r < lanes.size(); r++) {
+      BatchLane& R = lanes[r];
+      if (&R == &L || R.finished) continue;
+      todo.clear();
+      for (int b = R.b0; b < R.b0 + R.B; b++)
+        if (!scored[b] && finished[b]) todo.push_back(b);
+      if (todo.empty()) continue;
+      if (hipEventRecord(h->score_event[r], R.stream) != hipSuccess || hipStreamWaitEvent(L.stream, h->score_event[r], 0) != hipSuccess) continue;
+      score(L);
+    }
   };
   if (guess_in_args) launch_gicp_init1(lanes[0].stream, st, guesses_host, lanes[0].prog);
   else
@@ -908,7 +973,8 @@
     }
     {
       StageTimer tm(h, HGS_STAGE_SOLVE);
-      launch_gicp_decide(L.stream, dd, ls, c, L.partials_err, max_blocks, L.B, L.prog);
+      launch_gicp_decide(L.stream, dd, ls, c, L.partials_err, max_blocks, L.B, L.prog, score_early ? res + L.b0 : nullptr,
+                         score_early ? const_cast<int*>(finished) + L.b0 : nullptr);
     }
   }, finish_lane, early ? (long)h->early_run_ahead : kRunAhead);
   HGS_TRY(close_lanes(h, lanes));
@@ -922,7 +988,7 @@
 
 int run_icp_rounds(hgs_handle* h, const BatchShape& s, const double* fit_max_range) {
   const int B = s.B, max_blocks = s.max_blocks;
-  const IcpConsts c = icp_consts(h->prm);
+  const IcpConsts c = engine_icp_consts(h);
   HGS_HIP(h, h->states.reserve((size_t)B * sizeof(IcpState)));
   IcpState* st = h->states.as<IcpState>();
   const TargetView tv = s.d_tviews ? TargetView{} : target_view(h->target);
@@ -1295,6 +1361,8 @@
   if (comm) hgs::comm_destroy(comm);
   for (hipEvent_t ev : lane_event)
     if (ev) (void)hipEventDestroy(ev);
+  for (hipEvent_t ev : score_event)
+    if (ev) (void)hipEventDestroy(ev);
   for (hipEvent_t ev : {comm_event, early_event, up_big_event})
     if (ev) (void)hipEventDestroy(ev);
   for (const std::vector<ProfEvent>* list : {&prof_events, &prof_free})
@@ -1326,6 +1394,9 @@
   else if (k == "knn_qpw_tiny") h->knn_qpw_tiny = value < 0 ? -1 : std::max(0, std::min(32, value & ~7));
   else if (k == "knn_tiny_below") h->knn_tiny_below = std::max(0, value);
   else if (k == "seed_grid") h->seed_grid = value != 0 ? 1 : 0;
+  else if (k == "early_fitness") h->early_fitness = value != 0 ? 1 : 0;
+  else if (k == "fitness_borrow_seeds") h->fitness_borrow_seeds = value != 0 ? 1 : 0;
+  else if (k == "ordered_majority") h->ordered_majority = value != 0 ? 1 : 0;
   else if (k == "knn_replay") h->knn_replay = std::max(-1, std::min(2, value));
   else if (k == "ndt_resident") h->ndt_resident_blocks = std::max(0, value);
   else if (k == "ndt_chunk") h->ndt_chunk = std::max(0, value);
@@ -2898,7 +2969,7 @@
   HGS_HIP(h, hipMemcpyAsync(h->misc.p, T12, 12 * sizeof(double), hipMemcpyHostToDevice, h->stream));
   launch_gicp_debug_state(h->stream, h->states.as<GicpState>(), h->misc.as<double>());
   if (voxel) launch_vgicp_linearize(h->stream, d_descs, vgicp_target_view(t), h->states.as<GicpState>(), vgicp_consts(h->prm), h->partials.as<double>(), max_blocks, 1);
-  else launch_gicp_linearize(h->stream, d_descs, target_view(t), h->states.as<GicpState>(), gicp_consts(h->prm), h->partials.as<double>(), max_blocks, 1, 64);
+  else launch_gicp_linearize(h->stream, d_descs, target_view(t), h->states.as<GicpState>(), engine_gicp_consts(h), h->partials.as<double>(), max_blocks, 1, 64);
   double* d_out = h->misc.as<double>() + 16;
   launch_reduce_partials(h->stream, h->partials.as<double>(), max_blocks, kAcc, d_out);
   double acc[kAcc];
@@ -2956,7 +3027,7 @@
   HGS_HIP(h, h->states.reserve(sizeof(IcpState)));
   HGS_HIP(h, h->partials.reserve((size_t)max_blocks * kAccIcp * sizeof(double)));
   HGS_HIP(h, hipMemcpyAsync(h->states.p, &st, sizeof(st), hipMemcpyHostToDevice, h->stream));
-  launch_icp_correspond(h->stream, d_descs, target_view(t), h->states.as<IcpState>(), icp_consts(h->prm), h->partials.as<double>(), max_blocks, 1);
+  launch_icp_correspond(h->stream, d_descs, target_view(t), h->states.as<IcpState>(), engine_icp_consts(h), h->partials.as<double>(), max_blocks, 1);
   HGS_HIP(h, hipGetLastError());
   std::vector<double> part((size_t)max_blocks * kAccIcp);
   int s_nvalid = 0;
diff --git a/hdl_graph_slam_amd/csrc/hgs_gicp.h b/hdl_graph_slam_amd/csrc/hgs_gicp.h
--- a/hdl_graph_slam_amd/csrc/hgs_gicp.h
+++ b/hdl_graph_slam_amd/csrc/hgs_gicp.h
@@ -13,7 +13,9 @@
   int lm_max_iterations;
   int max_iterations;
   int k_correspondences;
+  int nn_flags;
 };
+constexpr int kNnOrderedMajority = 1;
 
 HGS_HD Sym3 gicp_neighbour_cov(const double* s1, const Sym3& s2, int found, int k, double lambda) {
   const double inv_f = 1.0 / (double)found, inv_k = 1.0 / (double)k;
diff --git a/hdl_graph_slam_amd/csrc/hgs_icp.h b/hdl_graph_slam_amd/csrc/hgs_icp.h
--- a/hdl_graph_slam_amd/csrc/hgs_icp.h
+++ b/hdl_graph_slam_amd/csrc/hgs_icp.h
@@ -12,7 +12,7 @@
   double trans_eps;
   double rot_thr;
   int reciprocal;
-  int pad;
+  int nn_flags;
 };
 
 enum IcpPhase { ICP_RUN = 0, ICP_DONE = 2 };
diff --git a/hdl_graph_slam_amd/csrc/hgs_kernels.hip b/hdl_graph_slam_amd/csrc/hgs_kernels.hip
--- a/hdl_graph_slam_amd/csrc/hgs_kernels.hip
+++ b/hdl_graph_slam_amd/csrc/hgs_kernels.hip
@@ -774,11 +774,15 @@
   return best;
 }
 
-__device__ __forceinline__ void packet_nn1(const BvhView& tv, float* park, const F3& q, bool active, float bound2, int seed, int qpw, float& d2, int& pos, int& orig) {
+__device__ __forceinline__ void packet_nn1(const BvhView& tv, float* park, const F3& q, bool active, float bound2, int seed, int qpw, int nn_flags, float& d2, int& pos,
+                                           int& orig) {
   const bool seeded = seed >= 0 && seed < tv.n;
   int leaf;
   bool tie, found;
-  if (__ballot(active && !seeded) != 0ull) wave_nn1_quad<true, true>(tv, park, q, active, bound2, seed, qpw >> 1, d2, leaf, tie, found);
+  const unsigned long long unseeded = __ballot(active && !seeded);
+  bool ordered = unseeded != 0ull;
+  if (ordered && (nn_flags & kNnOrderedMajority)) ordered = 2 * __popcll(unseeded) > __popcll(__ballot(active));
+  if (ordered) wave_nn1_quad<true, true>(tv, park, q, active, bound2, seed, qpw >> 1, d2, leaf, tie, found);
   else wave_nn1_quad<false, true>(tv, park, q, active, bound2, seed, qpw >> 1, d2, leaf, tie, found);
   if (__ballot(tie) != 0ull) {
     const F3 qa[1] = {q};
@@ -895,7 +899,7 @@
   const int seed = active ? __builtin_nontemporal_load(d.corr + idx) : -1;
   float d2;
   int j, orig;
-  packet_nn1(view_of(tgt), park[wave], q, active, c.search_bound2, seed, qpw, d2, j, orig);
+  packet_nn1(view_of(tgt), park[wave], q, active, c.search_bound2, seed, qpw, c.nn_flags, d2, j, orig);
   const double R[9] = {T.m[0], T.m[1], T.m[2], T.m[4], T.m[5], T.m[6], T.m[8], T.m[9], T.m[10]};
   int jj = active ? j : -1;
   if (jj >= 0 && !((double)d2 < c.max_corr2)) jj = -1;
@@ -1061,7 +1065,7 @@
   hipLaunchKernelGGL((k_gicp_error<true, const TargetView*>), dim3(err_blocks, B), dim3(kBlock), 0, s, descs, tviews, states_in, partials_err, max_blocks, c, states_out, partials, lin_tile_points);
 }
 
-__device__ __forceinline__ bool gicp_decide_wave(int ntiles, GicpState* state, const GicpConsts& c, const double* __restrict__ problem_partials_err) {
+__device__ __forceinline__ bool gicp_decide_wave(int ntiles, GicpState* state, const GicpConsts& c, const double* __restrict__ problem_partials_err, DevResult* result_out = nullptr) {
   __shared__ GicpState st;
   __shared__ double ws[kGicpControlWorkspace];
   bool finished_now = false;
@@ -1075,6 +1079,7 @@
   if (threadIdx.x == 0) {
     gicp_after_error(st, s, c, ws);
     finished_now = st.phase == GICP_DONE;
+    if (finished_now && result_out) *result_out = gicp_result_of(st);
   }
   __syncthreads();
   if (threadIdx.x < 64)
@@ -1082,28 +1087,32 @@
   return finished_now;
 }
 __global__ __launch_bounds__(64) __attribute__((amdgpu_waves_per_eu(HGS_CONTROL_WAVES))) void k_gicp_decide(const CloudDesc* descs, GicpState* states, GicpConsts c, const double* __restrict__ partials_err,
-                                                   int max_blocks, Progress prog) {
+                                                   int max_blocks, Progress prog, DevResult* results, int* host_finished) {
   const int b = blockIdx.x;
   bool finished_now = false;
   if (HGS_CONTROL_PRIO) __builtin_amdgcn_s_setprio(HGS_CONTROL_PRIO);
   if (states[b].phase == GICP_TRY) {
     const int ntiles = (descs[b].meta->nvalid + kBlock - 1) / kBlock;
-    finished_now = gicp_decide_wave(ntiles, states + b, c, partials_err + (size_t)b * max_blocks);
-  }
-  if (threadIdx.x == 0) progress_tick(prog, finished_now);
+    finished_now = gicp_decide_wave(ntiles, states + b, c, partials_err + (size_t)b * max_blocks, results ? results + b : nullptr);
+  }
+  if (threadIdx.x == 0) {
+    if (finished_now && host_finished) __hip_atomic_store(host_finished + b, 1, __ATOMIC_RELAXED, __HIP_MEMORY_SCOPE_SYSTEM);
+    progress_tick(prog, finished_now);
+  }
 }
 void launch_gicp_decide(hipStream_t s, const CloudDesc* descs, GicpState* states, GicpConsts c, const double* partials_err, int max_blocks, int B,
-                        Progress prog) {
-  hipLaunchKernelGGL(k_gicp_decide, dim3(B), dim3(64), 0, s, descs, states, c, partials_err, max_blocks, prog);
-}
-
-__global__ void k_gicp_results(const GicpState* states, DevResult* out, int B) {
+                        Progress prog, DevResult* results, int* host_finished) {
+  hipLaunchKernelGGL(k_gicp_decide, dim3(B), dim3(64), 0, s, descs, states, c, partials_err, max_blocks, prog, results, host_finished);
+}
+
+__global__ void k_gicp_results(const GicpState* states, DevResult* out, int B, int unfinished_only) {
   const int b = blockIdx.x * blockDim.x + threadIdx.x;
   if (b >= B) return;
+  if (unfinished_only && states[b].phase == GICP_DONE) return;
   out[b] = gicp_result_of(states[b]);
 }
-void launch_gicp_results(hipStream_t s, const GicpState* states, DevResult* out, int B) {
-  hipLaunchKernelGGL(k_gicp_results, dim3((B + 63) / 64), dim3(64), 0, s, states, out, B);
+void launch_gicp_results(hipStream_t s, const GicpState* states, DevResult* out, int B, int unfinished_only) {
+  hipLaunchKernelGGL(k_gicp_results, dim3((B + 63) / 64), dim3(64), 0, s, states, out, B, unfinished_only);
 }
 
 __global__ void k_icp_init(IcpState* states, const float* guesses, int B, Progress prog) {
@@ -1143,7 +1152,7 @@
   const int seed = active ? __builtin_nontemporal_load(d.corr + idx) : -1;
   float d2;
   int j, orig;
-  packet_nn1(view_of(tgt), park[wave], q, active, c.search_bound2, seed, qpw, d2, j, orig);
+  packet_nn1(view_of(tgt), park[wave], q, active, c.search_bound2, seed, qpw, c.nn_flags, d2, j, orig);
   int jj = active ? j : -1;
   if (jj >= 0 && !((double)d2 <= c.max_corr2)) jj = -1;
   const float4 bp = jj >= 0 ? tgt.pts[jj] : make_float4(0.f, 0.f, 0.f, 0.f);
@@ -1155,7 +1164,7 @@
       sv.nodes = d.nodes, sv.pts = d.pts, sv.lpts = d.lpts, sv.P = d.P, sv.n = n;
       float rd2;
       int rj, rorig;
-      packet_nn1(sv, park[wave], r, ractive, c.search_bound2, ractive ? idx : -1, qpw, rd2, rj, rorig);
+      packet_nn1(sv, park[wave], r, ractive, c.search_bound2, ractive ? idx : -1, qpw, c.nn_flags, rd2, rj, rorig);
       if (ractive && !(rj >= 0 && rorig == __float_as_int(a.w) && (double)rd2 <= c.max_corr2)) jj = -1;
     }
   }
@@ -1230,8 +1239,9 @@
 
 template <typename TGT = TargetView>
 __global__ __launch_bounds__(kBlock) __attribute__((amdgpu_waves_per_eu(HGS_FITNESS_WAVES))) void k_fitness(const CloudDesc* descs, TGT tgt_arg, const DevResult* poses, double max_range,
-                                                    double* __restrict__ partials, int max_blocks, int use_seed, int qpw) {
+                                                    double* __restrict__ partials, int max_blocks, int use_seed, int qpw, unsigned long long skip) {
   const int b = blockIdx.y;
+  if (b < 64 && ((skip >> b) & 1ull)) return;
   const TargetView& tgt = problem_target(tgt_arg, b);
   const CloudDesc d = descs[b];
   const int n = d.meta->nvalid;
@@ -1255,10 +1265,28 @@
   const bool active = (int)(threadIdx.x & 63) < qpw && idx < n;
   const float4 a = active ? load_stream(d.pts + idx) : make_float4(0.f, 0.f, 0.f, 0.f);
   const F3 q = transform_point_f(Tf, a.x, a.y, a.z);
-  int seed = (active && use_seed) ? __builtin_nontemporal_load(d.corr + idx) : -1;
+  int seed = (active && (use_seed & kFitnessCorrSeeds)) ? __builtin_nontemporal_load(d.corr + idx) : -1;
   const BvhView tv = view_of(tgt);
   if (tgt.seed_bits && __ballot(active && !(seed >= 0 && seed < tv.n)) != 0ull) {
     if (active && !(seed >= 0 && seed < tv.n)) seed = seed_grid_lookup(tgt, q);
+  }
+  {
+    const bool has_seed = seed >= 0 && seed < tv.n;
+    const unsigned long long needy = __ballot(active && !has_seed), donors = __ballot(active && has_seed);
+    if ((use_seed & kFitnessBorrowSeeds) && needy != 0ull && donors != 0ull) {
+      int l;
+      HGS_LANE_ID(l);
+      int* slot = reinterpret_cast<int*>(park[wave]);
+      __builtin_amdgcn_wave_barrier();
+      slot[l] = seed;
+      __builtin_amdgcn_wave_barrier();
+      const unsigned long long below = donors & ((1ull << l) - 1ull), above = (donors >> l) >> 1;
+      const int dn = below ? l - (63 - __clzll((long long)below)) : 128, up = above ? __ffsll((long long)above) : 128;
+      const int from = dn <= up ? l - dn : l + up;
+      const int borrowed = slot[from & 63];
+      __builtin_amdgcn_wave_barrier();
+      if (active && !has_seed) seed = borrowed;
+    }
   }
   const bool seeded = seed >= 0 && seed < tv.n;
   float d2;
@@ -1277,15 +1305,16 @@
   last_wave_stores<2>(lds, &arrivals, partials + ((size_t)b * max_blocks + tile) * 2, lane);
 }
 void launch_fitness(hipStream_t s, const CloudDesc* descs, TargetView tgt, const DevResult* poses, double max_range, double* partials, int max_blocks,
-                    int B, int use_seed, int qpw) {
-  hipLaunchKernelGGL(k_fitness<TargetView>, dim3(HGS_GRID_X(max_blocks), B), dim3(kBlock), 0, s, descs, tgt, poses, max_range, partials, max_blocks, use_seed, qpw);
+                    int B, int use_seed, int qpw, unsigned long long skip) {
+  hipLaunchKernelGGL(k_fitness<TargetView>, dim3(HGS_GRID_X(max_blocks), B), dim3(kBlock), 0, s, descs, tgt, poses, max_range, partials, max_blocks, use_seed, qpw, skip);
 }
 void launch_fitness(hipStream_t s, const CloudDesc* descs, const TargetView* tviews, const DevResult* poses, double max_range, double* partials, int max_blocks,
-                    int B, int use_seed, int qpw) {
-  hipLaunchKernelGGL(k_fitness<const TargetView*>, dim3(HGS_GRID_X(max_blocks), B), dim3(kBlock), 0, s, descs, tviews, poses, max_range, partials, max_blocks, use_seed, qpw);
-}
-__global__ __launch_bounds__(64) void k_fitness_final(const CloudDesc* descs, const double* __restrict__ partials, int max_blocks, DevResult* out, int tile_pts) {
+                    int B, int use_seed, int qpw, unsigned long long skip) {
+  hipLaunchKernelGGL(k_fitness<const TargetView*>, dim3(HGS_GRID_X(max_blocks), B), dim3(kBlock), 0, s, descs, tviews, poses, max_range, partials, max_blocks, use_seed, qpw, skip);
+}
+__global__ __launch_bounds__(64) void k_fitness_final(const CloudDesc* descs, const double* __restrict__ partials, int max_blocks, DevResult* out, int tile_pts, unsigned long long skip) {
   const int b = blockIdx.x;
+  if (b < 64 && ((skip >> b) & 1ull)) return;
   const int ntiles = (descs[b].meta->nvalid + tile_pts - 1) / tile_pts;
   double s = 0, c = 0;
   for (int t = threadIdx.x; t < ntiles; t += 64) {
@@ -1295,8 +1324,8 @@
   s = wave_sum(s), c = wave_sum(c);
   if (threadIdx.x == 0) out[b].fit_sum = s, out[b].fit_count = (unsigned)(c + 0.5);
 }
-void launch_fitness_final(hipStream_t s, const CloudDesc* descs, const double* partials, int max_blocks, DevResult* out, int B, int tile_pts) {
-  hipLaunchKernelGGL(k_fitness_final, dim3(B), dim3(64), 0, s, descs, partials, max_blocks, out, tile_pts);
+void launch_fitness_final(hipStream_t s, const CloudDesc* descs, const double* partials, int max_blocks, DevResult* out, int B, int tile_pts, unsigned long long skip) {
+  hipLaunchKernelGGL(k_fitness_final, dim3(B), dim3(64), 0, s, descs, partials, max_blocks, out, tile_pts, skip);
 }
 
 __global__ void k_results_to_records(const DevResult* __restrict__ res, const int* __restrict__ candidate_ids, int n, int n_slots, hgs_result* __restrict__ out) {
```

Result: no change. 5990 registrations/sec, median of 6 (+0.6%).
